# nka77/DAHiTra

Hardware: AMD Instinct MI355X
Metric: image-pairs/s (256x256) train step, 1/2/4/8 MI355X + CPU ref (higher is better)
Workload: dtype bf16; 1 GPU; LEVIR-CD 256x256 synthetic pairs, base_transformer_pos_s4, bf16, batch 32 per GPU (global 32), fwd+focal+bwd+allreduce+AdamW; net_G=base_transformer_pos_s4, global_batch=32, img_size=256, parallelism=dp1, hip_graph=True, step_form=one graph (AdamW inside), attn_dtype=bf16

## Files before the change

dahitra_amd/csrc/common.h:

```cpp
#pragma once
#include <hip/hip_runtime.h>
#include <stdint.h>

struct bf16 { unsigned short x; };

typedef __attribute__((ext_vector_type(4))) float f32x4;
typedef __attribute__((ext_vector_type(8))) short s16x8;
typedef __attribute__((ext_vector_type(4))) short s16x4;

#define DH_DTYPE_F32 0
#define DH_DTYPE_BF16 1

struct f32x3 { float v; };
struct f32x6 { float v; };
struct f32h3 { float v; };
constexpr float F32H3_WSCALE = 256.f;
template <typename T> struct Prec {
    static constexpr int NPL = 1;
    static constexpr bool X3 = false;
    static constexpr int CK = 64 / (int)sizeof(T);
};
template <> struct Prec<f32x3> {
    static constexpr int NPL = 2;
    static constexpr bool X3 = true;
// ... 116 lines not shown
#pragma unroll
    for (int j = 0; j < 8; ++j) r[j] = x[j];
#pragma unroll
    for (int p = 0; p < NPL; ++p) {
        pl[p] = pack16<bf16>(r);
        if (p + 1 < NPL) {
            float h[8];
            unpack16(pl[p], h);
#pragma unroll
            for (int j = 0; j < 8; ++j) r[j] -= h[j];
        }
    }
}
template <int NPL> __device__ __forceinline__ void split_bf16_planes(const uint4& a, const uint4& b, uint4 (&pl)[NPL]) {
    const float x[8] = {__uint_as_float(a.x), __uint_as_float(a.y), __uint_as_float(a.z), __uint_as_float(a.w),
                        __uint_as_float(b.x), __uint_as_float(b.y), __uint_as_float(b.z), __uint_as_float(b.w)};
    split_bf16_planes<NPL>(x, pl);
}
__device__ __forceinline__ void split_bf16x3(const float (&x)[8], uint4& hi, uint4& lo) {
    hi = pack16<bf16>(x);
    float h[8], r[8];
    unpack16(hi, h);
#pragma unroll
    for (int j = 0; j < 8; ++j) r[j] = x[j] - h[j];
    lo = pack16<bf16>(r);
}
__device__ __forceinline__ void split_bf16x3(const uint4& a, const uint4& b, uint4& hi, uint4& lo) {
    const float x[8] = {__uint_as_float(a.x), __uint_as_float(a.y), __uint_as_float(a.z), __uint_as_float(a.w),
                        __uint_as_float(b.x), __uint_as_float(b.y), __uint_as_float(b.z), __uint_as_float(b.w)};
    split_bf16x3(x, hi, lo);
}

__device__ __forceinline__ float row16_sum(float v) {
    v += __builtin_bit_cast(float, __builtin_amdgcn_update_dpp(0, __builtin_bit_cast(int, v), 0x128, 0xf, 0xf, false));
    v += __builtin_bit_cast(float, __builtin_amdgcn_update_dpp(0, __builtin_bit_cast(int, v), 0x124, 0xf, 0xf, false));
    v += __builtin_bit_cast(float, __builtin_amdgcn_update_dpp(0, __builtin_bit_cast(int, v), 0x122, 0xf, 0xf, false));
    v += __builtin_bit_cast(float, __builtin_amdgcn_update_dpp(0, __builtin_bit_cast(int, v), 0x121, 0xf, 0xf, false));
    return v;
}

__device__ __forceinline__ float wave_sum(float v) {
#pragma unroll
    for (int o = 32; o > 0; o >>= 1) v += __shfl_xor(v, o, 64);
    return v;
}
__device__ __forceinline__ float wave_max(float v) {
#pragma unroll
    for (int o = 32; o > 0; o >>= 1) v = fmaxf(v, __shfl_xor(v, o, 64));
    return v;
}

__device__ __forceinline__ float gelu_erf(float x) { return 0.5f * x * (1.0f + erff(x * 0.70710678118654752440f)); }
__device__ __forceinline__ float gelu_erf_grad(float x) {
    const float cdf = 0.5f * (1.0f + erff(x * 0.70710678118654752440f));
    const float pdf = 0.39894228040143267794f * __expf(-0.5f * x * x);
    return cdf + x * pdf;
}

#define DH_ACT_NONE 0
#define DH_ACT_RELU 1
#define DH_ACT_GELU 2

#include <stdio.h>
#include <string.h>
extern "C" void dh_set_error(const char* msg);
#define DH_FAIL(...)                                                     \
    do {                                                                 \
        char _b[512];                                                    \
        snprintf(_b, sizeof(_b), __VA_ARGS__);                           \
        dh_set_error(_b);                                                \
        return 1;                                                        \
    } while (0)
#define DH_REQUIRE(cond, ...)           \
    do {                                \
        if (!(cond)) DH_FAIL(__VA_ARGS__); \
    } while (0)
#define DH_CHECK_LAUNCH(name)                                                      \
    do {                                                                           \
        hipError_t _e = hipGetLastError();                                         \
        if (_e != hipSuccess) DH_FAIL("%s launch: %s", name, hipGetErrorString(_e)); \
    } while (0)
static inline int dh_cdiv(long a, long b) { return (int)((a + b - 1) / b); }

__device__ __forceinline__ void dh_reduce_partials_body(const float* __restrict__ partial, long nt, long n, float scale,
                                                        float* __restrict__ out, int accumulate, int bx, double (*red)[32]) {
    const int lane = threadIdx.x & 31, ph = threadIdx.x >> 5;
    const long i = (long)bx * 32 + lane;
    double s = 0.0;
    if (i < n) {
        double s1 = 0.0, s2 = 0.0, s3 = 0.0;
        long t = ph;
#pragma unroll 4
        for (; t + 24 < nt; t += 32) {
            s += (double)partial[t * n + i];
            s1 += (double)partial[(t + 8) * n + i];
            s2 += (double)partial[(t + 16) * n + i];
            s3 += (double)partial[(t + 24) * n + i];
        }
        for (; t < nt; t += 8) s += (double)partial[t * n + i];
        s = (s + s1) + (s2 + s3);
    }
    red[ph][lane] = s;
    __syncthreads();
    if (ph == 0 && i < n) {
        double t = 0.0;
#pragma unroll
        for (int r = 0; r < 8; ++r) t += red[r][lane];
        const float v = (float)(t * scale);
        if (accumulate) out[i] += v; else out[i] = v;
    }
}


__device__ __forceinline__ double dh_block_sum_f64(double v, double* sh) {
    for (int o = 32; o > 0; o >>= 1) v += __shfl_down(v, o, 64);
    const int w = threadIdx.x >> 6, l = threadIdx.x & 63;
    __syncthreads();
    if (l == 0) sh[w] = v;
    __syncthreads();
    double t = 0.0;
    if (threadIdx.x == 0) for (int i = 0; i < (int)(blockDim.x >> 6); ++i) t += sh[i];
    return t;
}
```

dahitra_amd/csrc/conv_wgrad.hip:

```cpp
#include "common.h"

namespace {

constexpr int TH = 8, TW = 16;
static inline int co_tile(int Cout) { return Cout <= 16 ? 16 : (Cout <= 32 ? 32 : 64); }

struct WgArgs {
    const void* x;
    const void* dy;
    float* part;
    int N, H, W, Cin, OH, OW, Cout, pad;
    int tilesX, tilesY, splitk, groups, npix, in_npix;
    int ci_tiles;
    int CinPitch;
    int dil;
    int CoutUse;
    int direct;
    const float* in_scale;
    const float* in_shift;
    int in_groups;
    int phase_mode;
    int no_xcd_remap;
    const void* dyt_y;
    const float* dytoef;
// ... 407 lines not shown
                }
            }
        }
        __syncthreads();
    }

    if constexpr (KSPLIT > 1) {
        float* red = reinterpret_cast<float*>(smem);
        for (int q = 1; q < KSPLIT; ++q) {
            if (kq == q) {
#pragma unroll
                for (int t = 0; t < TAPS; ++t)
#pragma unroll
                    for (int i = 0; i < NI; ++i)
                        *reinterpret_cast<f32x4*>(red + (((size_t)cw * TAPS * NI + t * NI + i) * 64 + lane) * 4) = acc[t][i];
            }
            __syncthreads();
            if (kq == 0) {
#pragma unroll
                for (int t = 0; t < TAPS; ++t)
#pragma unroll
                    for (int i = 0; i < NI; ++i) {
                        const f32x4 o = *reinterpret_cast<const f32x4*>(red + (((size_t)cw * TAPS * NI + t * NI + i) * 64 + lane) * 4);
                        acc[t][i][0] += o[0]; acc[t][i][1] += o[1]; acc[t][i][2] += o[2]; acc[t][i][3] += o[3];
                    }
            }
            __syncthreads();
        }
        if (kq != 0) return;
    }
    const int cob = co0 + (WCI ? 2 * cig * 16 : cw * 16) + g * 4, cib = ci0 + (WCI ? wv * 16 : cig * IT) + pl;
    float* out = p.part + ((size_t)grp * p.splitk + kz) * TAPS * p.Cout * p.Cin + (size_t)cob * p.Cin + cib;
    const int tstride = p.Cout * p.Cin;
    const int istep = WCI ? 16 * p.Cin : 16;
    bool okij[NI][4];
#pragma unroll
    for (int i = 0; i < NI; ++i)
#pragma unroll
        for (int j = 0; j < 4; ++j)
            okij[i][j] = WCI ? (cob + i * 16 + j < p.CoutUse && cib < p.Cin) : (cob + j < p.CoutUse && cib + i * 16 < p.Cin);
    if (p.direct == 2) {
#pragma unroll
        for (int t = 0; t < TAPS; ++t)
#pragma unroll
            for (int i = 0; i < NI; ++i)
#pragma unroll
                for (int j = 0; j < 4; ++j)
                    if (okij[i][j]) out[t * tstride + j * p.Cin + i * istep] += acc[t][i][j];
    } else {
#pragma unroll
        for (int t = 0; t < TAPS; ++t)
#pragma unroll
            for (int i = 0; i < NI; ++i)
#pragma unroll
                for (int j = 0; j < 4; ++j)
                    if (okij[i][j]) out[t * tstride + j * p.Cin + i * istep] = acc[t][i][j];
    }
}
template <typename T, int KS, int STRIDE, int IT, bool TR, int DIL, int CTT, int CIG, bool DYT = false>
__global__ __launch_bounds__(256 * CIG) void conv_wgrad_kernel(WgArgs p) {
    extern __shared__ __attribute__((aligned(16))) unsigned char smem[];
    wg_body<T, KS, STRIDE, IT, TR, DIL, CTT, CIG, DYT>(p, blockIdx.x, blockIdx.y, gridDim.x, gridDim.y, blockIdx.z, smem);
}
constexpr int WS_MAXJ = 16;
struct WsMulti {
    int njobs;
    int first[WS_MAXJ + 1];
    WgArgs a[WS_MAXJ];
};
static_assert(sizeof(WsMulti) <= 4096, "the kernel argument block");
template <typename T, int KS, int STRIDE, int IT, bool TR, int DIL, int CTT, int CIG>
__global__ __launch_bounds__(256 * CIG) void conv_wgrad_multi_kernel(WsMulti m) {
    extern __shared__ __attribute__((aligned(16))) unsigned char smem[];
    int j = 0;
    while (j + 1 < m.njobs && (int)blockIdx.x >= m.first[j + 1]) ++j;
    const WgArgs p = m.a[j];
    const int nbx = ((p.CoutUse + CTT - 1) / CTT) * p.ci_tiles, local = (int)blockIdx.x - m.first[j];
    if (local >= nbx * p.splitk) return;
    wg_body<T, KS, STRIDE, IT, TR, DIL, CTT, CIG, false>(p, local % nbx, local / nbx, nbx, p.splitk, 0, smem);
}

static inline int wgrad_reduce_epb(int I) { return (I & 3) == 0 ? 128 : 32; }
__device__ __forceinline__ void wgrad_reduce_block(const float* __restrict__ part, int splitk, int taps, int Oslab, int O,
                                                   int I, float* __restrict__ dw, int accumulate, long block, float (*red)[132]) {
    const long n = (long)O * I * taps;
    const int lane = threadIdx.x & 31, ph = threadIdx.x >> 5;
    const bool vec = (I & 3) == 0;
    const long i = vec ? (block * 32 + lane) * 4 : block * 32 + lane;
    float acc[4] = {0.f, 0.f, 0.f, 0.f};
    int tap = 0, ci = 0, o = 0;
    if (i < n) {
        ci = (int)(i % I);
        o = (int)((i / I) % O);
        tap = (int)(i / ((long)I * O));
        const size_t slab = (size_t)taps * Oslab * I;
        const float* src = part + ((size_t)tap * Oslab + o) * I + ci;
        if (vec) {
            float4 a0 = make_float4(0.f, 0.f, 0.f, 0.f), a1 = a0, a2 = a0, a3 = a0;
            auto add = [](float4& a, const float4 v) { a.x += v.x; a.y += v.y; a.z += v.z; a.w += v.w; };
            int k = ph;
            for (; k + 24 < splitk; k += 32) {
                add(a0, *reinterpret_cast<const float4*>(src + (size_t)k * slab));
                add(a1, *reinterpret_cast<const float4*>(src + (size_t)(k + 8) * slab));
                add(a2, *reinterpret_cast<const float4*>(src + (size_t)(k + 16) * slab));
                add(a3, *reinterpret_cast<const float4*>(src + (size_t)(k + 24) * slab));
            }
            for (; k < splitk; k += 8) add(a0, *reinterpret_cast<const float4*>(src + (size_t)k * slab));
            acc[0] = (a0.x + a1.x) + (a2.x + a3.x); acc[1] = (a0.y + a1.y) + (a2.y + a3.y);
            acc[2] = (a0.z + a1.z) + (a2.z + a3.z); acc[3] = (a0.w + a1.w) + (a2.w + a3.w);
        } else {
            float a1 = 0.f, a2 = 0.f, a3 = 0.f;
            int k = ph;
            for (; k + 24 < splitk; k += 32) {
                acc[0] += src[(size_t)k * slab];
                a1 += src[(size_t)(k + 8) * slab];
                a2 += src[(size_t)(k + 16) * slab];
                a3 += src[(size_t)(k + 24) * slab];
            }
            for (; k < splitk; k += 8) acc[0] += src[(size_t)k * slab];
            acc[0] = (acc[0] + a1) + (a2 + a3);
        }
    }
#pragma unroll
    for (int e = 0; e < 4; ++e) red[ph][lane * 4 + e] = acc[e];
    __syncthreads();
    const int t = threadIdx.x;
    if (t < (vec ? 128 : 32)) {
        const int l2 = vec ? t >> 2 : t, e = vec ? t & 3 : 0;
        const long i2 = vec ? (block * 32 + l2) * 4 + e : block * 32 + l2;
        if (i2 < n) {
            float s = 0.f;
#pragma unroll
            for (int r = 0; r < 8; ++r) s += red[r][l2 * 4 + e];
            const int ci2 = (int)(i2 % I), o2 = (int)((i2 / I) % O), tap2 = (int)(i2 / ((long)I * O));
            const size_t d = ((size_t)o2 * I + ci2) * taps + tap2;
            if (accumulate) dw[d] += s; else dw[d] = s;
        }
    }
}
__global__ void wgrad_reduce_oihw_kernel(const float* __restrict__ part, int splitk, int taps, int Oslab, int O, int I,
                                         float* __restrict__ dw, int accumulate) {
    __shared__ float red[8][132];
    const long n = (long)O * I * taps;
    wgrad_reduce_block(part + (size_t)blockIdx.y * splitk * taps * Oslab * I, splitk, taps, Oslab, O, I,
                       dw + (size_t)blockIdx.y * n, accumulate, blockIdx.x, red);
}
struct WgReduceJob {
    const float* part;
    float* dw;
    int splitk, taps, Oslab, O, I, accumulate, first_block, nblocks;
};
__global__ void wgrad_reduce_multi_kernel(const WgReduceJob* __restrict__ jobs, int njobs) {
    __shared__ float red[8][132];
    int j = 0;
    while (j + 1 < njobs && (int)blockIdx.x >= jobs[j + 1].first_block) ++j;
    const WgReduceJob job = jobs[j];
    wgrad_reduce_block(job.part, job.splitk, job.taps, job.Oslab, job.O, job.I, job.dw, job.accumulate,
                       (long)blockIdx.x - job.first_block, red);
}

#ifdef DH_WS_TIMING
__device__ long long g_ws[4096 * 16];
#define WS_NOW() ((long long)wall_clock64())
#define WS_T(...) __VA_ARGS__
#else
#define WS_T(...)
#endif
template <int DIL>
__device__ __forceinline__ void ws_body(const WgArgs& p, int bx, int kz, const int nbx, const int nkz, unsigned char* smem) {
    constexpr int KS = 3, TAPS = 9;
    constexpr int HH = (TH - 1) + (KS - 1) * DIL + 1, HWD = (TW - 1) + (KS - 1) * DIL + 1;
    constexpr int XP = lds_pitch(128), DP = lds_pitch(128);
    constexpr int STAGE = HH * HWD * XP + TH * TW * DP;
    float* bnp = reinterpret_cast<float*>(smem + 2 * STAGE);

    const int tid = threadIdx.x, lane = tid & 63, wv = tid >> 6;
    const int pl = lane & 15, g = lane >> 4;
    if (nbx > 1 && (nkz & 7) == 0 && !p.no_xcd_remap) {
        const unsigned lin = (unsigned)(kz * nbx + bx), xcd = lin & 7, sq = lin >> 3;
        bx = (int)(sq % nbx);
        kz = (int)((sq / nbx) * 8 + xcd);
    }
    const int cot = bx / p.ci_tiles, cit = bx % p.ci_tiles;
    const int co0 = cot * 64, ci0 = cit * 64;
    const int tiles_per_img = p.tilesX * p.tilesY;
    const int ntiles = p.N * tiles_per_img;
    const int my_tiles = kz < ntiles ? (ntiles - kz + p.splitk - 1) / p.splitk : 0;

    if (p.in_scale) {
        for (int i = tid; i < p.in_groups * 128; i += 512) {
            const int gi = i >> 7, k = (i >> 6) & 1, c = i & 63;
            bnp[i] = (k ? p.in_shift : p.in_scale)[gi * p.Cin + ci0 + c];
        }
        __syncthreads();
    }

    if (wv >= 4) {
        const int pt = tid - 256, q = pt & 7, prow = pt >> 3;
        constexpr int NXV = (HH * HWD + 31) / 32, NDV = TH * TW / 32;
        struct Regs { uint4 rx[NXV], rd[NDV]; unsigned okmask; int bng; };
        Regs RA, RB;
        int x_h[NXV];
#pragma unroll
        for (int i = 0; i < NXV; ++i) {
            const int px = prow + 32 * i;
            x_h[i] = px < HH * HWD ? ((px / HWD) << 8) | (px % HWD) : -1;
        }
        const unsigned xps = (unsigned)p.CinPitch * 2u, dps = (unsigned)p.Cout * 2u;
        const bool upper = p.x_split && ci0 >= p.Cin / 2;
        const long xsel = upper ? p.x_split : 0L;
        const unsigned xcb = (unsigned)((upper ? ci0 - p.Cin / 2 : ci0) + q * 8) * 2u, dcb = (unsigned)(co0 + q * 8) * 2u;
        const int dn = p.splitk / tiles_per_img, drem = p.splitk % tiles_per_img;
        const int dty = drem / p.tilesX, dtx = drem % p.tilesX;
        int f_n = kz / tiles_per_img, f_ty = (kz % tiles_per_img) / p.tilesX, f_tx = (kz % tiles_per_img) % p.tilesX;
        auto fetch = [&](Regs& R) {
            const int n = f_n;
            R.bng = p.in_scale ? n / (p.N / p.in_groups) : 0;
            const int oy0 = f_ty * TH, ox0 = f_tx * TW, iy0 = oy0 - p.pad, ix0 = ox0 - p.pad;
            const unsigned char* xb = reinterpret_cast<const unsigned char*>(p.x) + xsel + (size_t)n * p.H * p.W * xps;
            const unsigned char* db = reinterpret_cast<const unsigned char*>(p.dy) + (size_t)n * p.OH * p.OW * dps;
            R.okmask = 0;
#pragma unroll
            for (int i = 0; i < NXV; ++i) {
                const int iy = iy0 + (x_h[i] >> 8), ix = ix0 + (x_h[i] & 0xff);
                const bool ok = x_h[i] >= 0 && (unsigned)iy < (unsigned)p.H && (unsigned)ix < (unsigned)p.W;
                const uint4 v = *reinterpret_cast<const uint4*>(xb + (ok ? (unsigned)(iy * p.W + ix) * xps + xcb : 0u));
                R.rx[i] = ok ? v : make_uint4(0, 0, 0, 0);
                R.okmask |= ok ? (1u << i) : 0u;
            }
#pragma unroll
            for (int i = 0; i < NDV; ++i) {
                const int px = prow + 32 * i, oy = oy0 + (px >> 4), ox = ox0 + (px & 15);
                const bool ok = oy < p.OH && ox < p.OW;
                const uint4 v = *reinterpret_cast<const uint4*>(db + (ok ? (unsigned)(oy * p.OW + ox) * dps + dcb : 0u));
                R.rd[i] = ok ? v : make_uint4(0, 0, 0, 0);
            }
            f_tx += dtx;
            if (f_tx >= p.tilesX) { f_tx -= p.tilesX; ++f_ty; }
            f_ty += dty;
            if (f_ty >= p.tilesY) { f_ty -= p.tilesY; ++f_n; }
            f_n += dn;
// ... 565 lines not shown
    a.in_npix = npix_valid > 0 ? npix_valid : H * W;
    hipStream_t st = reinterpret_cast<hipStream_t>(stream);
    if (x_split) {
        a.ci_tiles = dh_cdiv(Cin, 64);
        DH_REQUIRE(dtype == DH_DTYPE_BF16 && ws_eligible(a, ks, stride, true, use_tr != 0) && wide_ci3x3(Cin, a.CoutUse, ks),
                   "conv2d_wgrad: a split input is served by the wave-specialised 3x3 kernel only (Cin=%d Cout=%d ks=%d)", Cin, Cout, ks);
    }
    const bool batching = g_wsb.on;
    if (!defer) g_wsb.on = false;
    int rc = dtype == DH_DTYPE_BF16 ? launch_all<bf16>(a, ks, stride, use_tr != 0, st)
             : wgrad_x3(dtype, a)   ? launch_all<f32x3>(a, ks, stride, true, st)
                                    : launch_all<float>(a, ks, stride, false, st);
    g_wsb.on = batching;
    if (rc) return rc;
    if (splitk_out) *splitk_out = a.direct ? 0 : a.splitk;
    if (a.direct || defer) return 0;
    const int taps = ks * ks;
    const int oreal = Cout_real > 0 ? Cout_real : Cout;
    const long n = (long)oreal * Cin * taps;
    hipLaunchKernelGGL(wgrad_reduce_oihw_kernel, dim3(dh_cdiv(n, wgrad_reduce_epb(Cin)), groups), dim3(256), 0, st, a.part, a.splitk,
                       taps, Cout, oreal, Cin, dw_oihw, accumulate);
    DH_CHECK_LAUNCH("wgrad_reduce");
    return 0;
}

extern "C" int dh_wgrad_batch_begin() { g_wsb.on = true; g_wsb.n = 0; g_wsb.lds = 0; g_c32b.n = 0; g_c32b.lds = 0; return 0; }
extern "C" int dh_wgrad_batch_pending() { return g_wsb.n + g_c32b.n; }
extern "C" int dh_wgrad_batch_abort() { g_wsb.on = false; g_wsb.n = 0; g_wsb.lds = 0; g_c32b.n = 0; g_c32b.lds = 0; return 0; }
extern "C" int dh_wgrad_batch_launch(void* stream) {
    const int rc = ws_batch_flush(reinterpret_cast<hipStream_t>(stream));
    return rc ? rc : c32_batch_flush(reinterpret_cast<hipStream_t>(stream));
}
extern "C" int dh_wgrad_batch_end(void* stream) {
    const int rc = dh_wgrad_batch_launch(stream);
    g_wsb.on = false;
    return rc;
}

extern "C" int dh_conv2d_wgrad(int dtype, const void* x, const void* dy, float* dw_oihw, int accumulate, int N,
                               int H, int W, int Cin, int OH, int OW, int Cout, int ks, int stride, int pad,
                               int groups, int npix_valid, int use_tr, int Cout_real, int cin_pitch, int dilation,
                               void* workspace, void* stream) {
    return conv2d_wgrad_impl(dtype, x, dy, dw_oihw, accumulate, N, H, W, Cin, OH, OW, Cout, ks, stride, pad, groups,
                             npix_valid, use_tr, Cout_real, cin_pitch, dilation, workspace, stream, 0, nullptr);
}

extern "C" int dh_conv2d_wgrad_partial(int dtype, const void* x, const void* dy, float* dw_oihw, int accumulate, int N,
                                       int H, int W, int Cin, int OH, int OW, int Cout, int ks, int stride, int pad,
                                       int groups, int npix_valid, int use_tr, int Cout_real, int cin_pitch,
                                       int dilation, void* workspace, int* splitk_out, void* stream) {
    DH_REQUIRE(groups == 1 && splitk_out, "conv2d_wgrad_partial: one group only");
    return conv2d_wgrad_impl(dtype, x, dy, dw_oihw, accumulate, N, H, W, Cin, OH, OW, Cout, ks, stride, pad, groups,
                             npix_valid, use_tr, Cout_real, cin_pitch, dilation, workspace, stream, 1, splitk_out);
}
bool dh_wgrad_split_supported(int N, int H, int W, int Cin, int Cout) {
    WgArgs a;
    memset(&a, 0, sizeof(a));
    a.dil = 1; a.in_groups = 1; a.dyt_groups = 1;
    a.N = N; a.H = H; a.W = W; a.Cin = Cin; a.OH = H; a.OW = W; a.Cout = Cout; a.CoutUse = Cout; a.pad = 1; a.groups = 1;
    a.CinPitch = Cin / 2; a.x_split = 16; a.npix = H * W; a.in_npix = H * W;
    return ws_eligible(a, 3, 1, true, true) && wide_ci3x3(Cin, Cout, 3);
}
extern "C" int dh_conv2d_wgrad_split(const void* x, long x_split_bytes, const void* dy, float* dw_oihw, int accumulate, int N, int H,
                                     int W, int Cin, int Cout, void* workspace, int* splitk_out, void* stream) {
    DH_REQUIRE(x_split_bytes > 0 && x_split_bytes % 16 == 0 && Cin % 128 == 0 && splitk_out, "conv2d_wgrad_split: bad arguments (Cin=%d)", Cin);
    return conv2d_wgrad_impl(DH_DTYPE_BF16, x, dy, dw_oihw, accumulate, N, H, W, Cin, H, W, Cout, 3, 1, 1, 1, 0, 1, 0, Cin / 2, 1,
                             workspace, stream, 1, splitk_out, nullptr, nullptr, 1, nullptr, nullptr, 1, x_split_bytes);
}
extern "C" int dh_conv2d_wgrad_bn_in(int dtype, const void* x, const void* dy, float* dw_oihw, int accumulate, int N,
                                     int H, int W, int Cin, int OH, int OW, int Cout, int ks, int stride, int pad,
                                     int use_tr, int Cout_real, int dilation, const float* in_scale, const float* in_shift,
                                     int in_groups, void* workspace, int* splitk_out, void* stream) {
    DH_REQUIRE(in_scale && in_shift, "conv2d_wgrad_bn_in: scale / shift missing");
    return conv2d_wgrad_impl(dtype, x, dy, dw_oihw, accumulate, N, H, W, Cin, OH, OW, Cout, ks, stride, pad, 1, 0, use_tr,
                             Cout_real, 0, dilation, workspace, stream, splitk_out ? 1 : 0, splitk_out, in_scale, in_shift,
                             in_groups);
}
extern "C" int dh_stem_wgrad_bn(const void* xs16, const void* d, const void* y, const float* coef, int groups, int N, int OH,
                                int OW, float* dw2, int use_tr, void* workspace, void* stream) {
    DH_REQUIRE(xs16 && d && y && coef && groups >= 1 && N % groups == 0, "stem_wgrad_bn: bad arguments (N=%d groups=%d)", N, groups);
    return conv2d_wgrad_impl(DH_DTYPE_BF16, xs16, d, dw2, 0, N, OH, OW, 16, OH, OW, 64, 4, 1, 2, 1, 0, use_tr, 0, 16, 1, workspace,
                             stream, 0, nullptr, nullptr, nullptr, 1, y, coef, groups);
}
extern "C" int dh_wgrad_reduce_job_size(void) { return (int)sizeof(WgReduceJob); }
extern "C" int dh_wgrad_reduce_outputs_per_block(int Cin) { return wgrad_reduce_epb(Cin); }
extern "C" int dh_wgrad_reduce_multi(const void* jobs_dev, int njobs, int total_blocks, void* stream) {
    if (njobs <= 0) return 0;
    hipLaunchKernelGGL(wgrad_reduce_multi_kernel, dim3(total_blocks), dim3(256), 0, reinterpret_cast<hipStream_t>(stream),
                       reinterpret_cast<const WgReduceJob*>(jobs_dev), njobs);
    DH_CHECK_LAUNCH("wgrad_reduce_multi");
    return 0;
}

static int phase_splitk(int N, int H, int W, int Cin) {
    const long tiles = (long)N * dh_cdiv(W, TW) * dh_cdiv(H, TH);
    const long slabs = (long)dh_cdiv(Cin, 32);
    long sk = (128 + slabs - 1) / slabs;
    if (sk > tiles / 8) sk = tiles / 8;
    return (int)(sk < 1 ? 1 : sk);
}
extern "C" long dh_conv2d_wgrad_phase_workspace_size(int N, int H, int W, int Cin) {
    return (long)4 * phase_splitk(N, H, W, Cin) * 4 * 32 * Cin * 4;
}
extern "C" int dh_conv2d_wgrad_phase(int dtype, const void* x, const void* dy, int N, int H, int W, int Cin, int use_tr,
                                     void* workspace, int* splitk_out, void* stream) {
    DH_REQUIRE(splitk_out && workspace, "conv2d_wgrad_phase: workspace / splitk_out missing");
    DH_REQUIRE((Cin * (dtype == DH_DTYPE_BF16 ? 2 : 4)) % 16 == 0, "conv2d_wgrad_phase: Cin=%d not 16-byte aligned", Cin);
    WgArgs a;
    a.x = x; a.dy = dy; a.part = reinterpret_cast<float*>(workspace);
    a.dil = 1; a.phase_mode = 1;
    a.no_xcd_remap = getenv("DAHITRA_NO_XCD_REMAP") ? 1 : 0;
    a.dyt_y = nullptr; a.dytoef = nullptr; a.dyt_groups = 1;
    a.in_scale = nullptr; a.in_shift = nullptr; a.in_groups = 1;
    a.CinPitch = Cin;
    a.N = N; a.H = H; a.W = W; a.Cin = Cin; a.OH = H; a.OW = W; a.Cout = 32; a.pad = 1;
    a.tilesX = dh_cdiv(W, TW); a.tilesY = dh_cdiv(H, TH);
    a.CoutUse = 32;
    a.x_split = 0;
    a.groups = 1; a.splitk = phase_splitk(N, H, W, Cin);
    a.direct = 0;
    a.npix = H * W; a.in_npix = H * W;
    hipStream_t st = reinterpret_cast<hipStream_t>(stream);
    const int rc = dtype == DH_DTYPE_BF16 ? launch_all<bf16>(a, 2, 1, use_tr != 0, st)
                   : wgrad_x3(dtype, a)   ? launch_all<f32x3>(a, 2, 1, true, st) : launch_all<float>(a, 2, 1, false, st);
    if (rc) return rc;
    *splitk_out = a.splitk;
    return 0;
}

namespace {
__global__ void phase_wgrad_combine_kernel(const float* __restrict__ dwab, float* __restrict__ dw, int Cin, int accumulate) {
    const int i = blockIdx.x * blockDim.x + threadIdx.x;
    if (i >= 32 * Cin) return;
    const size_t pstride = (size_t)32 * Cin * 4;
    const float* src = dwab + (size_t)i * 4;
    float v[4][4];
#pragma unroll
    for (int ph = 0; ph < 4; ++ph) {
        const float4 q = *reinterpret_cast<const float4*>(src + ph * pstride);
        v[ph][0] = q.x; v[ph][1] = q.y; v[ph][2] = q.z; v[ph][3] = q.w;
    }
    const int ra[3][2] = {{0, 1}, {0, 1}, {0, 1}}, rt[3][2] = {{0, 0}, {1, 0}, {1, 1}};
#pragma unroll
    for (int kh = 0; kh < 3; ++kh)
#pragma unroll
        for (int kw = 0; kw < 3; ++kw) {
            float s = 0.f;
#pragma unroll
            for (int m = 0; m < 2; ++m)
#pragma unroll
                for (int n = 0; n < 2; ++n) s += v[ra[kh][m] * 2 + ra[kw][n]][rt[kh][m] * 2 + rt[kw][n]];
            float* d = dw + (size_t)i * 9 + kh * 3 + kw;
            if (accumulate) *d += s; else *d = s;
        }
}

template <typename T>
__global__ void pack_phase_weights_kernel(const float* __restrict__ w, const float* __restrict__ bias, int Cin,
                                          T* __restrict__ fwd, T* __restrict__ dgrad, float* __restrict__ bias4) {
    const int i = blockIdx.x * blockDim.x + threadIdx.x;
    if (i < 128 && bias4) bias4[i] = bias ? bias[i & 31] : 0.f;
    if (i >= 32 * Cin) return;
    const int co = i / Cin, ci = i % Cin;
    float k[3][3];
#pragma unroll
    for (int j = 0; j < 9; ++j) k[j / 3][j % 3] = w[(size_t)i * 9 + j];
    const int lo[2][2] = {{0, 1}, {0, 2}}, hi[2][2] = {{0, 2}, {1, 2}};
#pragma unroll
    for (int a = 0; a < 2; ++a)
#pragma unroll
        for (int b = 0; b < 2; ++b)
#pragma unroll
            for (int t = 0; t < 2; ++t)
#pragma unroll
                for (int u = 0; u < 2; ++u) {
                    float s = 0.f;
                    for (int kh = lo[a][t]; kh <= hi[a][t]; ++kh)
                        for (int kw = lo[b][u]; kw <= hi[b][u]; ++kw) s += k[kh][kw];
                    const int ph = a * 2 + b;
                    if (fwd) stf(fwd + ((size_t)(t * 2 + u) * 128 + ph * 32 + co) * Cin + ci, s);
                    if (dgrad) stf(dgrad + ((size_t)((1 - t) * 2 + (1 - u)) * Cin + ci) * 128 + ph * 32 + co, s);
                }
}
}

namespace {
template <typename T>
__global__ void pack_s2_dgrad_phase_kernel(const float* __restrict__ w, int Co, int Ci, T* __restrict__ out) {
    const int i = blockIdx.x * blockDim.x + threadIdx.x;
    if (i >= Co * Ci) return;
    const int co = i / Ci, ci = i % Ci;
    float k[3][3];
#pragma unroll
    for (int j = 0; j < 9; ++j) k[j / 3][j % 3] = w[(size_t)i * 9 + j];
    const int kmap[2][2] = {{-1, 1}, {2, 0}};
#pragma unroll
    for (int a = 0; a < 2; ++a)
#pragma unroll
        for (int b = 0; b < 2; ++b)
#pragma unroll
            for (int t = 0; t < 2; ++t)
#pragma unroll
                for (int u = 0; u < 2; ++u) {
                    const int kh = kmap[a][t], kw = kmap[b][u];
                    const float v = (kh >= 0 && kw >= 0) ? k[kh][kw] : 0.f;
                    stf(out + ((size_t)(t * 2 + u) * 4 * Ci + (a * 2 + b) * Ci + ci) * Co + co, v);
                }
}
}
extern "C" int dh_pack_s2_dgrad_phase_weights(int dtype, const float* w_oihw, int Co, int Ci, void* out, void* stream) {
    DH_REQUIRE((Ci == 32 || Ci == 64) && Co % 16 == 0, "pack_s2_dgrad_phase_weights: Ci=%d (32 or 64) Co=%d", Ci, Co);
    const dim3 grid(dh_cdiv(Co * Ci, 256));
    hipStream_t st = reinterpret_cast<hipStream_t>(stream);
    if (dtype == DH_DTYPE_BF16) hipLaunchKernelGGL(pack_s2_dgrad_phase_kernel<bf16>, grid, dim3(256), 0, st, w_oihw, Co, Ci, (bf16*)out);
    else hipLaunchKernelGGL(pack_s2_dgrad_phase_kernel<float>, grid, dim3(256), 0, st, w_oihw, Co, Ci, (float*)out);
    DH_CHECK_LAUNCH("pack_s2_dgrad_phase_weights");
    return 0;
}
extern "C" int dh_phase_wgrad_combine(const float* dwab, float* dw_oihw, int Cin, int accumulate, void* stream) {
    hipLaunchKernelGGL(phase_wgrad_combine_kernel, dim3(dh_cdiv(32 * Cin, 256)), dim3(256), 0, reinterpret_cast<hipStream_t>(stream),
                       dwab, dw_oihw, Cin, accumulate);
    DH_CHECK_LAUNCH("phase_wgrad_combine");
    return 0;
}
extern "C" int dh_pack_phase_weights(int dtype, const float* w_oihw, const float* bias, int Cin, void* fwd, void* dgrad,
                                     float* bias4, void* stream) {
    DH_REQUIRE(Cin % 16 == 0, "pack_phase_weights: Cin=%d", Cin);
    const dim3 grid(dh_cdiv(32 * Cin, 256));
    hipStream_t st = reinterpret_cast<hipStream_t>(stream);
    if (dtype == DH_DTYPE_BF16)
        hipLaunchKernelGGL(pack_phase_weights_kernel<bf16>, grid, dim3(256), 0, st, w_oihw, bias, Cin, (bf16*)fwd, (bf16*)dgrad, bias4);
    else
        hipLaunchKernelGGL(pack_phase_weights_kernel<float>, grid, dim3(256), 0, st, w_oihw, bias, Cin, (float*)fwd, (float*)dgrad, bias4);
    DH_CHECK_LAUNCH("pack_phase_weights");
    return 0;
}
```

dahitra_amd/csrc/pointwise.hip:

```cpp
#include "common.h"

namespace {

inline int ew_grid(long n, int block) {
    long g = (n + block - 1) / block;
    return (int)(g > 8192 ? 8192 : (g < 1 ? 1 : g));
}
#define GSL(i, n) for (long i = (long)blockIdx.x * blockDim.x + threadIdx.x; i < (n); i += (long)gridDim.x * blockDim.x)

template <typename T>
__global__ void nchw_to_nhwc_kernel(const float* __restrict__ src, T* __restrict__ dst, int N, int C, long HW, int CP) {
    const long total = (long)N * HW * CP;
    GSL(i, total) {
        const int c = (int)(i % CP);
        const long p = (i / CP) % HW;
        const long n = i / (CP * HW);
        stf(dst + i, c < C ? src[(n * C + c) * HW + p] : 0.f);
    }
}
template <typename T>
__global__ void nchw_to_nhwc_piece_kernel(const float* __restrict__ src, T* __restrict__ dst, int N, int C, long HW) {
    constexpr int V = V16<T>::N;
    const long total = (long)N * HW;
    GSL(i, total) {
// ... 702 lines not shown

template <typename T>
__global__ void absdiff_kernel(const T* __restrict__ a, const T* __restrict__ b, T* __restrict__ y, long n) {
    GSL(i, n) stf(y + i, fabsf(ldf(a + i) - ldf(b + i)));
}
template <typename T>
__global__ void absdiff_bwd_kernel(const T* __restrict__ a, const T* __restrict__ b, const T* __restrict__ dy,
                                   T* __restrict__ da, T* __restrict__ db, long n, int accumulate) {
    GSL(i, n) {
        const float df = ldf(a + i) - ldf(b + i);
        const float sg = df > 0.f ? 1.f : (df < 0.f ? -1.f : 0.f);
        const float g = sg * ldf(dy + i);
        if (accumulate) { stf(da + i, ldf(da + i) + g); stf(db + i, ldf(db + i) - g); }
        else { stf(da + i, g); stf(db + i, -g); }
    }
}

template <typename T>
__global__ void zero_insert2_kernel(const T* __restrict__ dy, T* __restrict__ z, int N, int OH, int OW, int H, int W,
                                    int C) {
    const int vn = C / 4;
    GSL(i, (long)N * H * W * vn) {
        const int c = (int)(i % vn) * 4;
        long t = i / vn;
        const int x = (int)(t % W); t /= W;
        const int y = (int)(t % H);
        const long n = t / H;
        float v[4] = {0, 0, 0, 0};
        if (!(x & 1) && !(y & 1) && y / 2 < OH && x / 2 < OW) ld4(dy + ((n * OH + y / 2) * OW + x / 2) * C + c, v);
        st4(z + i * 4, v);
    }
}

template <typename T>
__global__ void add_coarse_kernel(T* __restrict__ x, const T* __restrict__ coarse, int N, int OH, int OW, int H, int W, int C) {
    constexpr int V = V16<T>::N;
    const int vn = C / V;
    GSL(i, (long)N * OH * OW * vn) {
        const int c = (int)(i % vn) * V;
        long t = i / vn;
        const int ox = (int)(t % OW); t /= OW;
        const int oy = (int)(t % OH);
        const long n = t / OH;
        if (2 * oy >= H || 2 * ox >= W) continue;
        float a[V], b[V];
        T* dst = x + ((n * H + 2 * oy) * W + 2 * ox) * C + c;
        ldv(dst, a);
        ldv(coarse + i * V, b);
#pragma unroll
        for (int j = 0; j < V; ++j) a[j] += b[j];
        stv(dst, a);
    }
}

template <typename T>
__global__ void pack_weight_kernel(const float* __restrict__ w, const float* __restrict__ oscale, int O, int I, int KS,
                                   int OPad, T* __restrict__ fwd, int IPad, int OK, T* __restrict__ dgrad) {
    const int taps = KS * KS;
    if (fwd) {
        GSL(i, (long)taps * OPad * I) {
            const int ci = (int)(i % I);
            const int o = (int)((i / I) % OPad);
            const int tap = (int)(i / ((long)I * OPad));
            stf(fwd + i, o < O ? w[((long)o * I + ci) * taps + tap] * (oscale ? oscale[o] : 1.f) : 0.f);
        }
    }
    if (dgrad) {
        GSL(i, (long)taps * IPad * OK) {
            const int o = (int)(i % OK);
            const int ci = (int)((i / OK) % IPad);
            const int tap = (int)(i / ((long)OK * IPad));
            stf(dgrad + i, (ci < I && o < O) ? w[((long)o * I + ci) * taps + (taps - 1 - tap)] : 0.f);
        }
    }
}

struct PackJob {
    const float* w;
    void* fwd;
    void* dgrad;
    int O, I, KS, OPad, IPad, OK;
    int dtype;
    int first_block, nblocks;
};
template <typename T>
__device__ __forceinline__ void pack_store8(T* dst, const float* __restrict__ src, unsigned stride, unsigned okmask) {
    float v[8];
#pragma unroll
    for (int e = 0; e < 8; ++e) v[e] = ((okmask >> e) & 1) ? src[(size_t)e * stride] : 0.f;
    if constexpr (sizeof(T) == 2) {
        uint4 u;
        u.x = f2bf2(v[0], v[1]); u.y = f2bf2(v[2], v[3]); u.z = f2bf2(v[4], v[5]); u.w = f2bf2(v[6], v[7]);
        *reinterpret_cast<uint4*>(dst) = u;
    } else {
        *reinterpret_cast<float4*>(dst) = make_float4(v[0], v[1], v[2], v[3]);
        *reinterpret_cast<float4*>(dst + 4) = make_float4(v[4], v[5], v[6], v[7]);
    }
}
template <typename T> __device__ __forceinline__ void pack_put8(T* dst, const float (&v)[8]) {
    if constexpr (sizeof(T) == 2) {
        uint4 u;
        u.x = f2bf2(v[0], v[1]); u.y = f2bf2(v[2], v[3]); u.z = f2bf2(v[4], v[5]); u.w = f2bf2(v[6], v[7]);
        *reinterpret_cast<uint4*>(dst) = u;
    } else {
        *reinterpret_cast<float4*>(dst) = make_float4(v[0], v[1], v[2], v[3]);
        *reinterpret_cast<float4*>(dst + 4) = make_float4(v[4], v[5], v[6], v[7]);
    }
}
constexpr int PK_T = 32, PK_ROW = PK_T * 9, PK_PITCH = PK_ROW + 1;
__host__ __device__ inline bool pack_tiled(const PackJob& j) {
    return j.KS == 3 && j.O % PK_T == 0 && j.I % PK_T == 0 && j.OPad == j.O && j.IPad == j.I && j.OK == j.O &&
           (reinterpret_cast<unsigned long long>(j.w) & 15) == 0;
}
template <typename T>
__device__ __forceinline__ void pack_job_tiled(const PackJob& j, int lb, float* t ) {
    const int tid = threadIdx.x, nti = j.I / PK_T, ntiles = (j.O / PK_T) * nti;
    T* fwd = reinterpret_cast<T*>(j.fwd);
    T* dgrad = reinterpret_cast<T*>(j.dgrad);
    const bool frag = (j.dtype & 0x200) != 0;
    for (int tile = lb; tile < ntiles; tile += j.nblocks) {
        const int o0 = (tile / nti) * PK_T, c0 = (tile % nti) * PK_T;
        __syncthreads();
        for (int q = tid; q < PK_T * (PK_ROW / 4); q += 256) {
            const int r = q / (PK_ROW / 4), k = (q % (PK_ROW / 4)) * 4;
            const float4 v = *reinterpret_cast<const float4*>(j.w + ((size_t)(o0 + r) * j.I + c0) * 9 + k);
            float* d = t + r * PK_PITCH + k;
            d[0] = v.x; d[1] = v.y; d[2] = v.z; d[3] = v.w;
        }
        __syncthreads();
        for (int q = tid; q < 9 * PK_T * 4; q += 256) {
            float v[8];
            if (frag) {
                const int lane = q & 63, tap = (q >> 6) % 9, blk = q / (64 * 9);
                const int rr = blk * 16 + (lane & 15), kk = (lane >> 4) * 8;
                if (fwd) {
#pragma unroll
                    for (int e = 0; e < 8; ++e) v[e] = t[rr * PK_PITCH + (kk + e) * 9 + tap];
                    pack_put8(fwd + ((((size_t)(o0 / 16 + blk) * (j.I / 32) + c0 / 32) * 9 + tap) * 64 + lane) * 8, v);
                }
                if (dgrad) {
#pragma unroll
                    for (int e = 0; e < 8; ++e) v[e] = t[(kk + e) * PK_PITCH + rr * 9 + (8 - tap)];
                    pack_put8(dgrad + ((((size_t)(c0 / 16 + blk) * (j.OK / 32) + o0 / 32) * 9 + tap) * 64 + lane) * 8, v);
                }
            } else {
                const int pc = q & 3, r = (q >> 2) & 31, tap = q >> 7;
                if (fwd) {
#pragma unroll
                    for (int e = 0; e < 8; ++e) v[e] = t[r * PK_PITCH + (pc * 8 + e) * 9 + tap];
                    pack_put8(fwd + ((size_t)tap * j.OPad + o0 + r) * j.I + c0 + pc * 8, v);
                }
                if (dgrad) {
#pragma unroll
                    for (int e = 0; e < 8; ++e) v[e] = t[(pc * 8 + e) * PK_PITCH + r * 9 + (8 - tap)];
                    pack_put8(dgrad + ((size_t)tap * j.IPad + c0 + r) * j.OK + o0 + pc * 8, v);
                }
            }
        }
    }
}
template <typename T>
__device__ __forceinline__ void pack_job(const PackJob& j, int lb) {
    const int taps = j.KS * j.KS;
    const unsigned step = (unsigned)j.nblocks * blockDim.x;
    T* fwd = reinterpret_cast<T*>(j.fwd);
    T* dgrad = reinterpret_cast<T*>(j.dgrad);
    const unsigned t0 = (unsigned)lb * blockDim.x + threadIdx.x;
    if (j.dtype & 0x200) {
        const int nch_f = j.I / 32, nch_d = j.OK / 32;
        if (fwd)
            for (unsigned i8 = t0; i8 < (unsigned)(taps * j.OPad * j.I) / 8; i8 += step) {
                const unsigned i = i8 * 8;
                const int lane = (int)((i >> 3) & 63), tap = (int)((i >> 9) % (unsigned)taps);
                const int c = (int)((i / (512u * (unsigned)taps)) % (unsigned)nch_f), r16 = (int)(i / (512u * (unsigned)taps * (unsigned)nch_f));
                const int o = r16 * 16 + (lane & 15), ci = c * 32 + (lane >> 4) * 8;
                pack_store8(fwd + i, j.w + (unsigned)((o * j.I + ci) * taps + tap), (unsigned)taps, o < j.O ? 0xffu : 0u);
            }
        if (dgrad)
            for (unsigned i8 = t0; i8 < (unsigned)(taps * j.IPad * j.OK) / 8; i8 += step) {
                const unsigned i = i8 * 8;
                const int lane = (int)((i >> 3) & 63), tap = (int)((i >> 9) % (unsigned)taps);
                const int c = (int)((i / (512u * (unsigned)taps)) % (unsigned)nch_d), r16 = (int)(i / (512u * (unsigned)taps * (unsigned)nch_d));
                const int ci = r16 * 16 + (lane & 15), o = c * 32 + (lane >> 4) * 8;
                unsigned ok = 0;
#pragma unroll
                for (int e = 0; e < 8; ++e) ok |= (unsigned)(ci < j.I && o + e < j.O) << e;
                pack_store8(dgrad + i, j.w + (unsigned)((o * j.I + ci) * taps + (taps - 1 - tap)), (unsigned)(j.I * taps), ok);
            }
        return;
    }
    if (fwd) {
        if (j.I % 8 == 0) {
            for (unsigned i8 = t0; i8 < (unsigned)(taps * j.OPad * j.I) / 8; i8 += step) {
                const unsigned i = i8 * 8;
                const int ci = (int)(i % (unsigned)j.I);
                const int o = (int)((i / (unsigned)j.I) % (unsigned)j.OPad);
                const int tap = (int)(i / (unsigned)(j.I * j.OPad));
                pack_store8(fwd + i, j.w + (unsigned)((o * j.I + ci) * taps + tap), (unsigned)taps, o < j.O ? 0xffu : 0u);
            }
        } else {
            for (unsigned i = t0; i < (unsigned)(taps * j.OPad * j.I); i += step) {
                const int ci = (int)(i % (unsigned)j.I);
                const int o = (int)((i / (unsigned)j.I) % (unsigned)j.OPad);
                const int tap = (int)(i / (unsigned)(j.I * j.OPad));
                stf(fwd + i, o < j.O ? j.w[(unsigned)((o * j.I + ci) * taps + tap)] : 0.f);
            }
        }
    }
    if (dgrad) {
        if (j.OK % 8 == 0) {
            for (unsigned i8 = t0; i8 < (unsigned)(taps * j.IPad * j.OK) / 8; i8 += step) {
                const unsigned i = i8 * 8;
                const int o = (int)(i % (unsigned)j.OK);
                const int ci = (int)((i / (unsigned)j.OK) % (unsigned)j.IPad);
                const int tap = (int)(i / (unsigned)(j.OK * j.IPad));
                unsigned ok = 0;
#pragma unroll
                for (int e = 0; e < 8; ++e) ok |= (unsigned)(ci < j.I && o + e < j.O) << e;
                pack_store8(dgrad + i, j.w + (unsigned)((o * j.I + ci) * taps + (taps - 1 - tap)), (unsigned)(j.I * taps), ok);
            }
        } else {
            for (unsigned i = t0; i < (unsigned)(taps * j.IPad * j.OK); i += step) {
                const int o = (int)(i % (unsigned)j.OK);
                const int ci = (int)((i / (unsigned)j.OK) % (unsigned)j.IPad);
                const int tap = (int)(i / (unsigned)(j.OK * j.IPad));
                stf(dgrad + i, (ci < j.I && o < j.O) ? j.w[(unsigned)((o * j.I + ci) * taps + (taps - 1 - tap))] : 0.f);
            }
        }
    }
}
__global__ __launch_bounds__(256) void pack_weights_multi_kernel(const PackJob* __restrict__ jobs, int njobs) {
    int lo = 0, hi = njobs - 1;
    while (lo < hi) {
        const int mid = (lo + hi + 1) >> 1;
        if (jobs[mid].first_block <= (int)blockIdx.x) lo = mid; else hi = mid - 1;
    }
    const PackJob j = jobs[lo];
    const int lb = blockIdx.x - j.first_block;
    __shared__ __attribute__((aligned(16))) float tile[PK_T * PK_PITCH];
    if (pack_tiled(j)) {
        if ((j.dtype & 0xff) == DH_DTYPE_BF16) pack_job_tiled<bf16>(j, lb, tile); else pack_job_tiled<float>(j, lb, tile);
        return;
    }
    if ((j.dtype & 0xff) == DH_DTYPE_BF16) pack_job<bf16>(j, lb); else pack_job<float>(j, lb);
}

template <typename T>
__global__ __launch_bounds__(256) void colsum_partial_kernel(const T* __restrict__ x, long P, int C,
                                                             float* __restrict__ partial) {
    __shared__ float red[256 * 8];
    constexpr int V = sizeof(T) == 2 ? 8 : 4;
    if (C % V == 0 && C <= 1024 && 256 % (C / V) == 0) {
        const int cvn = C / V, cv = threadIdx.x % cvn, ph = threadIdx.x / cvn, nph = 256 / cvn;
        float s[4][V];
#pragma unroll
        for (int u = 0; u < 4; ++u)
#pragma unroll
            for (int j = 0; j < V; ++j) s[u][j] = 0.f;
        const long step = (long)gridDim.x * nph;
        long p = (long)blockIdx.x * nph + ph;
        auto row = [&](long r, float (&acc)[V]) {
            float v[V];
            if constexpr (V == 8) unpack16(*reinterpret_cast<const uint4*>(x + r * C + cv * V), v);
            else ld4(x + r * C + cv * V, v);
#pragma unroll
            for (int j = 0; j < V; ++j) acc[j] += v[j];
        };
        for (; p + 3 * step < P; p += 4 * step) {
            row(p, s[0]); row(p + step, s[1]); row(p + 2 * step, s[2]); row(p + 3 * step, s[3]);
        }
        for (int u = 0; p < P; p += step, ++u) row(p, s[u & 3]);
        float* mine = red + threadIdx.x * V;
#pragma unroll
        for (int j = 0; j < V; ++j) mine[j] = (s[0][j] + s[1][j]) + (s[2][j] + s[3][j]);
        __syncthreads();
        for (int c = threadIdx.x; c < C; c += 256) {
            float t = 0.f;
            for (int r = 0; r < nph; ++r) t += red[(r * cvn + c / V) * V + (c % V)];
            partial[(long)blockIdx.x * C + c] = t;
        }
        return;
    }
    const int c = threadIdx.x % C, ph = threadIdx.x / C, nph = 256 / C;
    float s = 0.f;
    if (ph < nph)
        for (long p = (long)blockIdx.x * nph + ph; p < P; p += (long)gridDim.x * nph) s += ldf(x + p * C + c);
    red[threadIdx.x] = s;
    __syncthreads();
    if (threadIdx.x < C) {
        float t = 0.f;
        for (int r = 0; r < nph; ++r) t += red[r * C + threadIdx.x];
        partial[(long)blockIdx.x * C + threadIdx.x] = t;
    }
}

template <typename T>
__global__ void cast_from_f32_kernel(const float* __restrict__ src, T* __restrict__ dst, long n) {
    GSL(i, n) stf(dst + i, src[i]);
}
template <typename T>
__global__ void cast_to_f32_kernel(const T* __restrict__ src, float* __restrict__ dst, long n, int accumulate) {
    GSL(i, n) { if (accumulate) dst[i] += ldf(src + i); else dst[i] = ldf(src + i); }
}

}

#define ST(s) reinterpret_cast<hipStream_t>(s)
extern "C" int dh_reduce_partials(const float* partial, long nt, long n, float scale, float* out, int accumulate,
                                  void* stream);

extern "C" int dh_nchw_to_nhwc(int dtype, const float* src, void* dst, int N, int C, long HW, int CP, void* stream) {
    if (CP < C) CP = C;
    const long n = (long)N * CP * HW;
    if (CP * (dtype == DH_DTYPE_BF16 ? 2 : 4) == 16) {
        const long np = (long)N * HW;
        if (dtype == DH_DTYPE_BF16) hipLaunchKernelGGL(nchw_to_nhwc_piece_kernel<bf16>, dim3(ew_grid(np, 256)), dim3(256), 0, ST(stream), src, (bf16*)dst, N, C, HW);
        else hipLaunchKernelGGL(nchw_to_nhwc_piece_kernel<float>, dim3(ew_grid(np, 256)), dim3(256), 0, ST(stream), src, (float*)dst, N, C, HW);
        DH_CHECK_LAUNCH("nchw_to_nhwc");
        return 0;
    }
    if (dtype == DH_DTYPE_BF16) hipLaunchKernelGGL(nchw_to_nhwc_kernel<bf16>, dim3(ew_grid(n, 256)), dim3(256), 0, ST(stream), src, (bf16*)dst, N, C, HW, CP);
// ... 178 lines not shown
    return 0;
}
extern "C" int dh_upsample2_nearest_bwd(int dtype, const void* dy, void* dx, int N, int H, int W, int C, void* stream) {
    const int V = dtype == DH_DTYPE_BF16 ? 8 : 4;
    DH_REQUIRE(C % V == 0, "upsample2: C=%d must be a multiple of %d", C, V);
    const long n = (long)N * H * W * (C / V);
    if (dtype == DH_DTYPE_BF16) hipLaunchKernelGGL(up2_bwd_kernel<bf16>, dim3(ew_grid(n, 256)), dim3(256), 0, ST(stream), (const bf16*)dy, (bf16*)dx, N, H, W, C);
    else hipLaunchKernelGGL(up2_bwd_kernel<float>, dim3(ew_grid(n, 256)), dim3(256), 0, ST(stream), (const float*)dy, (float*)dx, N, H, W, C);
    DH_CHECK_LAUNCH("up2_bwd");
    return 0;
}
extern "C" int dh_absdiff_upsample4_fwd(int dtype, const void* a, const void* b, void* y, int N, int H, int W, int C, void* stream) {
    const int V = dtype == DH_DTYPE_BF16 ? 8 : 4;
    DH_REQUIRE(C % V == 0, "absdiff_upsample4: C=%d must be a multiple of %d", C, V);
    const long n = (long)N * H * W * (C / V);
    if (dtype == DH_DTYPE_BF16) hipLaunchKernelGGL(absdiff_up4_fwd_kernel<bf16>, dim3(ew_grid(n, 256)), dim3(256), 0, ST(stream), (const bf16*)a, (const bf16*)b, (bf16*)y, N, H, W, C);
    else hipLaunchKernelGGL(absdiff_up4_fwd_kernel<float>, dim3(ew_grid(n, 256)), dim3(256), 0, ST(stream), (const float*)a, (const float*)b, (float*)y, N, H, W, C);
    DH_CHECK_LAUNCH("absdiff_up4_fwd");
    return 0;
}
extern "C" int dh_absdiff_upsample4_bwd(int dtype, const void* a, const void* b, const void* dy, void* da, void* db, int N, int H, int W, int C, void* stream) {
    const int V = dtype == DH_DTYPE_BF16 ? 8 : 4;
    DH_REQUIRE(C % V == 0, "absdiff_upsample4: C=%d must be a multiple of %d", C, V);
    const long n = (long)N * H * W * (C / V);
    if (dtype == DH_DTYPE_BF16) hipLaunchKernelGGL(absdiff_up4_bwd_kernel<bf16>, dim3(ew_grid(n, 256)), dim3(256), 0, ST(stream), (const bf16*)a, (const bf16*)b, (const bf16*)dy, (bf16*)da, (bf16*)db, N, H, W, C);
    else hipLaunchKernelGGL(absdiff_up4_bwd_kernel<float>, dim3(ew_grid(n, 256)), dim3(256), 0, ST(stream), (const float*)a, (const float*)b, (const float*)dy, (float*)da, (float*)db, N, H, W, C);
    DH_CHECK_LAUNCH("absdiff_up4_bwd");
    return 0;
}
extern "C" int dh_absdiff_up4_combine(const float* partial, const void* a, const void* b, void* da, void* db, int N, int H, int W,
                                      void* stream) {
    DH_REQUIRE(H % 2 == 0 && W % 4 == 0, "absdiff_up4_combine: coarse map %dx%d must tile into 8x16 fine tiles", H, W);
    const long n = (long)N * H * W * 4;
    hipLaunchKernelGGL(absdiff_up4_combine_kernel, dim3(ew_grid(n, 256)), dim3(256), 0, ST(stream), partial, (const bf16*)a,
                       (const bf16*)b, (bf16*)da, (bf16*)db, N, H, W);
    DH_CHECK_LAUNCH("absdiff_up4_combine");
    return 0;
}
extern "C" int dh_absdiff(int dtype, const void* a, const void* b, void* y, long n, void* stream) {
    if (dtype == DH_DTYPE_BF16) hipLaunchKernelGGL(absdiff_kernel<bf16>, dim3(ew_grid(n, 256)), dim3(256), 0, ST(stream), (const bf16*)a, (const bf16*)b, (bf16*)y, n);
    else hipLaunchKernelGGL(absdiff_kernel<float>, dim3(ew_grid(n, 256)), dim3(256), 0, ST(stream), (const float*)a, (const float*)b, (float*)y, n);
    DH_CHECK_LAUNCH("absdiff");
    return 0;
}
extern "C" int dh_absdiff_bwd(int dtype, const void* a, const void* b, const void* dy, void* da, void* db, long n, int accumulate, void* stream) {
    if (dtype == DH_DTYPE_BF16) hipLaunchKernelGGL(absdiff_bwd_kernel<bf16>, dim3(ew_grid(n, 256)), dim3(256), 0, ST(stream), (const bf16*)a, (const bf16*)b, (const bf16*)dy, (bf16*)da, (bf16*)db, n, accumulate);
    else hipLaunchKernelGGL(absdiff_bwd_kernel<float>, dim3(ew_grid(n, 256)), dim3(256), 0, ST(stream), (const float*)a, (const float*)b, (const float*)dy, (float*)da, (float*)db, n, accumulate);
    DH_CHECK_LAUNCH("absdiff_bwd");
    return 0;
}
extern "C" int dh_zero_insert2(int dtype, const void* dy, void* z, int N, int OH, int OW, int H, int W, int C, void* stream) {
    DH_REQUIRE(C % 4 == 0, "zero_insert2: C %% 4");
    const long n = (long)N * H * W * (C / 4);
    if (dtype == DH_DTYPE_BF16) hipLaunchKernelGGL(zero_insert2_kernel<bf16>, dim3(ew_grid(n, 256)), dim3(256), 0, ST(stream), (const bf16*)dy, (bf16*)z, N, OH, OW, H, W, C);
    else hipLaunchKernelGGL(zero_insert2_kernel<float>, dim3(ew_grid(n, 256)), dim3(256), 0, ST(stream), (const float*)dy, (float*)z, N, OH, OW, H, W, C);
    DH_CHECK_LAUNCH("zero_insert2");
    return 0;
}
extern "C" int dh_add_coarse(int dtype, void* x, const void* coarse, int N, int OH, int OW, int H, int W, int C, void* stream) {
    const int V = dtype == DH_DTYPE_BF16 ? 8 : 4;
    DH_REQUIRE(C % V == 0 && x && coarse && OH == (H + 1) / 2 && OW == (W + 1) / 2, "add_coarse: C=%d, %dx%d <- %dx%d", C, H, W, OH, OW);
    const long n = (long)N * OH * OW * (C / V);
    if (dtype == DH_DTYPE_BF16) hipLaunchKernelGGL(add_coarse_kernel<bf16>, dim3(ew_grid(n, 256)), dim3(256), 0, ST(stream), (bf16*)x, (const bf16*)coarse, N, OH, OW, H, W, C);
    else hipLaunchKernelGGL(add_coarse_kernel<float>, dim3(ew_grid(n, 256)), dim3(256), 0, ST(stream), (float*)x, (const float*)coarse, N, OH, OW, H, W, C);
    DH_CHECK_LAUNCH("add_coarse");
    return 0;
}
extern "C" int dh_pack_weight(int dtype, const float* w_oihw, const float* out_scale, int O, int I, int ks, int OPad, void* fwd, int IPad, int dgrad_inner, void* dgrad, void* stream) {
    const int OK = dgrad_inner > O ? dgrad_inner : O;
    const long n = (long)ks * ks * (OPad > IPad ? OPad : IPad) * (OK > I ? OK : I);
    if (dtype == DH_DTYPE_BF16) hipLaunchKernelGGL(pack_weight_kernel<bf16>, dim3(ew_grid(n, 256)), dim3(256), 0, ST(stream), w_oihw, out_scale, O, I, ks, OPad, (bf16*)fwd, IPad, OK, (bf16*)dgrad);
    else hipLaunchKernelGGL(pack_weight_kernel<float>, dim3(ew_grid(n, 256)), dim3(256), 0, ST(stream), w_oihw, out_scale, O, I, ks, OPad, (float*)fwd, IPad, OK, (float*)dgrad);
    DH_CHECK_LAUNCH("pack_weight");
    return 0;
}
extern "C" int dh_pack_job_size(void) { return (int)sizeof(PackJob); }
extern "C" int dh_pack_weights_multi(const void* jobs_dev, int njobs, int total_blocks, void* stream) {
    if (njobs <= 0) return 0;
    hipLaunchKernelGGL(pack_weights_multi_kernel, dim3(total_blocks), dim3(256), 0, ST(stream),
                       reinterpret_cast<const PackJob*>(jobs_dev), njobs);
    DH_CHECK_LAUNCH("pack_weights_multi");
    return 0;
}
extern "C" int dh_colsum(int dtype, const void* x, long P, int C, float* out, int accumulate, void* workspace, void* stream) {
    DH_REQUIRE(C >= 1 && C <= 256, "colsum: C=%d out of range", C);
    const long rows_per_pass = 256 / (C >= 4 && (C & 3) == 0 ? C / 4 : C);
    long want = (P + rows_per_pass * 8 - 1) / (rows_per_pass * 8);
    const int grid = (int)(want < 64 ? 64 : (want > 256 ? 256 : want));
    float* partial = reinterpret_cast<float*>(workspace);
    if (dtype == DH_DTYPE_BF16) hipLaunchKernelGGL(colsum_partial_kernel<bf16>, dim3(grid), dim3(256), 0, ST(stream), (const bf16*)x, P, C, partial);
    else hipLaunchKernelGGL(colsum_partial_kernel<float>, dim3(grid), dim3(256), 0, ST(stream), (const float*)x, P, C, partial);
    DH_CHECK_LAUNCH("colsum");
    return dh_reduce_partials(partial, grid, C, 1.0f, out, accumulate, stream);
}
extern "C" int dh_cast_from_f32(int dtype, const float* src, void* dst, long n, void* stream) {
    if (dtype == DH_DTYPE_BF16) hipLaunchKernelGGL(cast_from_f32_kernel<bf16>, dim3(ew_grid(n, 256)), dim3(256), 0, ST(stream), src, (bf16*)dst, n);
    else hipLaunchKernelGGL(cast_from_f32_kernel<float>, dim3(ew_grid(n, 256)), dim3(256), 0, ST(stream), src, (float*)dst, n);
    DH_CHECK_LAUNCH("cast_from_f32");
    return 0;
}
extern "C" int dh_cast_to_f32(int dtype, const void* src, float* dst, long n, int accumulate, void* stream) {
    if (dtype == DH_DTYPE_BF16) hipLaunchKernelGGL(cast_to_f32_kernel<bf16>, dim3(ew_grid(n, 256)), dim3(256), 0, ST(stream), (const bf16*)src, dst, n, accumulate);
    else hipLaunchKernelGGL(cast_to_f32_kernel<float>, dim3(ew_grid(n, 256)), dim3(256), 0, ST(stream), (const float*)src, dst, n, accumulate);
    DH_CHECK_LAUNCH("cast_to_f32");
    return 0;
}

namespace {
template <typename T>
__device__ __forceinline__ void absdiff_halves_body(const T* __restrict__ tok, T* __restrict__ out, int B, long n, int bid, int nb) {
    GSLB(i, (long)B * n, bid, nb) {
        const long b = i / n, j = i % n;
        stf(out + i, fabsf(ldf(tok + (b * 2 + 1) * n + j) - ldf(tok + (b * 2) * n + j)));
    }
}
template <typename T>
__global__ void absdiff_halves_kernel(const T* __restrict__ tok, T* __restrict__ out, int B, long n) {
    absdiff_halves_body<T>(tok, out, B, n, blockIdx.x, gridDim.x);
}
template <typename T>
__device__ __forceinline__ void absdiff_halves_bwd_body(const T* __restrict__ tok, const T* __restrict__ dout, T* __restrict__ dtok,
                                                        int B, long n, int bid, int nb) {
    GSLB(i, (long)B * n, bid, nb) {
        const long b = i / n, j = i % n;
        const float df = ldf(tok + (b * 2 + 1) * n + j) - ldf(tok + (b * 2) * n + j);
        const float g = (df > 0.f ? 1.f : (df < 0.f ? -1.f : 0.f)) * ldf(dout + i);
        T* p1 = dtok + (b * 2 + 1) * n + j;
        T* p0 = dtok + (b * 2) * n + j;
        stf(p1, ldf(p1) + g);
        stf(p0, ldf(p0) - g);
    }
}
template <typename T>
__global__ void absdiff_halves_bwd_kernel(const T* __restrict__ tok, const T* __restrict__ dout, T* __restrict__ dtok,
                                          int B, long n) {
    absdiff_halves_bwd_body<T>(tok, dout, dtok, B, n, blockIdx.x, gridDim.x);
}

enum { DH_EW_ADD_POS = 1, DH_EW_CAT_HALVES = 2, DH_EW_SPLIT_HALVES = 3, DH_EW_ABSDIFF_HALVES = 4, DH_EW_ABSDIFF_HALVES_BWD = 5,
       DH_EW_ADD_POS_BWD = 6 };
struct EwJob {
    int op, blk0, nblk, i0, i1;
    long l0;
    const void* a;
    const void* b;
    void* c;
};
constexpr int EW_MAXJ = 12;
struct EwMulti {
    EwJob j[EW_MAXJ];
    int n;
};
__global__ __launch_bounds__(256) void ew_multi_kernel(EwMulti m) {
    int k = 0;
    while (k + 1 < m.n && (int)blockIdx.x >= m.j[k + 1].blk0) ++k;
    const EwJob& J = m.j[k];
    const int bid = (int)blockIdx.x - J.blk0, nb = J.nblk;
    switch (J.op) {
        case DH_EW_ADD_POS: add_pos16_body<bf16>((const bf16*)J.a, (const float*)J.b, (bf16*)J.c, J.i0, J.l0, J.i1, bid, nb); break;
        case DH_EW_CAT_HALVES: cat_halves_body<bf16, false>((bf16*)const_cast<void*>(J.a), (bf16*)J.c, J.i0, J.l0, bid, nb); break;
        case DH_EW_SPLIT_HALVES: cat_halves_body<bf16, true>((bf16*)J.c, (bf16*)const_cast<void*>(J.a), J.i0, J.l0, bid, nb); break;
        case DH_EW_ABSDIFF_HALVES: absdiff_halves_body<float>((const float*)J.a, (float*)J.c, J.i0, J.l0, bid, nb); break;
        case DH_EW_ABSDIFF_HALVES_BWD: absdiff_halves_bwd_body<float>((const float*)J.a, (const float*)J.b, (float*)J.c, J.i0, J.l0, bid, nb); break;
        case DH_EW_ADD_POS_BWD: add_pos_bwd32_body((const bf16*)J.a, (float*)J.c, J.i0, J.l0, J.i1, bid); break;
        default: break;
    }
}
}
extern "C" int dh_ew_multi(int n, const int* op, const void* const* a, const void* const* b, void* const* c, const int* i0,
                           const int* i1, const long* l0, void* stream) {
    DH_REQUIRE(n >= 1 && n <= EW_MAXJ && op && a && b && c && i0 && i1 && l0, "ew_multi: 1 .. %d jobs, got %d", EW_MAXJ, n);
    EwMulti m;
    int nblk = 0;
    for (int k = 0; k < n; ++k) {
        EwJob& J = m.j[k];
        J.op = op[k]; J.a = a[k]; J.b = b[k]; J.c = c[k]; J.i0 = i0[k]; J.i1 = i1[k]; J.l0 = l0[k];
// ... 42 lines not shown
```

dahitra_amd/engine.py:

```python
import os
import sys
import types

import torch

from . import ops
from .netspec import (ATTN_SCALE, BIT_DIM_HEAD, BIT_HEADS, BN_EPS, BN_MOMENTUM, DIM, LN_EPS, UNET_LEVELS,
                      get_config, is_active, state_spec)

RELU, GELU, NONE = ops.ACT_RELU, ops.ACT_GELU, ops.ACT_NONE



def _drain(gen):
    try:
        while True:
            next(gen)
    except StopIteration as e:
        return e.value


class Packed:
    __slots__ = ("fwd", "dgrad", "fwd_frag", "dgrad_frag")

# ... 175 lines not shown
                       w_frag=self.pk[wkey].dgrad_frag if stride == 1 else None)
        return Gated(*r) if gate is not None else r

    def conv_bn(self, x, wkey, bnkey, ks, stride, pad, groups, relu, residual=None, dilation=1, lazy=False, side_wgrad=False):
        cout = self.shapes[wkey][0]
        lazy = lazy and self.training and self.lazy_bn and relu and residual is None and not self.fused_bn_bwd
        gamma, beta = self.p[bnkey + ".weight"], self.p[bnkey + ".bias"]
        rm, rv = self.p[bnkey + ".running_mean"], self.p[bnkey + ".running_var"]
        act = RELU if relu else NONE
        split = isinstance(x, ops.SplitCat)
        if split and not (self.training and ks == 3 and stride == 1 and pad == 1 and dilation == 1 and residual is None):
            x, split = x.materialize(), False
        relu_bits = None
        if self.training:
            if split:
                y, st = ops.conv3x3_split(x, self.pk[wkey].fwd, self.pk[wkey].fwd_frag, cout, want_stats=True)
            else:
                y, st = ops.conv2d(x, self.pk[wkey].fwd, cout, ks, stride, pad, want_stats=True, dilation=dilation,
                                   w_frag=self.pk[wkey].fwd_frag if stride == 1 else None)
            N, OH, OW, _ = y.shape
            mean, invstd, scale, shift = ops.bn_finalize(st, cout, groups, (N // groups) * OH * OW, gamma, beta, rm, rv,
                                                         BN_MOMENTUM, BN_EPS, nbt=self.p[bnkey + ".num_batches_tracked"])
            if lazy:
                out = ops.BnInput(y, scale, shift, groups)
            elif relu and residual is not None and self.need_grad:
                out, relu_bits = ops.bn_apply(y, scale, shift, groups, act, residual, want_bits=True)
            else:
                out = ops.bn_apply(y, scale, shift, groups, act, residual)
        else:
            scale, shift = ops.bn_eval_params(gamma, beta, rm, rv, BN_EPS)
            wp = ops.pack_weight(self.p[wkey], self.dtype, want_dgrad=False, out_scale=scale)[0]
            out = ops.conv2d(x, wp, cout, ks, stride, pad, bias=shift, residual=residual, act=act, dilation=dilation)
            y = mean = invstd = None
        if not self.need_grad:
            return out, None
        has_res = residual is not None

        def bwd(dout, need_dx=True, dx_res=None, next_gate=None, coarse_dx=False, through_up4=None):
            if isinstance(dout, HeadGrad):
                dy = ops.head_bn_bwd(dout.dl, dout.w, dout.ncls, y, scale, shift, mean, invstd, gamma,
                                     self.g[bnkey + ".weight"], self.g[bnkey + ".bias"], groups, dw=dout.gw, db=dout.gb)
                dres = None
            elif isinstance(dout, Gated):
                dy = ops.bn_bwd_from_partials(dout.g, y, dout.partial, mean, invstd, gamma, self.g[bnkey + ".weight"],
                                              self.g[bnkey + ".bias"], groups, accumulate=True)
                dres = dout.g if has_res else None
            elif relu and not has_res:
                dy, dres = ops.bn_bwd(dout, None, y, mean, invstd, gamma, self.g[bnkey + ".weight"],
                                      self.g[bnkey + ".bias"], groups, accumulate=True, mask_scale=scale,
                                      mask_shift=shift), None
            else:
                r = ops.bn_bwd(dout, out if relu else None, y, mean, invstd, gamma, self.g[bnkey + ".weight"],
                               self.g[bnkey + ".bias"], groups, accumulate=True, want_dres=has_res, bits=relu_bits)
                dy, dres = r if has_res else (r, None)
            if side_wgrad and self.side is not None:
                self._deferred_wgrad = (x, dy, wkey, ks, stride, pad, dilation)
            else:
                ops.conv2d_wgrad(x, dy, self.g[wkey], ks, stride, pad, accumulate=True, use_tr=self.use_tr,
                                 dilation=dilation)
            if through_up4 is not None:
                return ops.conv3x3_dgrad_through_up4(dy, self.pk[wkey].dgrad, *through_up4), dres
            if split and need_dx:
                assert dx_res is None and next_gate is None and not coarse_dx
                cin = x.shape[-1]
                return ops.conv3x3_split(dy, self.pk[wkey].dgrad, self.pk[wkey].dgrad_frag, cin, split_out=True,
                                         alg_flops=2.0 * dy.shape[0] * dy.shape[1] * dy.shape[2] * cout * cin * 9), dres
            dx = self.conv_dgrad(dy, wkey, ks, stride, pad, x.shape, residual=dx_res, dilation=dilation,
                                 gate=next_gate, coarse=coarse_dx) if need_dx else None
            return dx, dres
        bwd.gate = (out if relu else None, y, mean, invstd, groups) if (self.fused_bn_bwd and cout % 16 == 0) else None
        bwd.bn = (y, scale, shift, mean, invstd, groups) if (self.training and relu and not has_res) else None
        return out, bwd

    def conv_act(self, x, wkey, bkey, ks, pad, act, cpad_grad=False):
        cout = self.shapes[wkey][0]
        out = ops.conv2d(x, self.pk[wkey].fwd, cout, ks, 1, pad, bias=self.p[bkey] if bkey else None, act=act)
        if not self.need_grad:
            return out, None

        def bwd(dout, need_dx=True, dx_res=None, masked=False):
            dy = ops.act_bwd(dout, out, RELU) if (act == RELU and not masked) else dout
            ops.conv2d_wgrad(x, dy, self.g[wkey], ks, 1, pad, accumulate=True, use_tr=self.use_tr)
            if bkey:
                ops.colsum(dy.view(-1, cout), self.g[bkey], accumulate=True)
            dx = self.conv_dgrad(dy, wkey, ks, 1, pad, x.shape, residual=dx_res) if need_dx else None
            return dx
        return out, bwd

    def conv_pred_phase(self, x):
        wkey, bkey = "conv_pred.weight", "conv_pred.bias"
        wf, wd, b4 = ops.pack_phase_weights(self.p[wkey], self.p[bkey], self.dtype)
        out = ops.conv_up2_fwd(x, wf, b4)
        if not self.need_grad:
            return out, None

        def bwd(dout):
            ops.conv_up2_wgrad(x, dout, self.g[wkey], accumulate=True, use_tr=self.use_tr)
            ops.colsum(dout.view(-1, 32), self.g[bkey], accumulate=True)
            return ops.conv_up2_dgrad(dout, wd, x.shape[-1])
        return out, bwd

    def stem(self, x1, x2, groups, pool=False):
        B = x1.shape[0]
        H, W = x1.shape[2], x1.shape[3]
        wkey, bnkey = "resnet.conv1.weight", "resnet.bn1"
        gamma, beta = self.p[bnkey + ".weight"], self.p[bnkey + ".bias"]
        rm, rv = self.p[bnkey + ".running_mean"], self.p[bnkey + ".running_var"]
        oh, ow = H // 2, W // 2
        direct = self.direct_stem and self.dtype == torch.bfloat16
        if not direct:
            cp = ops.chunk_channels(self.dtype)
            xs = torch.empty(2 * B, H // 2, W // 2, cp, dtype=self.dtype, device=x1.device)
            ops.stem_space_to_depth_into(x1, xs[:B])
            ops.stem_space_to_depth_into(x2, xs[B:])
        if self.training:
            if direct:
                y, st, xs = ops.stem7_fwd(x1, x2, self.p[wkey], want_stats=True, want_xs=self.need_grad, groups=groups)
            else:
                y, st = ops.conv2d(xs, self.pk[wkey].fwd, 64, 4, 1, 2, want_stats=True, out_hw=(oh, ow))
            mean, invstd, scale, shift = ops.bn_finalize(st, 64, groups, B * oh * ow, gamma, beta, rm, rv, BN_MOMENTUM,
                                                         BN_EPS, nbt=self.p[bnkey + ".num_batches_tracked"])
            if pool:
                out = None
                pooled, parg = ops.maxpool(y, want_arg=True, bn=(scale, shift, groups))
            else:
                out = ops.bn_apply(y, scale, shift, groups, RELU)
        else:
            scale, shift = ops.bn_eval_params(gamma, beta, rm, rv, BN_EPS)
            if direct:
                out = ops.stem7_fwd(x1, x2, self.p[wkey], out_scale=scale, bias=shift, relu=True)[0]
            else:
                wp = ops.stem_pack_weight(self.p[wkey], self.dtype, out_scale=scale)
                out = ops.conv2d(xs, wp, 64, 4, 1, 2, bias=shift, act=RELU, out_hw=(oh, ow))
            y = mean = invstd = None
            if pool:
                pooled, parg = ops.maxpool(out), None
        oshape = (2 * B, oh, ow, 64)

        def bwd(dout):
            dy = ops.bn_bwd(dout, None, y, mean, invstd, gamma, self.g[bnkey + ".weight"], self.g[bnkey + ".bias"],
                            groups, accumulate=True, mask_scale=scale, mask_shift=shift)
            ops.stem_wgrad(xs, dy, self.g[wkey], accumulate=True, use_tr=self.use_tr)

        def from_pool(parg_, dpool, extra=None):
            d, coef = ops.stem_pool_bn_bwd(parg_, dpool, y, scale, shift, mean, invstd, gamma, self.g[bnkey + ".weight"],
                                           self.g[bnkey + ".bias"], groups, extra=extra)
            ops.stem_wgrad(xs, d, self.g[wkey], accumulate=True, use_tr=self.use_tr, bn=(y, coef, groups))
        if self.training and direct and self.fused_stem_bwd and self.need_grad:
            bwd.from_pool = from_pool
        if pool:
            return pooled, parg, oshape, (bwd if self.need_grad else None)
        if not self.need_grad:
            return out, None
        return out, bwd

    def basic_block(self, x, pfx, stride, groups):
        h, b1 = self.conv_bn(x, pfx + ".conv1.weight", pfx + ".bn1", 3, stride, 1, groups, True, lazy=True)
        has_ds = (pfx + ".downsample.0.weight") in self.shapes
        if has_ds:
            idt, bds = self.conv_bn(x, pfx + ".downsample.0.weight", pfx + ".downsample.1", 1, stride, 0, groups, False)
        else:
            idt, bds = x, None
        out, b2 = self.conv_bn(h, pfx + ".conv2.weight", pfx + ".bn2", 3, 1, 1, groups, True, residual=idt)
        if not self.need_grad:
            return out, None

        def bwd(dout, next_gate=None):
            dh, dres = b2(dout, next_gate=b1.gate)
            if has_ds:
                if stride == 2 and next_gate is None and self.phase_s2_dgrad and x.shape[-1] in (32, 64):
                    dxds, _ = bds(dres, coarse_dx=True)
                    dx, _ = b1(dh, dx_res=CoarseRes(dxds), next_gate=next_gate)
                else:
                    dxds, _ = bds(dres)
                    dx, _ = b1(dh, dx_res=dxds, next_gate=next_gate)
            else:
                dx, _ = b1(dh, dx_res=dres, next_gate=next_gate)
            return dx
        bwd.gate = b2.gate
        return out, bwd

# ... 447 lines not shown
        with self.side.fork(x.y if isinstance(x, ops.BnInput) else (x.a if isinstance(x, ops.Up4Input) else x), dy):
            ops.conv2d_wgrad(x, dy, self.g[wkey], ks, stride, pad, accumulate=True, use_tr=self.use_tr, dilation=dilation)

    def _side_join(self):
        if self.side is not None:
            self.run_deferred_wgrad()
            self.side.join()

    def backward_second(self):
        ops.set_f32_mma_mode(self.mma_bwd)
        second, state = self._split_state
        self._split_state = None
        try:
            second(state)
            self._wgrad_plan.run()
        finally:
            self._wgrad_plan.__exit__(*sys.exc_info())

    def _head_out(self, h, wkey, bkey):
        ncls = self.shapes[wkey][0]
        ck = ops.chunk_channels(self.dtype)
        if self.pk[wkey].fwd.shape[-2] == 16 and self.fused_head_out:
            out = ops.conv3x3_head(h, self.pk[wkey].fwd, ncls, self.p[bkey], w_oihw=self.p[wkey])
        else:
            out = ops.nhwc_to_nchw(ops.conv2d(h, self.pk[wkey].fwd, ncls, 3, 1, 1, bias=self.p[bkey]))
        if not self.need_grad:
            return out, None

        small = 8 if (self.dtype == torch.bfloat16 or ncls > 4) else 4
        direct = h.shape[-1] == 32 and ncls <= small

        def bwd(dl_nchw, next_gate=None, head_bn=None, relu_out=None):
            if direct and next_gate is None:
                fuse = self.fused_head_bn and ncls <= 8 and self.g[wkey].is_contiguous() and \
                    (self.dtype == torch.bfloat16 or (self.dtype == torch.float32 and ops.get_f32_mma_mode() != 0))
                if head_bn is not None and fuse:
                    return HeadGrad(ops.head_dlogits_pack(dl_nchw, self.dtype), self.p[wkey], ncls, self.g[wkey], self.g[bkey])
                if relu_out is not None and fuse and relu_out is h:
                    return ops.head_relu_bwd(ops.head_dlogits_pack(dl_nchw, self.dtype), self.p[wkey], ncls, h, self.g[wkey],
                                             self.g[bkey])
                dl = ops.nchw_to_nhwc(dl_nchw, self.dtype, cpad=small)
                ops.conv2d_wgrad(h, dl, self.g[wkey], 3, 1, 1, accumulate=True, use_tr=self.use_tr, cout_real=ncls)
                tmp = torch.empty(small, dtype=torch.float32, device=h.device)
                ops.colsum(dl.view(-1, small), tmp)
                ops.reduce_rows(tmp, 1, ncls, self.g[bkey], accumulate=True)
                if head_bn is not None and self.gated_head_dgrad and self.dtype == torch.bfloat16 and ncls <= 2:
                    return Gated(*ops.head_dgrad3x3_bn(dl, self.p[wkey], ncls, *head_bn))
                return ops.head_dgrad3x3(dl, self.p[wkey], ncls, relu_out=relu_out)
            dl = ops.nchw_to_nhwc(dl_nchw, self.dtype, cpad=ck)
            ops.conv2d_wgrad(h, dl, self.g[wkey], 3, 1, 1, accumulate=True, use_tr=self.use_tr, cout_real=ncls)
            tmp = torch.empty(ck, dtype=torch.float32, device=h.device)
            ops.colsum(dl.view(-1, ck), tmp)
            ops.reduce_rows(tmp, 1, ncls, self.g[bkey], accumulate=True)
            dh = self.conv_dgrad(dl, wkey, 3, 1, 1, h.shape, gate=next_gate)
            return ops.act_bwd(dh, relu_out, RELU) if relu_out is not None else dh
        return out, bwd

    def _bit(self, x1, x2):
        cfg, L = self.cfg, self.cfg["token_len"]
        B = x1.shape[0]
        S2 = 2 * B
        xp, xarg, xshape, b_stem = self.stem(x1, x2, 2, pool=True)
        self._pack_join()
        if cfg.get("backbone") == "resnet50":
            l1, b_l1 = self.res50_layer(xp, 1, 1, 1, 1, 2)
            l2, b_l2 = self.res50_layer(l1, 2, 2, 1, 1, 2)
            l3, b_l3 = self.res50_layer(l2, 3, 1, 1, 2, 2)
        else:
            l1, b_l1 = self.res_layer(xp, 1, 1, 2)
            l2, b_l2 = self.res_layer(l1, 2, 2, 2)
            l3, b_l3 = self.res_layer(l2, 3, 1, 2)
        phased = self.phase_conv_pred and l3.shape[-1] % 64 == 0
        if phased:
            feat, b_pred = self.conv_pred_phase(l3)
        else:
            up = ops.upsample2(l3)
            feat, b_pred = self.conv_act(up, "conv_pred.weight", "conv_pred.bias", 3, 1, NONE)
        _, fh, fw, _ = feat.shape
        hw = fh * fw
        wa = self.p["conv_a.weight"]
        tok_cat, tsaved = ops.tokenizer_fwd(feat, wa, self.p["pos_embedding"], B, L)
        tok2d, b_enc = self.encoder(tok_cat.view(B * 2 * L, DIM), "transformer", cfg["enc_depth"], BIT_HEADS,
                                    BIT_DIM_HEAD, B, 2 * L)
        dtok = torch.zeros_like(tok2d) if self.need_grad else None
        dec, b_dec = self.decoder(feat.view(S2 * hw, DIM), S2, tok2d, 2 * L * DIM, L * DIM, B, dtok,
                                  "transformer_decoder", cfg["dec_depth"], BIT_HEADS, cfg["dec_dim_head"], L)
        dec4 = dec.view(S2, fh, fw, DIM)
        k0 = "classifier.0.weight"
        if self.fused_up4_fwd and self.dtype == torch.bfloat16 and DIM == 32 and tuple(self.shapes[k0][:2]) == (32, 32) and \
                tuple(self.pk[k0].fwd.shape) == (9, 32, 32):
            upd = ops.Up4Input(dec4[:B].contiguous(), dec4[B:].contiguous())
        else:
            upd = ops.absdiff_upsample4(dec4[:B], dec4[B:])
        h, b_c0 = self.conv_bn(upd, k0, "classifier.1", 3, 1, 1, 1, True, lazy=True, side_wgrad=True)
        logits, b_out = self._head_out(h, "classifier.3.weight", "classifier.3.bias")
        if not self.need_grad:
            return logits, None

        def bwd_first(dl):
            dh = b_out(dl, next_gate=b_c0.gate, head_bn=getattr(b_c0, "bn", None))
            fuse = self.fused_up4_bwd and self.dtype == torch.bfloat16 and fh % 2 == 0 and fw % 4 == 0 and \
                self.pk["classifier.0.weight"].dgrad.dim() == 3 and self.pk["classifier.0.weight"].dgrad.shape[1] == 32
            if fuse:
                dec_g = torch.empty_like(dec4)
                b_c0(dh, through_up4=(dec4[:B], dec4[B:], dec_g[:B], dec_g[B:]))
            else:
                dupd, _ = b_c0(dh)
                dec_g = torch.empty_like(dec4)
                ops.absdiff_upsample4_bwd_into(dec4[:B], dec4[B:], dupd, dec_g[:B], dec_g[B:])
            dfeat = b_dec(dec_g.view(S2 * hw, DIM))
            if self.side is not None:
                self.run_deferred_wgrad()
            dtok_cat = b_enc(dtok)
            dfeat4 = dfeat.view(S2, fh, fw, DIM)
            ops.tokenizer_bwd(feat, wa, tsaved, dtok_cat, dfeat4, self.g["conv_a.weight"], self.g["pos_embedding"],
                              B, L, accumulate=True)
            dl3 = b_pred(dfeat4) if phased else ops.upsample2_bwd(b_pred(dfeat4))
            return b_l3(dl3, next_gate=b_l2.gate)

        def bwd_second(dl2):
            dxp = b_l1(b_l2(dl2, next_gate=b_l1.gate))
            if hasattr(b_stem, "from_pool"):
                b_stem.from_pool(xarg, dxp)
            else:
                b_stem(ops.maxpool_bwd(xarg, dxp, xshape))

        def bwd(dl):
            bwd_second(bwd_first(dl))
        bwd.split = (bwd_first, bwd_second, ("resnet.conv1.", "resnet.bn1.", "resnet.layer1.", "resnet.layer2."))
        return logits, bwd

    def _zeros_like(self, t):
        zp, n = getattr(self, "_zpool", None), t.numel()
        if zp is not None and t.dtype == torch.float32 and zp[1] + n <= zp[0].numel():
            out = zp[0][zp[1]:zp[1] + n].view(t.shape)
            zp[1] += (n + 63) // 64 * 64
            return out
        return torch.zeros_like(t)

    def _run_staged(self, gens, ew=False):
        vals = {}
        streams = None
        if self.level_streams and len(gens) > 1 and ops.PROFILE is None:
            dev = torch.cuda.current_device()
            while len(self._lstreams) < len(gens):
                self._lstreams.append(ops.SideStream(torch.device("cuda", dev)))
            streams = self._lstreams
        with ops.EncoderBatch(decoder=True, ew=ew and streams is None) as eb:
            live = list(enumerate(gens))
            while live:
                paused = []
                for i, g in live:
                    try:
                        if streams is not None:
                            with streams[i].fork():
                                next(g)
                        else:
                            next(g)
                        paused.append((i, g))
                    except StopIteration as e:
                        vals[id(g)] = e.value
                if streams is not None:
                    for st in streams:
                        st.join()
                eb.launch()
                live = paused
        return [vals[id(g)] for g in gens]

    def _level(self, l, xa_b, B):
        lv, L = UNET_LEVELS[l], self.cfg["token_len"]
        S2 = 2 * B
        sq, b_sq = self.conv_act(xa_b, "conv_squeeze_%d.0.weight" % l, None, 1, 0, RELU)
        _, fh, fw, _ = sq.shape
        hw = fh * fw
        wa = self.p["conv_token_%d.weight" % l]
        tok_cat, tsaved = ops.tokenizer_fwd(sq, wa, self.p["pos_embedding_%d" % l], B, L)
        tok2d, b_enc = self.encoder(tok_cat.view(B * 2 * L, DIM), "transformer_%d" % l, self.cfg["enc_depth"],
                                    lv["heads"], lv["dim_head"], B, 2 * L)
        pos = self.p["pos_embedding_decoder_%d" % l]
        xin = ops.add_pos(sq, pos)
        yield
        dtok = self._zeros_like(tok2d) if self.need_grad else None
        dp = "transformer_decoder_%d" % l
        dec, b_dec = yield from self._decoder_gen(xin.view(S2 * hw, DIM), S2, tok2d, 2 * L * DIM, L * DIM, B, dtok, dp,
                                                  lv["dec_depth"], lv["heads"], lv["dim_head"], L)
        dec4 = dec.view(S2, fh, fw, DIM)
        cat = ops.cat_halves(dec4)
        tk3 = tok2d.view(B, 2, L * DIM)
        dtk = torch.empty(B, L, DIM, dtype=torch.float32, device=sq.device)
        ops.absdiff_halves(tk3, dtk)
        ddtk = self._zeros_like(dtk) if self.need_grad else None
        yield
        dxc, b_cd = self.conv_act(cat, "conv_decode_%d.weight" % l, None, 3, 1, NONE)
        xin3 = ops.add_pos(dxc, pos)
        out, b_dec3 = yield from self._decoder_gen(xin3.view(B * hw, DIM), B, dtk.view(B * L, DIM), L * DIM, 0, B, ddtk, dp,
                                                   lv["dec_depth"], lv["heads"], lv["dim_head"], L)
        out4 = out.view(B, fh, fw, DIM)
        if not self.need_grad:
            return out4, None
        gpos = self.g["pos_embedding_decoder_%d" % l]

        def bwd(dout4):
            dxin3 = (yield from b_dec3(dout4.reshape(B * hw, DIM))).view(B, fh, fw, DIM)
            ops.add_pos_bwd(dxin3, gpos, accumulate=True)
            dcat = b_cd(dxin3)
            ops.absdiff_halves_bwd(tk3, ddtk, dtok)
            ddec = ops.split_halves(dcat)
            dxin = (yield from b_dec(ddec.view(S2 * hw, DIM))).view(S2, fh, fw, DIM)
            ops.add_pos_bwd(dxin, gpos, accumulate=True)
            dtok_cat = b_enc(dtok)
            yield
            ops.tokenizer_bwd(sq, wa, tsaved, dtok_cat, dxin, self.g["conv_token_%d.weight" % l],
                              self.g["pos_embedding_%d" % l], B, L, accumulate=True)
            yield
            return b_sq(dxin)
        return out4, bwd

    def _xbd_level(self, l, xa_b, B):
        lv, L = UNET_LEVELS[l], self.cfg["token_len"]
        sq, b_sq = self.conv_act(xa_b, "conv_squeeze_%d.0.weight" % l, None, 1, 0, RELU)
        _, fh, fw, _ = sq.shape
        hw = fh * fw
        wa = self.p["conv_token_%d.weight" % l]
        with_pos = l == 5
        pos_tok = self.p["pos_embedding_3"] if with_pos else torch.zeros(1, 2 * L, DIM, device=sq.device)
        tok_cat, tsaved = ops.tokenizer_fwd(sq, wa, pos_tok, B, L)
        tok2d, b_enc = self.encoder(tok_cat.view(B * 2 * L, DIM), "transformer_%d" % l, self.cfg["enc_depth"],
                                    lv["heads"], lv["dim_head"], B, 2 * L)
        yield
        tk3 = tok2d.view(B, 2, L * DIM)
        dtk = torch.empty(B, L, DIM, dtype=torch.float32, device=sq.device)
        ops.absdiff_halves(tk3, dtk)
        ddtk = self._zeros_like(dtk) if self.need_grad else None
        cat = ops.cat_halves(sq)
        dxc, b_cd = self.conv_act(cat, "conv_decode_%d.weight" % l, None, 3, 1, NONE)
        pos = self.p["pos_embedding_decoder_3"] if (with_pos and self.cfg["decoder_pos"]) else None
        xin = ops.add_pos(dxc, pos) if pos is not None else dxc
        out, b_dec = yield from self._decoder_gen(xin.view(B * hw, DIM), B, dtk.view(B * L, DIM), L * DIM, 0, B, ddtk,
                                                  "transformer_decoder_%d" % l, lv["dec_depth"], lv["heads"], lv["dim_head"], L)
        out4 = out.view(B, fh, fw, DIM)
        if not self.need_grad:
            return out4, None

        def bwd(dout4):
            dxin = (yield from b_dec(dout4.reshape(B * hw, DIM))).view(B, fh, fw, DIM)
            if pos is not None:
                ops.add_pos_bwd(dxin, self.g["pos_embedding_decoder_3"], accumulate=True)
            dcat = b_cd(dxin)
            dtok = torch.zeros_like(tok2d)
            ops.absdiff_halves_bwd(tk3, ddtk, dtok)
            dtok_cat = b_enc(dtok)
            yield
            dsq = ops.split_halves(dcat)
            gpos = self.g["pos_embedding_3"] if with_pos else torch.zeros(1, 2 * L, DIM, device=sq.device)
            ops.tokenizer_bwd(sq, wa, tsaved, dtok_cat, dsq, self.g["conv_token_%d.weight" % l], gpos, B, L,
                              accumulate=True)
            yield
            return b_sq(dsq)
        return out4, bwd

    def _up_conv(self, l, x):
        wkey, bkey = "conv_layer%d.0.weight" % l, "conv_layer%d.0.bias" % l
        if not (self.phase_up_conv and x.shape[-1] == 32 and self.shapes[wkey][0] == 32):
            up = ops.upsample2(x)
            out, b = self.conv_act(up, wkey, bkey, 3, 1, RELU)
            if not self.need_grad:
                return out, None
            return out, (lambda d, masked=False: ops.upsample2_bwd(b(d, masked=masked)))
        wf, wd, b4 = ops.pack_phase_weights(self.p[wkey], self.p[bkey], self.dtype)
        out = ops.conv_up2_fwd(x, wf, b4, act=RELU)
        if not self.need_grad:
            return out, None

        def bwd(dout, masked=False):
            dy = dout if masked else ops.act_bwd(dout, out, RELU)
            ops.conv_up2_wgrad(x, dy, self.g[wkey], accumulate=True, use_tr=self.use_tr)
            ops.colsum(dy.view(-1, 32), self.g[bkey], accumulate=True)
            return ops.conv_up2_dgrad(dy, wd, 32)
        return out, bwd

    def _unet(self, x1, x2):
        B = x1.shape[0]
        s2, b_stem = self.stem(x1, x2, 2)
        self._pack_join()
        p4, arg4 = ops.maxpool(s2, want_arg=True)
        s4, b_l1 = self.res_layer(p4, 1, 1, 2)
        s8, b_l2 = self.res_layer(s4, 2, 2, 2)
        p16, arg16 = ops.maxpool(s8, want_arg=True)
        s16, b_l3 = self.res_layer(p16, 3, 1, 2)
        level = self._xbd_level if self.cfg["kind"] == "xbd" else self._level
        if self.need_grad:
            self._zpool = [torch.zeros(3 * 3 * B * self.cfg["token_len"] * DIM, dtype=torch.float32, device=s4.device), 0]
        ew = self.cfg["kind"] != "xbd"
        (o5, b5), (t4, b4), (t3, b3) = self._run_staged([level(5, s16, B), level(4, s8, B), level(3, s4, B)], ew=ew)
        self._zpool = None
        o5u = ops.upsample2(o5)
        o4, bu4 = self._up_conv(4, ops.add(t4, o5u))
        o3, bu3 = self._up_conv(3, ops.add(t3, o4))
        _, h2, w2, c2 = s2.shape
        k20 = "conv_layer2_0.0.weight"
        split2 = self.split_cat and self.training and self.pk[k20].fwd_frag is not None and \
            (not self.need_grad or self.pk[k20].dgrad_frag is not None) and \
            ops.conv3x3_split_supported(B, h2, w2, 2 * c2, self.shapes[k20][0], self.dtype)
        cat2 = ops.SplitCat(s2) if split2 else ops.SplitCat(s2).materialize()
        y, b20 = self.conv_bn(cat2, k20, "conv_layer2_0.1", 3, 1, 1, 1, True, lazy=True)
        y2 = ops.conv2d(y, self.pk["conv_layer2_0.3.weight"].fwd, 32, 3, 1, 1, bias=self.p["conv_layer2_0.3.bias"],
                        residual=o3)
        o2, bu2 = self._up_conv(2, y2)
        logits, b_out = self._head_out(o2, "classifier.weight", "classifier.bias")
        if not self.need_grad:
            return logits, None

        def bwd_first(dl):
            do2 = b_out(dl, relu_out=o2)
            dy2 = bu2(do2, masked=True)
            ops.conv2d_wgrad(y, dy2, self.g["conv_layer2_0.3.weight"], 3, 1, 1, accumulate=True, use_tr=self.use_tr)
            ops.colsum(dy2.view(-1, 32), self.g["conv_layer2_0.3.bias"], accumulate=True)
            dy = self.conv_dgrad(dy2, "conv_layer2_0.3.weight", 3, 1, 1, y.shape, gate=b20.gate)
            dcat2, _ = b20(dy)
            if split2:
                ds2 = dcat2
            else:
                ds2 = ops.split_halves(dcat2)
            dsum3 = bu3(dy2)
            dsum4 = bu4(dsum3)
            ds4, ds8, ds16 = self._run_staged([b3(dsum3), b4(dsum4), b5(ops.upsample2_bwd(dsum4))], ew=ew)
            return ds16, ds8, ds4, ds2

        def bwd_second(state):
            ds16, ds8, ds4, ds2 = state
            dp16 = b_l3(ds16)
            ds8 = ops.add(ds8, ops.maxpool_bwd(arg16, dp16, s8.shape))
            ds4 = ops.add(ds4, b_l2(ds8))
            dp4 = b_l1(ds4)
            if hasattr(b_stem, "from_pool") and os.environ.get("DAHITRA_NO_FUSED_STEM_BWD_UNET", "0") != "1":
                b_stem.from_pool(arg4, dp4, extra=ds2)
            else:
                b_stem(ops.add(ds2, ops.maxpool_bwd(arg4, dp4, s2.shape)))

        def bwd(dl):
            bwd_second(bwd_first(dl))
        bwd.split = (bwd_first, bwd_second, ("resnet.",))
        return logits, bwd
```

dahitra_amd/graph.py:

```python
import os

import torch
import torch.distributed as dist

from . import ops, parallel
from .models import losses


class GraphedTrainStep:
    CHECK_EVERY = 64

    def __init__(self, net, opt, a, b, lab, warmup=3, confusion=None):
        if not getattr(opt, "capturable", False):
            raise ValueError("GraphedTrainStep needs dahitra_amd.optim.AdamW(..., capturable=True)")
        self.net, self.opt = net, opt
        self.confusion = confusion
        self.world = dist.get_world_size() if dist.is_initialized() else 1
        self.exchange = parallel.exchange_enabled()
        self.split_off = None
        self.persist_bn_launches = None
        self._set_inputs(a, b, lab)
        net._ensure_arena(a.device)
        flat0 = net._arena.flat.clone()
        bufs0 = [t.clone() for t in net.buffers()]
        conf0 = confusion.clone() if confusion is not None else None
        opt0 = opt.snapshot_flat_state(net)
        s = torch.cuda.Stream()
        s.wait_stream(torch.cuda.current_stream())
        split = self.exchange and self._can_split()
        with torch.cuda.stream(s):
            for _ in range(warmup):
                if split:
                    self._split_first()
                    self._second()
                    self._update()
                else:
                    self._body(include_opt=True)
        torch.cuda.current_stream().wait_stream(s)
        torch.cuda.synchronize()
        net._arena.flat.copy_(flat0)
        for t, t0 in zip(net.buffers(), bufs0):
            t.copy_(t0)
        opt.restore_flat_state(net, opt0)
        if confusion is not None:
            confusion.copy_(conf0)
        cs = self._capture_stream = torch.cuda.Stream()
        ops.rekey_workspace(a.device, s, cs)
        self.graph = torch.cuda.CUDAGraph()
        if split:
            self.graph2 = torch.cuda.CUDAGraph()
            n0 = ops.BN_PERSIST_LAUNCHES
            with torch.cuda.graph(self.graph, stream=cs):
                self.loss = self._split_first()
            n1 = ops.BN_PERSIST_LAUNCHES
            with torch.cuda.graph(self.graph2, pool=self.graph.pool(), stream=cs):
                self._second()
            self.persist_bn_launches = (n1 - n0, ops.BN_PERSIST_LAUNCHES - n1)
            if self.persist_bn_launches[1] and os.environ.get("DAHITRA_OVERLAP_PERSIST_BN") != "1":
                raise RuntimeError("dahitra_amd: %d persistent BatchNorm launches were recorded into the graph that overlaps the "
                                   "gradient all-reduce" % self.persist_bn_launches[1])
        else:
            self.split_off = None
            with torch.cuda.graph(self.graph, stream=cs):
                self.loss = self._body(include_opt=not self.exchange)
        self._pinned = ops.pin_captured_buffers(net)
        self._generation = net._arena.generation
        self._calls = 0
        torch.cuda.synchronize()
        ops.bn_persist_check(a.device)

    def _set_inputs(self, a, b, lab):
        self.a, self.b, self.lab = a.clone(), b.clone(), lab.clone()

    def _copy_inputs(self, a, b, lab):
        self.a.copy_(a, non_blocking=True)
        self.b.copy_(b, non_blocking=True)
        self.lab.copy_(lab, non_blocking=True)

    def _eager_body(self, include_opt):
        logits = self.net(self.a, self.b)
        self.logits = logits.detach()
        self.opt.zero_grad()
        loss = losses.focal_loss(logits, self.lab)
        loss.backward()
        self._count(self.logits)
        if include_opt:
            self.opt.step()
        return loss.detach()

    def _body(self, include_opt):
        if type(self)._eager_body is not GraphedTrainStep._eager_body or os.environ.get("DAHITRA_GRAPH_AUTOGRAD") == "1":
            return self._eager_body(include_opt)
        net = self.net
        logits = self._forward_split()
        bwd = net._engine.take_backward()
        self.logits = logits
        loss, dl = self._loss_and_grad(logits)
        self._count(logits)
        net._arena.grad.zero_()
        net._engine.backward(dl, bwd)
        net._bind_grad_views()
        if include_opt:
            self.opt.step()
        return loss

    def _forward_split(self):
        return self.net._run_forward(self.a, self.b, need_grad=True)

    def _loss_and_grad(self, logits):
        tgt = self.lab[:, 0] if self.lab.dim() == logits.dim() else self.lab
        return ops.focal_loss(logits, tgt.to(torch.int64).contiguous(), want_grad=True)

    def _count(self, logits):
        if self.confusion is not None:
            tgt = self.lab[:, 0] if self.lab.dim() == logits.dim() else self.lab
            ops.confusion_matrix(logits, tgt.to(torch.int64).contiguous(), self.confusion)

    def _can_split(self):
        self.split_off = parallel.split_offset(self.net, self.world)
        return self.split_off is not None

    def _split_first(self):
        net = self.net
        logits = self._forward_split()
        bwd = net._engine.take_backward()
        self.logits = logits
        loss, dl = self._loss_and_grad(logits)
        self._count(logits)
        net._arena.grad.zero_()
        net._engine.backward_first(dl, bwd)
        net._bind_grad_views()
        return loss

    def _second(self):
        if os.environ.get("DAHITRA_OVERLAP_PERSIST_BN") == "1":
            self.net._engine.backward_second()
            return
        with ops.no_persist_bn():
            self.net._engine.backward_second()

    def _after_replay(self):
        parallel.allreduce_net_grads_(self.net)
        self._update()

    def _replay_overlapped(self):
        _, grad = self.net.flat_params()
        self.graph.replay()
        w1 = dist.all_reduce(grad[self.split_off:], op=dist.ReduceOp.SUM, async_op=True)
        self.graph2.replay()
        w2 = dist.all_reduce(grad[:self.split_off], op=dist.ReduceOp.SUM, async_op=True)
        w1.wait()
        w2.wait()
        self._update()

    def _update(self):
        self.opt.step()

    def __call__(self, *inputs):
        if self.net._arena.generation != self._generation:
            raise RuntimeError("dahitra_amd: the net's parameter arena was rebuilt (moved to another device / "
                               "parameters replaced) after this step was captured; build a new GraphedTrainStep")
        if inputs and inputs[0] is not None:
            self._copy_inputs(*inputs)
        self._calls += 1
        if self._calls in (2, 8) or self._calls % self.CHECK_EVERY == 0:
            ops.bn_persist_check(self.a.device)
        self.opt.sync_hyper(1.0 / self.world)
        if self.split_off is not None:
            self._replay_overlapped()
            return self.loss
        self.graph.replay()
        if self.exchange:
            self._after_replay()
        return self.loss


class GraphedEvalStep:

    def __init__(self, net, a, b, lab=None, confusion=None, warmup=2):
        self.net, self.confusion = net, confusion
        net.eval()
        self.a, self.b = a.clone(), b.clone()
        self.lab = lab.clone() if lab is not None else None
        if confusion is not None and lab is None:
            raise ValueError("GraphedEvalStep: a confusion matrix needs the labels")
        net._ensure_arena(a.device)
        conf0 = confusion.clone() if confusion is not None else None
        s = torch.cuda.Stream()
        s.wait_stream(torch.cuda.current_stream())
        with torch.cuda.stream(s):
            for _ in range(warmup):
                self._body()
        torch.cuda.current_stream().wait_stream(s)
        torch.cuda.synchronize()
        if confusion is not None:
            confusion.copy_(conf0)
        cs = self._capture_stream = torch.cuda.Stream()
        ops.rekey_workspace(a.device, s, cs)
        self.graph = torch.cuda.CUDAGraph()
        with torch.cuda.graph(self.graph, stream=cs):
            self.logits = self._body()
        self._pinned = ops.pin_captured_buffers(net)
        self._generation = net._arena.generation
        torch.cuda.synchronize()

    def _body(self):
        with torch.no_grad():
            logits = self.net(self.a, self.b)
        if self.confusion is not None:
            tgt = self.lab[:, 0] if self.lab.dim() == logits.dim() else self.lab
            ops.confusion_matrix(logits.detach().float().contiguous(), tgt.to(torch.int64).contiguous(), self.confusion)
        return logits

    def __call__(self, a=None, b=None, lab=None):
        if self.net._arena.generation != self._generation:
            raise RuntimeError("dahitra_amd: the net's parameter arena was rebuilt after this evaluation step was captured; "
                               "build a new GraphedEvalStep")
        if self.net.training:
            raise RuntimeError("dahitra_amd: GraphedEvalStep replays the eval-mode forward; call net.eval() (a train-mode forward "
                               "in between re-packs the weights for training)")
        if a is not None:
            self.a.copy_(a, non_blocking=True)
# ... 59 lines not shown
```

dahitra_amd/ops.py:

```python
import ctypes
import os
import sys

import torch

from . import _lib

ACT_NONE, ACT_RELU, ACT_GELU = 0, 1, 2
_DT = {torch.float32: 0, torch.bfloat16: 1}
_vp = ctypes.c_void_p
_ci = ctypes.c_int
_cl = ctypes.c_long
_cf = ctypes.c_float
_cd = ctypes.c_double


def dt(t):
    try:
        return _DT[t.dtype]
    except KeyError:
        raise TypeError("dahitra_amd: unsupported activation dtype %s" % t.dtype)


def set_f32_mma_mode(mode):
# ... 29 lines not shown
    assert t.is_cuda and t.is_contiguous(), "dahitra_amd ops need contiguous device tensors"
    return _vp(t.data_ptr())


def S():
    return _vp(torch.cuda.current_stream().cuda_stream)


_ws = {}


def workspace(nbytes, device):
    key = (str(device), torch.cuda.current_stream(device).cuda_stream) if torch.device(device).type == "cuda" else str(device)
    buf = _ws.get(key)
    if buf is None or buf.numel() < nbytes:
        buf = torch.empty(max(int(nbytes), 1 << 20), dtype=torch.uint8, device=device)
        _ws[key] = buf
    return buf


def rekey_workspace(device, old_stream, new_stream):
    buf = _ws.pop((str(device), old_stream.cuda_stream), None)
    if buf is not None:
        cur = _ws.get((str(device), new_stream.cuda_stream))
        if cur is None or cur.numel() < buf.numel():
            _ws[(str(device), new_stream.cuda_stream)] = buf


_PINNED = []


def pin_captured_buffers(net):
    keep = list(_ws.values())
    eng = net._engine
    if eng._wgrad_plan is not None:
        keep += list(eng._wgrad_plan.slots) + list(eng._wgrad_plan.tables.values())
    for pack, _, xstack, wstack in eng._plans.values():
        keep += [pack.table] + list(pack.keep) + list(xstack.values())
        for fwd_stack, dgrad_stack in wstack.values():
            keep += [fwd_stack, dgrad_stack]
    keep += [net._arena.flat, net._arena.grad]
    keep = [t for t in keep if t is not None]
    _PINNED.extend(keep)
    return keep


def _call(name, *args):
    L = _lib.lib()
    _lib.check(getattr(L, name)(*args), name)


def cdiv(a, b):
    return (a + b - 1) // b


def pad16(c):
    return cdiv(c, 16) * 16


def pack_weight(w, dtype, want_dgrad=True, dgrad_inner=0, out_scale=None, want_fwd=True, out_dgrad=None):
    if w.dim() == 2:
        O, I = w.shape
        ks = 1
    else:
        O, I, ks, _ = w.shape
    OPad, IPad = pad16(O), pad16(I)
    OK = max(O, dgrad_inner)
    fwd = torch.empty(ks * ks, OPad, I, dtype=dtype, device=w.device) if want_fwd else None
    if out_dgrad is not None:
        assert out_dgrad.numel() == ks * ks * IPad * OK and out_dgrad.dtype == dtype
        dg = out_dgrad
    else:
        dg = torch.empty(ks * ks, IPad, OK, dtype=dtype, device=w.device) if want_dgrad else None
    _call("dh_pack_weight", _ci(_DT[dtype]), P(w), P(out_scale), _ci(O), _ci(I), _ci(ks), _ci(OPad), P(fwd), _ci(IPad), _ci(OK),
          P(dg), S())
    return fwd, dg


class PackPlan:

    class _Job(ctypes.Structure):
        _fields_ = [("w", ctypes.c_void_p), ("fwd", ctypes.c_void_p), ("dgrad", ctypes.c_void_p), ("O", ctypes.c_int),
                    ("I", ctypes.c_int), ("KS", ctypes.c_int), ("OPad", ctypes.c_int), ("IPad", ctypes.c_int),
                    ("OK", ctypes.c_int), ("dtype", ctypes.c_int), ("first_block", ctypes.c_int), ("nblocks", ctypes.c_int)]

    def __init__(self, device):
        self.device, self.jobs, self.blocks, self.table, self.keep = device, [], 0, None, []

    def add(self, w, dtype, want_fwd=True, want_dgrad=True, dgrad_inner=0, out_dgrad=None, frag=False, out_fwd=None):
        if w.dim() == 2:
            (O, I), ks = w.shape, 1
        else:
            O, I, ks, _ = w.shape
        OPad, IPad, OK = pad16(O), pad16(I), max(O, dgrad_inner)
        ck = chunk_channels(dtype)
        if frag:
            assert ks == 3 and dtype == torch.bfloat16 and I % 32 == 0 and OK % 32 == 0 and out_dgrad is None
            fwd = torch.empty(OPad // 16, I // 32, ks * ks, 64, 8, dtype=dtype, device=w.device) if want_fwd else None
            dg = torch.empty(IPad // 16, OK // 32, ks * ks, 64, 8, dtype=dtype, device=w.device) if want_dgrad else None
        else:
            fwd = out_fwd if out_fwd is not None else \
                (torch.empty(ks * ks, OPad, I, dtype=dtype, device=w.device) if want_fwd else None)
            dg = out_dgrad if out_dgrad is not None else \
                (torch.empty(ks * ks, IPad, OK, dtype=dtype, device=w.device) if want_dgrad else None)
        n = max(fwd.numel() if fwd is not None else 0, dg.numel() if dg is not None else 0)
        assert n < 2 ** 31 and w.numel() < 2 ** 31, "pack_weights_multi indexes a layer with 32-bit arithmetic"
        nb = max(1, min(256, cdiv(n, 2048)))
        if ks == 3 and O % 32 == 0 and I % 32 == 0 and OK == O:
            nb = min(256, (O // 32) * (I // 32))
        self.jobs.append(self._Job(w.data_ptr(), fwd.data_ptr() if fwd is not None else None,
                                   dg.data_ptr() if dg is not None else None, O, I, ks, OPad, IPad, OK,
                                   _DT[dtype] | (0x200 if frag else 0), self.blocks, nb))
        self.blocks += nb
        self.keep += [w, fwd, dg]
        return fwd, dg

    def run(self):
        if not self.jobs:
            return
        if self.table is None:
            assert ctypes.sizeof(self._Job) == _lib.lib().dh_pack_job_size()
            raw = b"".join(bytes(j) for j in self.jobs)
            self.table = torch.frombuffer(bytearray(raw), dtype=torch.uint8).to(self.device)
        _call("dh_pack_weights_multi", P(self.table), _ci(len(self.jobs)), _ci(self.blocks), S())


class WgradPlan:

    class _Job(ctypes.Structure):
        _fields_ = [("part", ctypes.c_void_p), ("dw", ctypes.c_void_p), ("splitk", ctypes.c_int), ("taps", ctypes.c_int),
                    ("Oslab", ctypes.c_int), ("O", ctypes.c_int), ("I", ctypes.c_int), ("accumulate", ctypes.c_int),
                    ("first_block", ctypes.c_int), ("nblocks", ctypes.c_int)]

    def __init__(self, device, batch=False):
        self.device, self.slots, self.cur, self.blocks = device, [], 0, 0
        self.tables, self.sigs, self.phase = {}, {}, 0
        self._prev = None
        self.post = []
        self.batch = batch and os.environ.get("DAHITRA_WGRAD_BATCH", "1") != "0"
        self.batching, self.keep = False, []

    def __enter__(self):
        global _WGRAD_PLAN
        self._prev, _WGRAD_PLAN = _WGRAD_PLAN, self
        self.cur = 0
        self.jobs = []
        self.post = []
        self.blocks = 0
        self.phase = 0
        self.keep = []
        self.batching = self.batch and PROFILE is None
        if self.batching:
            _call("dh_wgrad_batch_begin")
        elif self._prev is None:
            _call("dh_wgrad_batch_abort")
        return self

    def __exit__(self, *exc):
        global _WGRAD_PLAN
        _WGRAD_PLAN = self._prev
        if self.batching:
            self.batching = False
            if exc and exc[0] is not None:
                _lib.lib().dh_wgrad_batch_abort()
            else:
                _call("dh_wgrad_batch_end", S())
            self.keep = []
        return False

    def hold(self, *tensors):
        if self.batching:
            self.keep += [t for t in tensors if t is not None]

    def slab(self, nbytes):
        if self.cur == len(self.slots):
            self.slots.append(torch.empty(max(int(nbytes), 16), dtype=torch.uint8, device=self.device))
        elif self.slots[self.cur].numel() < nbytes:
            _PINNED.append(self.slots[self.cur])
            self.slots[self.cur] = torch.empty(int(nbytes), dtype=torch.uint8, device=self.device)
            self.tables = {}
        buf = self.slots[self.cur]
        self.cur += 1
        return buf

    def add(self, part, dw, splitk, taps, oslab, o, i, accumulate):
        nb = cdiv(o * i * taps, _lib.lib().dh_wgrad_reduce_outputs_per_block(i))
        self.jobs.append(self._Job(part.data_ptr(), dw.data_ptr(), splitk, taps, oslab, o, i, int(accumulate),
                                   self.blocks, nb))
        self.blocks += nb

    def run(self):
        if self.batching:
            _call("dh_wgrad_batch_launch", S())
            self.keep = []
        if self.jobs:
            self._run_reduce()
        for fn in self.post:
            fn()
        self.jobs, self.post, self.blocks = [], [], 0
        self.phase += 1

    def _run_reduce(self):
        sig = b"".join(bytes(j) for j in self.jobs)
        if self.tables.get(self.phase) is None or sig != self.sigs.get(self.phase):
            if torch.cuda.is_current_stream_capturing():
                raise RuntimeError("dahitra_amd: the weight-gradient plan changed during graph capture; run one eager "
                                   "step of the same shapes first")
            assert ctypes.sizeof(self._Job) == _lib.lib().dh_wgrad_reduce_job_size()
            if self.tables.get(self.phase) is not None:
                _PINNED.append(self.tables[self.phase])
            self.tables[self.phase] = torch.frombuffer(bytearray(sig), dtype=torch.uint8).to(self.device)
            self.sigs[self.phase] = sig
        _call("dh_wgrad_reduce_multi", P(self.tables[self.phase]), _ci(len(self.jobs)), _ci(self.blocks), S())


_WGRAD_PLAN = None


class SideStream:

    def __init__(self, device):
        self.stream, self.keep, self.active, self._ctx = torch.cuda.Stream(device=device), [], False, None

    def fork(self, *tensors):
        global _PERSIST_BLOCK
        self.stream.wait_stream(torch.cuda.current_stream())
        self.keep += [t for t in tensors if t is not None]
        if not self.active:
            _PERSIST_BLOCK += 1
        self.active = True
        return self

    def __enter__(self):
        self._ctx = torch.cuda.stream(self.stream)
        self._ctx.__enter__()
        return self

    def __exit__(self, *exc):
        self._ctx.__exit__(*exc)
        self._ctx = None
        return False

    def join(self):
        global _PERSIST_BLOCK
        if self.active:
            torch.cuda.current_stream().wait_stream(self.stream)
            self.keep, self.active = [], False
            _PERSIST_BLOCK -= 1


PROFILE = None
REPLAY = None


class _Prof:
    __slots__ = ("ev",)

    def __init__(self, key, flops, nbytes):
        self.ev = None
        if PROFILE is not None:
            self.ev = (torch.cuda.Event(enable_timing=True), torch.cuda.Event(enable_timing=True))
            PROFILE.setdefault(key, []).append((self.ev, float(flops), float(nbytes)))

    def __enter__(self):
        if self.ev is not None:
            self.ev[0].record()

    def __exit__(self, *exc):
        if self.ev is not None:
            self.ev[1].record()
        return False


def _nb(*tensors):
    return sum(t.numel() * t.element_size() for t in tensors if t is not None)


def _bn_in_args(b):
    if b is None:
        return _vp(0), _vp(0), _ci(0)
    return P(b.scale), P(b.shift), _ci(b.groups)

# ... 190 lines not shown
          _cl(w_image_stride), P(pre), _ci(1), *_gate_args(None), *_bn_in_args(None), _ci(0), _vp(0), S())
    assert images == 1 or rpi % 16 == 0
    return (y, pre) if want_preact else y


def conv2d_wgrad(x, dy, dw, ks, stride, pad, accumulate=False, groups=1, use_tr=True, cout_real=0, cin=0, dilation=1,
                 defer=True):
    if isinstance(x, BnInput):
        return _conv2d_wgrad_bn_in(x, dy, dw, ks, stride, pad, accumulate, use_tr, cout_real, dilation, defer)
    if isinstance(x, SplitCat):
        return _conv2d_wgrad_split(x, dy, dw, ks, stride, pad, accumulate, defer)
    if isinstance(x, Up4Input):
        x = x.materialize()
    N, H, W, pitch = x.shape
    Cin = cin if cin else pitch
    _, OH, OW, Cout = dy.shape
    L = _lib.lib()
    nbytes = L.dh_conv2d_wgrad_workspace_size(N, OH, OW, Cin, Cout, ks, groups)
    plan = _WGRAD_PLAN
    if plan is not None and groups == 1 and defer:
        ws = plan.slab(nbytes)
        sk = ctypes.c_int(0)
        with _Prof("conv_wgrad<%s,ks%d,s%d>" % ("bf16" if x.dtype == torch.bfloat16 else "f32", ks, stride),
                   2.0 * N * OH * OW * Cout * Cin * ks * ks, _nb(x, dy)):
            _call("dh_conv2d_wgrad_partial", _ci(dt(x)), P(x), P(dy), P(dw), _ci(int(accumulate)), _ci(N), _ci(H), _ci(W),
                  _ci(Cin), _ci(OH), _ci(OW), _ci(Cout), _ci(ks), _ci(stride), _ci(pad), _ci(1), _ci(0), _ci(int(use_tr)),
                  _ci(cout_real), _ci(pitch), _ci(dilation), P(ws), ctypes.byref(sk), S())
        plan.hold(x, dy)
        if sk.value > 0:
            plan.add(ws, dw, sk.value, ks * ks, Cout, cout_real if cout_real else Cout, Cin, accumulate)
        return
    ws = workspace(nbytes, x.device)
    _call("dh_conv2d_wgrad", _ci(dt(x)), P(x), P(dy), P(dw), _ci(int(accumulate)), _ci(N), _ci(H), _ci(W), _ci(Cin),
          _ci(OH), _ci(OW), _ci(Cout), _ci(ks), _ci(stride), _ci(pad), _ci(groups), _ci(0), _ci(int(use_tr)),
          _ci(cout_real), _ci(pitch), _ci(dilation), P(ws), S())


def _conv2d_wgrad_split(xs, dy, dw, ks, stride, pad, accumulate, defer):
    assert ks == 3 and stride == 1 and pad == 1
    N, H, W, Cin = xs.shape
    Cout = dy.shape[-1]
    nbytes = _lib.lib().dh_conv2d_wgrad_workspace_size(N, H, W, Cin, Cout, 3, 1)
    plan, own = (_WGRAD_PLAN if defer else None), False
    if plan is None:
        plan, own = WgradPlan(dy.device), True
        plan.__enter__()
    try:
        ws = plan.slab(nbytes)
        sk = ctypes.c_int(0)
        with _Prof("conv_wgrad<bf16,ks3,s1>", 2.0 * N * H * W * Cout * Cin * 9, _nb(xs.t, dy)):
            _call("dh_conv2d_wgrad_split", P(xs.t), _cl(xs.split_bytes), P(dy), P(dw), _ci(int(accumulate)), _ci(N), _ci(H), _ci(W),
                  _ci(Cin), _ci(Cout), P(ws), ctypes.byref(sk), S())
        plan.hold(xs.t, dy)
        plan.add(ws, dw, sk.value, 9, Cout, Cout, Cin, accumulate)
        if own:
            plan.run()
    finally:
        if own:
            plan.__exit__(*sys.exc_info())


def _conv2d_wgrad_bn_in(b, dy, dw, ks, stride, pad, accumulate, use_tr, cout_real, dilation, defer):
    x = b.y
    N, H, W, Cin = x.shape
    _, OH, OW, Cout = dy.shape
    nbytes = _lib.lib().dh_conv2d_wgrad_workspace_size(N, OH, OW, Cin, Cout, ks, 1)
    plan = _WGRAD_PLAN if defer else None
    ws = plan.slab(nbytes) if plan is not None else workspace(nbytes, x.device)
    sk = ctypes.c_int(0)
    with _Prof("conv_wgrad<%s,ks%d,s%d>" % ("bf16" if x.dtype == torch.bfloat16 else "f32", ks, stride),
               2.0 * N * OH * OW * Cout * Cin * ks * ks, _nb(x, dy)):
        _call("dh_conv2d_wgrad_bn_in", _ci(dt(x)), P(x), P(dy), P(dw), _ci(int(accumulate)), _ci(N), _ci(H), _ci(W), _ci(Cin),
              _ci(OH), _ci(OW), _ci(Cout), _ci(ks), _ci(stride), _ci(pad), _ci(int(use_tr)), _ci(cout_real), _ci(dilation),
              P(b.scale), P(b.shift), _ci(b.groups), P(ws), ctypes.byref(sk) if plan is not None else None, S())
    if plan is not None:
        plan.hold(x, dy, b.scale, b.shift)
    if plan is not None and sk.value > 0:
        plan.add(ws, dw, sk.value, ks * ks, Cout, cout_real if cout_real else Cout, Cin, accumulate)


def pack_phase_weights(w, bias, dtype):
    O, I = w.shape[0], w.shape[1]
    assert O == 32 and tuple(w.shape[2:]) == (3, 3)
    fwd = torch.empty(4, 128, I, dtype=dtype, device=w.device)
    dg = torch.empty(4, I, 128, dtype=dtype, device=w.device)
    b4 = torch.empty(128, dtype=torch.float32, device=w.device)
    _call("dh_pack_phase_weights", _ci(_DT[dtype]), P(w), P(bias), _ci(I), P(fwd), P(dg), P(b4), S())
    return fwd, dg, b4


def conv_up2_fwd(x, wfwd, bias4, act=ACT_NONE):
    N, H, W, Cin = x.shape
    y = torch.empty(N, 2 * H, 2 * W, 32, dtype=x.dtype, device=x.device)
    key = "conv_phase<%s,up2_fwd>" % ("bf16" if x.dtype == torch.bfloat16 else "f32")
    with _Prof(key, 2.0 * N * 4 * H * W * 32 * Cin * 9, _nb(x, y, wfwd)):
        _call("dh_conv2d_fwd", _ci(dt(x)), P(x), P(wfwd), P(y), P(bias4), _vp(0), _vp(0), _ci(N), _ci(H), _ci(W), _ci(Cin),
              _ci(H), _ci(W), _ci(128), _ci(128), _ci(2), _ci(1), _ci(1), _ci(act), _ci(0), _cl(0), _vp(0), _ci(1),
              *_gate_args(None), *_bn_in_args(None), _ci(1), _vp(0), S())
    return y


def pack_s2_dgrad_phase_weights(w, dtype):
    Co, Ci = w.shape[0], w.shape[1]
    out = torch.empty(4, 4 * Ci, Co, dtype=dtype, device=w.device)
    _call("dh_pack_s2_dgrad_phase_weights", _ci(_DT[dtype]), P(w), _ci(Co), _ci(Ci), P(out), S())
    return out


def conv3x3s2_dgrad(dy, wphase, cin, coarse_residual=None, alg_flops=0):
    N, OH, OW, Co = dy.shape
    dx = torch.empty(N, 2 * OH, 2 * OW, cin, dtype=dy.dtype, device=dy.device)
    key = "conv_phase<%s,s2_dgrad>" % ("bf16" if dy.dtype == torch.bfloat16 else "f32")
    with _Prof(key, alg_flops if alg_flops else 2.0 * N * OH * OW * Co * cin * 9, _nb(dy, dx, wphase, coarse_residual)):
        _call("dh_conv2d_fwd", _ci(dt(dy)), P(dy), P(wphase), P(dx), _vp(0), P(coarse_residual), _vp(0), _ci(N), _ci(OH),
              _ci(OW), _ci(Co), _ci(OH), _ci(OW), _ci(4 * cin), _ci(4 * cin), _ci(2), _ci(1), _ci(1), _ci(ACT_NONE), _ci(0),
              _cl(0), _vp(0), _ci(1), *_gate_args(None), *_bn_in_args(None), _ci(1), _vp(0), S())
    return dx


def conv_up2_dgrad(dy, wdgrad, cin):
    N, H2, W2, C = dy.shape
    assert C == 32 and H2 % 2 == 0 and W2 % 2 == 0 and (cin % 64 == 0 or cin == 32)
    H, W = H2 // 2, W2 // 2
    dx = torch.empty(N, H, W, cin, dtype=dy.dtype, device=dy.device)
    key = "conv_phase<%s,up2_dgrad>" % ("bf16" if dy.dtype == torch.bfloat16 else "f32")
    with _Prof(key, 2.0 * N * H2 * W2 * 32 * cin * 9, _nb(dy, dx, wdgrad)):
        _call("dh_conv2d_fwd", _ci(dt(dy)), P(dy), P(wdgrad), P(dx), _vp(0), _vp(0), _vp(0), _ci(N), _ci(H), _ci(W), _ci(128),
              _ci(H), _ci(W), _ci(cin), _ci(cin), _ci(2), _ci(1), _ci(1), _ci(ACT_NONE), _ci(0), _cl(0), _vp(0), _ci(1),
              *_gate_args(None), *_bn_in_args(None), _ci(2), _vp(0), S())
    return dx


def conv_up2_wgrad(x, dy, dw, accumulate=True, use_tr=True):
    N, H, W, Cin = x.shape
    L = _lib.lib()
    plan, own = _WGRAD_PLAN, False
    if plan is None:
        plan, own = WgradPlan(x.device), True
        plan.__enter__()
    try:
        ws = plan.slab(L.dh_conv2d_wgrad_phase_workspace_size(N, H, W, Cin))
        dwab = plan.slab(4 * 32 * Cin * 4 * 4).view(torch.float32)
        sk = ctypes.c_int(0)
        with _Prof("conv_wgrad<%s,ks3,s1>" % ("bf16" if x.dtype == torch.bfloat16 else "f32"),
                   2.0 * N * 4 * H * W * 32 * Cin * 9, _nb(x, dy)):
            _call("dh_conv2d_wgrad_phase", _ci(dt(x)), P(x), P(dy), _ci(N), _ci(H), _ci(W), _ci(Cin), _ci(int(use_tr)), P(ws),
                  ctypes.byref(sk), S())
        per = sk.value * 4 * 32 * Cin * 4
        for ph in range(4):
            plan.add(ws[ph * per:], dwab[ph * 32 * Cin * 4:], sk.value, 4, 32, 32, Cin, False)
        plan.post.append(lambda: _call("dh_phase_wgrad_combine", P(dwab), P(dw), _ci(Cin), _ci(int(accumulate)), S()))
        if own:
            plan.run()
    finally:
        if own:
            plan.__exit__()


def linear_wgrad(x2d, dy2d, dw, accumulate=False, images=1, per_image=False, use_tr=True):
    rows, Cin = x2d.shape
    Cout = dy2d.shape[1]
    rpi = rows // images
    Hh = cdiv(rpi, 16)
    groups = images if per_image else 1
    L = _lib.lib()
    nbytes = L.dh_conv2d_wgrad_workspace_size(images, Hh, 16, Cin, Cout, 1, groups)
    ws = workspace(nbytes, x2d.device)
    assert images == 1 or rpi % 16 == 0
    _call("dh_conv2d_wgrad", _ci(dt(x2d)), P(x2d), P(dy2d), P(dw), _ci(int(accumulate)), _ci(images), _ci(Hh), _ci(16),
          _ci(Cin), _ci(Hh), _ci(16), _ci(Cout), _ci(1), _ci(1), _ci(0), _ci(groups), _ci(rpi), _ci(int(use_tr)),
          _ci(0), _ci(0), _ci(1), P(ws), S())


def add_coarse_(x, coarse):
    N, H, W, C = x.shape
    n2, OH, OW, c2 = coarse.shape
    assert n2 == N and c2 == C and x.dtype == coarse.dtype and x.is_contiguous() and coarse.is_contiguous()
    _call("dh_add_coarse", _ci(dt(x)), P(x), P(coarse), _ci(N), _ci(OH), _ci(OW), _ci(H), _ci(W), _ci(C), S())
    return x


def zero_insert2(dy, H, W):
    N, OH, OW, C = dy.shape
    z = torch.empty(N, H, W, C, dtype=dy.dtype, device=dy.device)
    _call("dh_zero_insert2", _ci(dt(dy)), P(dy), P(z), _ci(N), _ci(OH), _ci(OW), _ci(H), _ci(W), _ci(C), S())
    return z


def stem_space_to_depth(x_nchw, dtype):
    N, C, H, W = x_nchw.shape
    assert C == 3
    cp = chunk_channels(dtype)
    y = torch.empty(N, H // 2, W // 2, cp, dtype=dtype, device=x_nchw.device)
    _call("dh_stem_space_to_depth", _ci(_DT[dtype]), P(x_nchw), P(y), _ci(N), _ci(H), _ci(W), _ci(cp), S())
    return y


def stem_pack_weight(w, dtype, out_scale=None):
    O = w.shape[0]
    cp = chunk_channels(dtype)
    out = torch.empty(16, O, cp, dtype=dtype, device=w.device)
    _call("dh_stem_pack_weight", _ci(_DT[dtype]), P(w), P(out_scale), P(out), _ci(O), _ci(cp), S())
    return out


def stem7_fwd(x1, x2, w, out_scale=None, bias=None, relu=False, want_stats=False, want_xs=False, groups=1):
    B, C, H, W = x1.shape
    assert C == 3 and x1.dtype == torch.float32 and x1.is_contiguous() and (x2 is None or (x2.shape == x1.shape and x2.is_contiguous()))
    N = B if x2 is None else 2 * B
    y = torch.empty(N, H // 2, W // 2, 64, dtype=torch.bfloat16, device=x1.device)
    nt = _lib.lib().dh_stem7_fwd_num_slots(N, H, W, groups)
    stats = torch.empty(2, 64, nt, dtype=torch.float32, device=x1.device) if want_stats else None
    xs = torch.empty(N, H // 2, W // 2, 16, dtype=torch.bfloat16, device=x1.device) if want_xs else None
    with _Prof("stem7_fwd", 2.0 * N * (H // 2) * (W // 2) * 64 * 147, _nb(x1, x2, y, xs)):
        _call("dh_stem7_fwd", P(x1), P(x2), _ci(B), _ci(N), _ci(H), _ci(W), P(w), P(out_scale), P(bias), _ci(int(relu)), P(y),
              P(stats), _ci(groups), P(xs), S())
    return y, stats, xs


def stem_pool_bn_bwd(arg, dpool, y, scale, shift, mean, invstd, gamma, dgamma, dbeta, groups, accumulate=True, extra=None):
    N, H, W, C = y.shape
    d = torch.empty_like(y)
    coef = torch.empty(groups, 3, C, dtype=torch.float32, device=y.device)
    L = _lib.lib()
    ws = workspace(L.dh_stem_pool_bn_bwd_workspace_size(C, groups), y.device)
    assert extra is None or (extra.shape == y.shape and extra.dtype == y.dtype)
    with _Prof("bn_bwd", 0, _nb(arg, dpool, y, d, extra)):
        _call("dh_stem_pool_bn_bwd_plus", P(arg), P(dpool), P(extra), P(y), P(scale), P(shift), P(mean), P(invstd), P(gamma), _ci(N), _ci(H),
              _ci(W), _ci(C), _ci(groups), P(d), P(coef), P(dgamma), P(dbeta), _ci(int(accumulate)), P(ws), S())
    return d, coef


def stem_wgrad(x_s2d, dy, dw, accumulate=False, use_tr=True, bn=None):
    N, H2, W2, cp = x_s2d.shape
    O = dy.shape[-1]
    dw2 = torch.empty(O, 16, 4, 4, dtype=torch.float32, device=dy.device)
    if bn is not None:
        y, coef, groups = bn
        assert cp == 16 and O == 64 and y.shape == dy.shape
        L = _lib.lib()
        ws = workspace(L.dh_conv2d_wgrad_workspace_size(N, H2, W2, 16, O, 4, 1), dy.device)
        with _Prof("conv_wgrad<bf16,ks4,s1>", 2.0 * N * H2 * W2 * O * 16 * 16, _nb(x_s2d, dy, y)):
            _call("dh_stem_wgrad_bn", P(x_s2d), P(dy), P(y), P(coef), _ci(groups), _ci(N), _ci(H2), _ci(W2), P(dw2),
                  _ci(int(use_tr)), P(ws), S())
    else:
        conv2d_wgrad(x_s2d, dy, dw2, ks=4, stride=1, pad=2, use_tr=use_tr, cin=16, defer=False)
    _call("dh_stem_unpack_grad", P(dw2), P(dw), _ci(O), _ci(16), _ci(int(accumulate)), S())


def bn_finalize(stats, C, groups, count, gamma, beta, running_mean, running_var, momentum=0.1, eps=1e-5, nbt=None):
    _, cp, nt = stats.shape
    dev = stats.device
    mean = torch.empty(groups, C, dtype=torch.float32, device=dev)
    invstd, scale, shift = torch.empty_like(mean), torch.empty_like(mean), torch.empty_like(mean)
    _call("dh_bn_finalize", P(stats), _ci(nt), _ci(cp), _ci(C), _ci(groups), _cd(float(count)), P(gamma), P(beta),
          P(running_mean), P(running_var), _cf(momentum), _cf(eps), P(mean), P(invstd), P(scale), P(shift), P(nbt), S())
    return mean, invstd, scale, shift


def bn_eval_params(gamma, beta, rm, rv, eps=1e-5):
    C = gamma.numel()
    scale = torch.empty(1, C, dtype=torch.float32, device=gamma.device)
    shift = torch.empty_like(scale)
    _call("dh_bn_eval_params", P(gamma), P(beta), P(rm), P(rv), _cf(eps), _ci(C), P(scale), P(shift), S())
    return scale, shift


RELU_BITS = os.environ.get("DAHITRA_NO_RELU_BITS", "0") != "1"


def bn_apply(x, scale, shift, groups=1, act=ACT_NONE, residual=None, want_bits=False):
    C = x.shape[-1]
    npix = x.numel() // C
    y = torch.empty_like(x)
    bits = None
    v = 8 if x.dtype == torch.bfloat16 else 4
    if want_bits and RELU_BITS and act == ACT_RELU and C % v == 0:
        bits = torch.empty(x.numel() // v, dtype=torch.uint8, device=x.device)
    with _Prof("bn_apply", 0, _nb(x, residual, y)):
        if bits is not None:
            _call("dh_bn_apply_bits", _ci(dt(x)), P(x), P(residual), P(y), P(scale), P(shift), _cl(npix), _ci(C), _ci(groups),
                  _ci(act), P(bits), S())
        else:
            _call("dh_bn_apply", _ci(dt(x)), P(x), P(residual), P(y), P(scale), P(shift), _cl(npix), _ci(C), _ci(groups),
                  _ci(act), S())
    return (y, bits) if want_bits else y


_BN_SYNC = {}
BN_BWD_PERSIST = os.environ.get("DAHITRA_NO_PERSIST_BN", "0") != "1"
if os.environ.get("DAHITRA_PERSIST_BN_FORCE", "0") == "1":
    BN_BWD_PERSIST = "force"
_PERSIST_BLOCK = 0
BN_PERSIST_LAUNCHES = 0


class no_persist_bn:

    def __enter__(self):
        global _PERSIST_BLOCK
        _PERSIST_BLOCK += 1

    def __exit__(self, *exc):
        global _PERSIST_BLOCK
        _PERSIST_BLOCK -= 1
        return False


def bn_sync_words(device):
    key = (str(device), torch.cuda.current_stream(device).cuda_stream)
    t = _BN_SYNC.get(key)
    if t is None:
        t = _BN_SYNC[key] = torch.zeros(8192, dtype=torch.int32, device=device)
    return t


def bn_persist_check(device=None):
    bad = []
    for (dev, stream), t in list(_BN_SYNC.items()):
        if device is not None and dev != str(device):
            continue
        word = _lib.lib().dh_bn_bwd_persist_status(P(t), _vp(torch.cuda.current_stream(t.device).cuda_stream))
        if word:
            bad.append((dev, stream, word))
    if bad:
        raise _lib.HipLibraryError(
            "dahitra_amd: the persistent BatchNorm backward failed (device, stream, word): %s -- bit 0: its device-wide "
            "barrier timed out (another stream's kernel kept workgroups out: set DAHITRA_NO_PERSIST_BN=1 or keep such "
            "launches inside ops.no_persist_bn()), bit 1: non-finite gradient sums; the gradients of that step are NaN" % bad)


def bn_bwd(dout, out_relu, x, mean, invstd, gamma, dgamma, dbeta, groups=1, accumulate=False, want_dres=False,
           mask_scale=None, mask_shift=None, bits=None):
    C = x.shape[-1]
    npix = x.numel() // C
    dx = torch.empty_like(x)
    dres = torch.empty_like(x) if want_dres else None
    L = _lib.lib()
    ws = workspace(L.dh_bn_bwd_workspace_size(_cl(npix), C, groups), x.device)
    if BN_BWD_PERSIST and not _PERSIST_BLOCK and \
            (L.dh_bn_bwd_persist_preferred if BN_BWD_PERSIST is True else L.dh_bn_bwd_persist_supported)(
            _ci(dt(x)), _cl(npix), C, groups):
        global BN_PERSIST_LAUNCHES
        BN_PERSIST_LAUNCHES += 1
        with _Prof("bn_bwd", 0, _nb(dout, bits if bits is not None else out_relu, x) + _nb(dx, dres)):
            if bits is not None:
                _call("dh_bn_bwd_persist_bits", P(dout), P(bits), P(x), P(mean), P(invstd), P(gamma), _cl(npix), _ci(C),
                      _ci(groups), P(dx), P(dres), P(dgamma), P(dbeta), _ci(int(accumulate)), P(ws), P(bn_sync_words(x.device)), S())
            else:
                _call("dh_bn_bwd_persist", P(dout), P(out_relu), P(x), P(mean), P(invstd), P(gamma), _cl(npix), _ci(C),
                      _ci(groups), P(dx), P(dres), P(dgamma), P(dbeta), _ci(int(accumulate)), P(mask_scale), P(mask_shift),
                      P(ws), P(bn_sync_words(x.device)), S())
        return (dx, dres) if want_dres else dx
    with _Prof("bn_bwd", 0, 2 * _nb(dout, bits if bits is not None else out_relu, x) + _nb(dx, dres)):
        if bits is not None:
            _call("dh_bn_bwd_bits", _ci(dt(x)), P(dout), P(bits), P(x), P(mean), P(invstd), P(gamma), _cl(npix), _ci(C),
                  _ci(groups), P(dx), P(dres), P(dgamma), P(dbeta), _ci(int(accumulate)), P(ws), S())
        else:
            _call("dh_bn_bwd", _ci(dt(x)), P(dout), P(out_relu), P(x), P(mean), P(invstd), P(gamma), _cl(npix), _ci(C),
                  _ci(groups), P(dx), P(dres), P(dgamma), P(dbeta), _ci(int(accumulate)), P(mask_scale), P(mask_shift), P(ws), S())
    return (dx, dres) if want_dres else dx


def bn_bwd_from_partials(g, x, partial, mean, invstd, gamma, dgamma, dbeta, groups=1, accumulate=False):
    C = x.shape[-1]
    npix = x.numel() // C
    _, cp, nt = partial.shape
    assert cp == C and g.shape == x.shape
    dx = torch.empty_like(x)
    ws = workspace(groups * 2 * C * 4, x.device)
    _call("dh_bn_bwd_from_partials", _ci(dt(x)), P(g), P(x), P(partial), _ci(nt), P(mean), P(invstd), P(gamma), _cl(npix),
          _ci(C), _ci(groups), P(dx), P(dgamma), P(dbeta), _ci(int(accumulate)), P(ws), S())
    return dx


def layernorm(x2d, gamma, beta, eps=1e-5, want_stats=True):
    rows, C = x2d.shape
    y = torch.empty_like(x2d)
    stats = torch.empty(rows, 2, dtype=torch.float32, device=x2d.device) if want_stats else None
    _call("dh_layernorm_fwd", _ci(dt(x2d)), P(x2d), P(gamma), P(beta), P(y), P(stats), _cl(rows), _ci(C), _cf(eps), S())
    return (y, stats) if want_stats else y


def layernorm_bwd(dy, x2d, stats, gamma, dgamma, dbeta, dx_add=None, accumulate=False):
    rows, C = x2d.shape
    dx = torch.empty_like(x2d)
    L = _lib.lib()
    ws = workspace(L.dh_layernorm_bwd_workspace_size(_cl(rows)), x2d.device)
    _call("dh_layernorm_bwd", _ci(dt(x2d)), P(dy), P(x2d), P(stats), P(gamma), P(dx), P(dx_add), P(dgamma), P(dbeta),
          _ci(int(accumulate)), _cl(rows), _ci(C), P(ws), S())
    return dx


def nchw_to_nhwc(x, dtype, cpad=0):
    N, C, H, W = x.shape
    cp = max(C, cpad)
    y = torch.empty(N, H, W, cp, dtype=dtype, device=x.device)
# ... 150 lines not shown

def add_pos_bwd(dy, dpos, accumulate=False):
    N, H, W, C = dy.shape
    assert dy.is_contiguous() and dpos.is_contiguous()
    if dy.dtype == torch.bfloat16 and C == 32 and _ew_record(EW_ADD_POS_BWD, dy, None, dpos, N, int(accumulate), H * W):
        return
    _call("dh_add_pos_bwd", _ci(dt(dy)), P(dy), P(dpos), _ci(N), _cl(H * W), _ci(C), _ci(int(accumulate)), S())


def act_bwd(dy, ref, act):
    dx = torch.empty_like(dy)
    _call("dh_act_bwd", _ci(dt(dy)), P(dy), P(ref), P(dx), _cl(dy.numel()), _ci(act), S())
    return dx


def maxpool(x, want_arg=False, bn=None):
    N, H, W, C = x.shape
    y = torch.empty(N, (H - 1) // 2 + 1, (W - 1) // 2 + 1, C, dtype=x.dtype, device=x.device)
    arg = torch.empty(y.shape, dtype=torch.uint8, device=x.device) if want_arg else None
    sc, sh, groups = bn if bn is not None else (None, None, 0)
    _call("dh_maxpool3x3s2_fwd", _ci(dt(x)), P(x), P(y), P(arg), _ci(N), _ci(H), _ci(W), _ci(C), P(sc), P(sh), _ci(groups),
          S())
    return (y, arg) if want_arg else y


def maxpool_bwd(arg, dy, in_shape):
    N, H, W, C = in_shape
    dx = torch.empty(N, H, W, C, dtype=dy.dtype, device=dy.device)
    _call("dh_maxpool3x3s2_bwd", _ci(dt(dy)), P(arg), P(dy), P(dx), _ci(N), _ci(H), _ci(W), _ci(C), S())
    return dx


def upsample2(x):
    N, H, W, C = x.shape
    y = torch.empty(N, 2 * H, 2 * W, C, dtype=x.dtype, device=x.device)
    _call("dh_upsample2_nearest_fwd", _ci(dt(x)), P(x), P(y), _ci(N), _ci(H), _ci(W), _ci(C), S())
    return y


def upsample2_bwd(dy):
    N, H2, W2, C = dy.shape
    dx = torch.empty(N, H2 // 2, W2 // 2, C, dtype=dy.dtype, device=dy.device)
    _call("dh_upsample2_nearest_bwd", _ci(dt(dy)), P(dy), P(dx), _ci(N), _ci(H2 // 2), _ci(W2 // 2), _ci(C), S())
    return dx


def absdiff_upsample4(a, b):
    N, H, W, C = a.shape
    y = torch.empty(N, 4 * H, 4 * W, C, dtype=a.dtype, device=a.device)
    _call("dh_absdiff_upsample4_fwd", _ci(dt(a)), P(a), P(b), P(y), _ci(N), _ci(H), _ci(W), _ci(C), S())
    return y


def absdiff_upsample4_bwd(a, b, dy):
    N, H, W, C = a.shape
    da, db = torch.empty_like(a), torch.empty_like(b)
    _call("dh_absdiff_upsample4_bwd", _ci(dt(a)), P(a), P(b), P(dy), P(da), P(db), _ci(N), _ci(H), _ci(W), _ci(C), S())
    return da, db


def conv3x3_dgrad_through_up4(dy, wdgrad, a, b, da=None, db=None):
    N, H, W, C = a.shape
    assert C == 32 and a.dtype == torch.bfloat16 and dy.shape[:3] == (N, 4 * H, 4 * W) and wdgrad.shape[-2] == 32
    L = _lib.lib()
    partial = torch.empty(L.dh_conv3x3_dgrad_up4_partial_floats(N, 4 * H, 4 * W), dtype=torch.float32, device=a.device)
    with _Prof("conv_mfma<bf16,ks3,s1,nt32>", 2.0 * N * 16 * H * W * 32 * dy.shape[-1] * 9, _nb(dy, wdgrad, partial)):
        _call("dh_conv3x3_dgrad_up4", _ci(dt(dy)), P(dy), P(wdgrad), _ci(N), _ci(4 * H), _ci(4 * W), _ci(dy.shape[-1]), P(partial), S())
    da = torch.empty_like(a) if da is None else da
    db = torch.empty_like(b) if db is None else db
    _call("dh_absdiff_up4_combine", P(partial), P(a), P(b), P(da), P(db), _ci(N), _ci(H), _ci(W), S())
    return da, db


def absdiff(a, b):
    y = torch.empty_like(a)
    _call("dh_absdiff", _ci(dt(a)), P(a), P(b), P(y), _cl(a.numel()), S())
    return y


def absdiff_bwd(a, b, dy, da, db, accumulate=True):
    _call("dh_absdiff_bwd", _ci(dt(a)), P(a), P(b), P(dy), P(da), P(db), _cl(a.numel()), _ci(int(accumulate)), S())


def colsum(x2d, out, accumulate=False):
    C = x2d.shape[-1]
    Pn = x2d.numel() // C
    ws = workspace(1024 * C * 4 + 1024, x2d.device)
    _call("dh_colsum", _ci(dt(x2d)), P(x2d), _cl(Pn), _ci(C), P(out), _ci(int(accumulate)), P(ws), S())


def cast_from_f32(src, dtype):
    dst = torch.empty(src.shape, dtype=dtype, device=src.device)
    _call("dh_cast_from_f32", _ci(_DT[dtype]), P(src), P(dst), _cl(src.numel()), S())
    return dst


def cast_to_f32(src, dst=None, accumulate=False):
    if dst is None:
        dst = torch.empty(src.shape, dtype=torch.float32, device=src.device)
    _call("dh_cast_to_f32", _ci(dt(src)), P(src), P(dst), _cl(src.numel()), _ci(int(accumulate)), S())
    return dst


def tokenizer_fwd(x, wa, pos, B, L):
    Sn, H, W, C = x.shape
    HW = H * W
    dev = x.device
    logits = torch.empty(Sn * HW, L, dtype=torch.float32, device=dev)
    stats = torch.empty(Sn, L, 2, dtype=torch.float32, device=dev)
    pooled = torch.empty(Sn, L, 32, dtype=torch.float32, device=dev)
    tok = torch.empty(B, 2 * L, 32, dtype=torch.float32, device=dev)
    nws = _lib.lib().dh_tokenizer_fwd_workspace_size(Sn, HW, L)
    args = lambda ws: (_ci(dt(x)), P(x), P(wa), P(pos), _ci(Sn), _ci(B), _ci(HW), _ci(L), P(logits), P(stats), P(pooled),
                       P(tok), P(ws), S())
    if _XPREP_BATCH is not None and _ENC_BATCH is not None:
        ws = torch.empty(max(int(nws), 1), dtype=torch.uint8, device=dev)
        _XPREP_BATCH.extend((ws, x, pos))
        _call("dh_tokenizer_fwd", *args(ws))
    else:
        with _XprepPaused():
            _call("dh_tokenizer_fwd", *args(workspace(nws, dev)))
    return tok, (logits, stats, pooled)


def flush_recorded_tokens():
    if _XPREP_BATCH is not None:
        _call("dh_xprep_batch_launch_fwd", S())


def tokenizer_bwd(x, wa, saved, dtok_cat, dx_accum, dwa, dpos, B, L, accumulate=False):
    Sn, H, W, C = x.shape
    HW = H * W
    logits, stats, pooled = saved
    Lb = _lib.lib()
    nws = Lb.dh_tokenizer_bwd_workspace_size(Sn, HW, L)
    if _XPREP_BATCH is not None:
        ws = torch.empty(max(int(nws), 1), dtype=torch.uint8, device=x.device)
        _XPREP_BATCH.extend((ws, dtok_cat, dx_accum, dpos))
    else:
        ws = workspace(nws, x.device)
    assert dtok_cat.dtype == torch.float32
    _call("dh_tokenizer_bwd", _ci(dt(x)), P(x), P(wa), _ci(Sn), _ci(B), _ci(HW), _ci(L), P(logits), P(stats), P(pooled),
          P(dtok_cat), P(dx_accum), P(dwa), P(dpos), _ci(int(accumulate)), P(ws), S())


def prep_mfma_supported(dtype, Sn, L, heads, dim_head, HLP):
    return bool(_lib.lib().dh_xattn_prep_mfma_supported(_ci(_DT[dtype]), _ci(Sn), _ci(L), _ci(heads), _ci(dim_head), _ci(HLP)))


DEC_RECORD = None


def _dec_recorded(kind, rows_of, depth_of, mlp_of):
    import functools

    def deco(fn):
        @functools.wraps(fn)
        def wrapped(*a, **k):
            if DEC_RECORD is not None:
                DEC_RECORD.append(dict(kind=kind, rows=rows_of(a), depth=depth_of(a), mlp=mlp_of(a, k),
                                       call=functools.partial(fn, *a, **k)))
            return fn(*a, **k)
        return wrapped
    return deco


class XattnPrep:

    def __init__(self, tok, bstride, sstride, B, Sn, L, heads, dim_head, ln_g, ln_b, wq, wkT, wvT, woT, dtype,
# ... 481 lines not shown
```

include/dahitra_hip.h:

```cpp
#ifndef DAHITRA_HIP_H
#define DAHITRA_HIP_H
#ifdef __cplusplus
extern "C" {
#endif

#define DH_F32 0
#define DH_BF16 1
#define DH_ACT_NONE 0
#define DH_ACT_RELU 1
#define DH_ACT_GELU 2

int dh_abi_version(void);
const char* dh_last_error(void);
void dh_set_error(const char* msg);

int dh_conv2d_fwd(int dtype, const void* x, const void* w_packed, void* y, const float* bias,
                  const void* residual, float* stats_partial, int N, int H, int W, int Cin, int OH, int OW,
                  int Cout, int CoutPad, int ks, int stride, int pad, int act, int npix_valid,
                  long w_image_stride, void* y_preact, int dilation, const void* gate_out, const void* gate_y,
                  const float* gate_mean, const float* gate_invstd, int gate_groups, const float* in_scale,
                  const float* in_shift, int in_groups, int phase_mode, const void* w_frag, void* stream);
int dh_conv2d_fwd_num_tiles(int dtype, int N, int OH, int OW, int Cin, int ks, int stride);
int dh_conv_wreg_mode(int mode);
int dh_set_f32_mma_mode(int mode);
int dh_get_f32_mma_mode(void);
long dh_conv3x3_dgrad_up4_partial_floats(int N, int H, int W);
int dh_conv3x3_dgrad_up4(int dtype, const void* dy, const void* w_packed, int N, int H, int W, int K, float* partial, void* stream);
int dh_absdiff_up4_combine(const float* partial, const void* a, const void* b, void* da, void* db, int N, int H, int W, void* stream);
int dh_conv3x3_head_fwd(int dtype, const void* x, const void* w_packed, const float* bias, int N, int H, int W, int Cin,
                        int Cout, const float* in_scale, const float* in_shift, int in_groups, float* logits_nchw, void* stream);

int dh_conv2d_wgrad(int dtype, const void* x, const void* dy, float* dw_oihw, int accumulate, int N, int H,
                    int W, int Cin, int OH, int OW, int Cout, int ks, int stride, int pad, int groups,
                    int npix_valid, int use_tr, int Cout_real, int cin_pitch, int dilation, void* workspace, void* stream);
int dh_conv2d_wgrad_1x1_blocks(int N, int H, int W, int Cin, int Cout);
long dh_conv2d_wgrad_workspace_size(int N, int OH, int OW, int Cin, int Cout, int ks, int groups);
int dh_conv2d_wgrad_partial(int dtype, const void* x, const void* dy, float* dw_oihw, int accumulate, int N, int H,
                            int W, int Cin, int OH, int OW, int Cout, int ks, int stride, int pad, int groups,
                            int npix_valid, int use_tr, int Cout_real, int cin_pitch, int dilation, void* workspace,
                            int* splitk_out, void* stream);
int dh_conv2d_wgrad_bn_in(int dtype, const void* x, const void* dy, float* dw_oihw, int accumulate, int N, int H, int W,
                          int Cin, int OH, int OW, int Cout, int ks, int stride, int pad, int use_tr, int Cout_real,
                          int dilation, const float* in_scale, const float* in_shift, int in_groups, void* workspace,
                          int* splitk_out, void* stream);
int dh_conv3x3_split_supported(int N, int H, int W, int Cin, int Cout);
int dh_conv3x3_split_fwd(const void* x, long x_split_bytes, const void* w_packed, const void* w_frag, void* y, long y_split_bytes,
                         float* stats_partial, int N, int H, int W, int Cin, int Cout, void* stream);
int dh_conv2d_wgrad_split(const void* x, long x_split_bytes, const void* dy, float* dw_oihw, int accumulate, int N, int H, int W,
                          int Cin, int Cout, void* workspace, int* splitk_out, void* stream);
int dh_conv3x3_up4_fwd(const void* a, const void* b, const void* w_packed, const float* bias, int act, void* y, float* stats_partial,
                       int N, int H, int W, void* stream);
int dh_wgrad_batch_begin(void);
int dh_wgrad_batch_pending(void);
int dh_wgrad_batch_launch(void* stream);
int dh_wgrad_batch_end(void* stream);
int dh_wgrad_batch_abort(void);
int dh_wgrad_reduce_multi(const void* jobs_dev, int njobs, int total_blocks, void* stream);
int dh_pack_phase_weights(int dtype, const float* w_oihw, const float* bias, int Cin, void* fwd, void* dgrad, float* bias4,
                          void* stream);
long dh_conv2d_wgrad_phase_workspace_size(int N, int H, int W, int Cin);
int dh_conv2d_wgrad_phase(int dtype, const void* x, const void* dy, int N, int H, int W, int Cin, int use_tr, void* workspace,
                          int* splitk_out, void* stream);
int dh_phase_wgrad_combine(const float* dwab, float* dw_oihw, int Cin, int accumulate, void* stream);
int dh_pack_s2_dgrad_phase_weights(int dtype, const float* w_oihw, int Co, int Ci, void* out, void* stream);
int dh_wgrad_reduce_job_size(void);
int dh_wgrad_reduce_outputs_per_block(int Cin);
int dh_conv2d_wgrad_splitk(int N, int OH, int OW, int Cin, int Cout, int ks, int groups);

int dh_pack_weight(int dtype, const float* w_oihw, const float* out_scale, int O, int I, int ks, int OPad, void* fwd, int IPad,
                   int dgrad_inner, void* dgrad, void* stream);
int dh_pack_weights_multi(const void* jobs_dev, int njobs, int total_blocks, void* stream);
int dh_pack_job_size(void);
int dh_zero_insert2(int dtype, const void* dy, void* z, int N, int OH, int OW, int H, int W, int C, void* stream);
int dh_add_coarse(int dtype, void* x, const void* coarse, int N, int OH, int OW, int H, int W, int C, void* stream);

int dh_stem_space_to_depth(int dtype, const float* x_nchw, void* y, int N, int H, int W, int CP, void* stream);
int dh_stem_pack_weight(int dtype, const float* w_oihw, const float* out_scale, void* packed, int O, int CP, void* stream);
int dh_stem_unpack_grad(const float* dw2, float* dw_oihw, int O, int CP, int accumulate, void* stream);
int dh_stem7_fwd(const float* xa, const float* xb, int B, int N, int H, int W, const float* w_oihw, const float* out_scale,
                 const float* bias, int relu, void* y, float* stats, int groups, void* xs16, void* stream);
int dh_stem7_fwd_num_slots(int N, int H, int W, int groups);
long dh_stem_pool_bn_bwd_workspace_size(int C, int groups);
int dh_stem_pool_bn_bwd(const unsigned char* argmax, const void* dpool, const void* y, const float* mask_scale,
                        const float* mask_shift, const float* mean, const float* invstd, const float* gamma, int N, int H, int W,
                        int C, int groups, void* d, float* coef, float* dgamma, float* dbeta, int accumulate, void* workspace,
                        void* stream);
int dh_stem_pool_bn_bwd_plus(const unsigned char* argmax, const void* dpool, const void* extra, const void* y,
                             const float* mask_scale, const float* mask_shift, const float* mean, const float* invstd,
                             const float* gamma, int N, int H, int W, int C, int groups, void* d, float* coef, float* dgamma,
                             float* dbeta, int accumulate, void* workspace, void* stream);
int dh_stem_wgrad_bn(const void* xs16, const void* d, const void* y, const float* coef, int groups, int N, int OH, int OW,
                     float* dw2, int use_tr, void* workspace, void* stream);

int dh_bn_finalize(const float* partial, int ntiles, int CP, int C, int groups, double count, const float* gamma,
                   const float* beta, float* running_mean, float* running_var, float momentum, float eps,
                   float* mean, float* invstd, float* scale, float* shift, long long* num_batches_tracked,
                   void* stream);
int dh_bn_eval_params(const float* gamma, const float* beta, const float* running_mean, const float* running_var,
                      float eps, int C, float* scale, float* shift, void* stream);
int dh_bn_apply(int dtype, const void* x, const void* residual, void* y, const float* scale, const float* shift,
                long npix, int C, int groups, int act, void* stream);
int dh_bn_bwd(int dtype, const void* dout, const void* out_relu, const void* x, const float* mean,
              const float* invstd, const float* gamma, long npix, int C, int groups, void* dx, void* dres,
              float* dgamma, float* dbeta, int accumulate, const float* mask_scale, const float* mask_shift,
              void* workspace, void* stream);
long dh_bn_bwd_workspace_size(long npix, int C, int groups);
int dh_bn_bwd_persist_supported(int dtype, long npix, int C, int groups);
int dh_bn_bwd_persist_preferred(int dtype, long npix, int C, int groups);
int dh_bn_bwd_persist(const void* dout, const void* out_relu, const void* x, const float* mean, const float* invstd,
                      const float* gamma, long npix, int C, int groups, void* dx, void* dres, float* dgamma, float* dbeta,
                      int accumulate, const float* mask_scale, const float* mask_shift, void* workspace, unsigned* sync,
                      void* stream);
int dh_bn_apply_bits(int dtype, const void* x, const void* residual, void* y, const float* scale, const float* shift, long npix,
                     int C, int groups, int act, unsigned char* relu_bits, void* stream);
int dh_bn_bwd_bits(int dtype, const void* dout, const unsigned char* relu_bits, const void* x, const float* mean, const float* invstd,
                   const float* gamma, long npix, int C, int groups, void* dx, void* dres, float* dgamma, float* dbeta, int accumulate,
                   void* workspace, void* stream);
int dh_bn_bwd_persist_bits(const void* dout, const unsigned char* relu_bits, const void* x, const float* mean, const float* invstd,
                           const float* gamma, long npix, int C, int groups, void* dx, void* dres, float* dgamma, float* dbeta,
                           int accumulate, void* workspace, unsigned* sync, void* stream);
int dh_bn_bwd_persist_status(unsigned* sync, void* stream);
int dh_bn_bwd_persist_test_spin_limit(unsigned limit);
int dh_bn_bwd_from_partials(int dtype, const void* g, const void* x, const float* partial, int ntiles, const float* mean,
                            const float* invstd, const float* gamma, long npix, int C, int groups, void* dx,
                            float* dgamma, float* dbeta, int accumulate, void* workspace, void* stream);
int dh_layernorm_fwd(int dtype, const void* x, const float* gamma, const float* beta, void* y, float* stats,
                     long rows, int C, float eps, void* stream);
int dh_layernorm_bwd(int dtype, const void* dy, const void* x, const float* stats, const float* gamma, void* dx,
                     const void* dx_add, float* dgamma, float* dbeta, int accumulate, long rows, int C,
                     void* workspace, void* stream);
long dh_layernorm_bwd_workspace_size(long rows);
int dh_reduce_partials(const float* partial, long nt, long n, float scale, float* out, int accumulate, void* stream);

int dh_augment_pairs_u8(const unsigned char* a, const unsigned char* b, const unsigned char* l, const int* idx,
                        const int* params, int N, int H, int W, int h, int w, float* out_a, float* out_b,
                        unsigned char* out_l, void* stream);
int dh_nchw_to_nhwc(int dtype, const float* src, void* dst, int N, int C, long HW, int CP, void* stream);
int dh_head_dgrad3x3(int dtype, const void* dy, int CP, const float* w_oihw, int NC, void* dx, int N, int H, int W,
                     void* stream);
int dh_head_dgrad3x3_relu(const void* dy, const float* w_oihw, int NC, const void* relu_out, void* dx, int N, int H, int W,
                          void* stream);
int dh_head_dgrad3x3_bn_blocks(int N, int H, int W, int groups);
int dh_head_dgrad3x3_bn(const void* dy, const float* w_oihw, int NC, const void* y, const float* mask_scale, const float* mask_shift,
                        const float* mean, const float* invstd, int groups, void* g, float* partial, int N, int H, int W,
                        void* stream);
int dh_head_bn_bwd_blocks(int N, int H, int W, int groups);
long dh_head_bn_bwd_workspace_size(int N, int H, int W, int groups);
int dh_head_dlogits_pack(int dtype, const float* dlogits_nchw, int N, int NC, int H, int W, void* dlp, void* stream);
int dh_head_bn_bwd(int dtype, const void* dlp, const float* w_oihw, int NC, const void* y, const float* mask_scale, const float* mask_shift,
                   const float* mean, const float* invstd, const float* gamma, int groups, void* dx, float* dgamma, float* dbeta,
                   float* dw, float* db, int accumulate, int N, int H, int W, void* workspace, void* stream);
int dh_head_relu_bwd(int dtype, const void* dlp, const float* w_oihw, int NC, const void* relu_out, void* dx, float* dw, float* db,
                     int accumulate, int N, int H, int W, void* workspace, void* stream);
int dh_head_fwd_supported(int NC, int W);
int dh_head_fwd(int dtype, const void* x, const float* w_oihw, const float* bias, int NC, const float* in_scale, const float* in_shift,
                int in_groups, float* logits_nchw, int N, int H, int W, void* stream);
enum { DH_EW_ADD_POS = 1, DH_EW_CAT_HALVES = 2, DH_EW_SPLIT_HALVES = 3, DH_EW_ABSDIFF_HALVES = 4, DH_EW_ABSDIFF_HALVES_BWD = 5,
       DH_EW_ADD_POS_BWD = 6 };
int dh_ew_multi(int n, const int* op, const void* const* a, const void* const* b, void* const* c, const int* i0, const int* i1,
                const long* l0, void* stream);
int dh_nhwc_to_nchw(int dtype, const void* src, float* dst, int N, int C, long HW, void* stream);
int dh_copy_channels(int dtype, const void* src, int Cs, int sc0, void* dst, int Cd, int dc0, int Cn, long P, void* stream);
int dh_cat_halves(int dtype, void* t, void* cat, int C, long P, int inverse, void* stream);
int dh_add(int dtype, const void* a, const void* b, void* y, long n, void* stream);
int dh_add_pos(int dtype, const void* x, const float* pos, void* y, int N, long HW, int C, void* stream);
int dh_add_pos_bwd(int dtype, const void* dy, float* dpos, int N, long HW, int C, int accumulate, void* stream);
int dh_act_bwd(int dtype, const void* dy, const void* ref, void* dx, long n, int act, void* stream);
int dh_maxpool3x3s2_fwd(int dtype, const void* x, void* y, unsigned char* argmax, int N, int H, int W, int C,
                        const float* bn_scale, const float* bn_shift, int groups, void* stream);
int dh_maxpool3x3s2_bwd(int dtype, const unsigned char* argmax, const void* dy, void* dx, int N, int H, int W, int C, void* stream);
int dh_upsample2_nearest_fwd(int dtype, const void* x, void* y, int N, int H, int W, int C, void* stream);
int dh_upsample2_nearest_bwd(int dtype, const void* dy, void* dx, int N, int H, int W, int C, void* stream);
int dh_absdiff_upsample4_fwd(int dtype, const void* a, const void* b, void* y, int N, int H, int W, int C, void* stream);
int dh_absdiff_upsample4_bwd(int dtype, const void* a, const void* b, const void* dy, void* da, void* db, int N, int H, int W, int C, void* stream);
int dh_absdiff(int dtype, const void* a, const void* b, void* y, long n, void* stream);
int dh_absdiff_bwd(int dtype, const void* a, const void* b, const void* dy, void* da, void* db, long n, int accumulate, void* stream);
int dh_colsum(int dtype, const void* x, long P, int C, float* out, int accumulate, void* workspace, void* stream);
int dh_cast_from_f32(int dtype, const float* src, void* dst, long n, void* stream);
int dh_cast_to_f32(int dtype, const void* src, float* dst, long n, int accumulate, void* stream);

int dh_tokenizer_fwd(int dtype, const void* x, const float* wa, const float* pos, int S, int B, int HW, int L,
                     float* logits, float* stats, float* pooled, float* tok_cat, void* workspace, void* stream);
long dh_tokenizer_fwd_workspace_size(int S, int HW, int L);
int dh_tokenizer_bwd(int dtype, const void* x, const float* wa, int S, int B, int HW, int L, const float* logits,
                     const float* stats, const float* pooled, const float* dtok_cat, void* dx_accum, float* dwa,
                     float* dpos, int accumulate, void* workspace, void* stream);
long dh_tokenizer_bwd_workspace_size(int S, int HW, int L);
int dh_xattn_prep_fwd(int dtype, const void* tok, long tok_bstride, long tok_sstride, int B, int S, int L, int heads,
                      int dim_head, int HLP, float scale, float eps, const float* ln_g, const float* ln_b,
                      const float* wq, const void* wkT, const void* wvT, const void* woT, float* mn, float* mstats,
                      float* k, float* v, void* kq, void* kqT, void* vo, void* voT, void* stream);
int dh_xattn_prep_fwd_stack(int dtype, const void* tok, long tok_bstride, long tok_sstride, int B, int S, int L, int heads,
                            int dim_head, int HLP, float scale, float eps, int layers, long param_stride,
                            const float* ln_g, const float* ln_b, const float* wq, const void* wkT, const void* wvT,
                            const void* woT, float* mn, float* mstats, float* k, float* v, void* kq, void* kqT, void* vo,
                            void* voT, void* stream);
int dh_xattn_prep_mfma_supported(int dtype, int S, int L, int heads, int dim_head, int HLP);
int dh_xattn_prep_fwd_stack_mfma(const void* tok, long tok_bstride, long tok_sstride, int B, int S, int heads, int dim_head,
                                 int HLP, float scale, float eps, int layers, long param_stride, const float* ln_g,
                                 const float* ln_b, const float* wk, const float* wv, const float* wo, const void* wqT,
                                 float* mn, float* mstats, float* k, float* v, void* kq, void* kqT, void* vo, void* voT,
                                 void* stream);
int dh_xattn_prep_bwd_stack_mfma(const void* tok, void* dtok_accum, long tok_bstride, long tok_sstride, int B, int S, int heads,
                                 int dim_head, int HLP, float scale, int layers, long param_stride, const float* ln_g,
                                 const float* wq, const void* woT, const void* wkT, const void* wvT, const float* mn,
                                 const float* mstats, const float* k, const float* v, const float* dkq, const float* dvoT,
                                 float* dk, float* dv, float* dln_g, float* dln_b, float* dwq, float* dwk, float* dwv,
                                 float* dwo, int accumulate, void* workspace, void* stream);
int dh_xattn_prep_bwd_stack(int dtype, const void* tok, void* dtok_accum, long tok_bstride, long tok_sstride, int B, int S,
                            int L, int heads, int dim_head, int HLP, float scale, int layers, long param_stride,
                            const float* ln_g, const void* wqT, const float* wk, const float* wv, const float* wo,
                            const float* mn, const float* mstats, const float* k, const float* v, const float* dkq,
                            const float* dvoT, float* dk, float* dv, float* dln_g, float* dln_b, float* dwq, float* dwk,
                            float* dwv, float* dwo, int accumulate, void* workspace, void* stream);
long dh_xattn_prep_bwd_stack_workspace_size(int S, int L, int layers);
int dh_xattn_prep_bwd(int dtype, const void* tok, void* dtok_accum, long tok_bstride, long tok_sstride, int B, int S,
                      int L, int heads, int dim_head, int HLP, float scale, const float* ln_g, const void* wqT,
                      const float* wk, const float* wv, const float* wo, const float* mn, const float* mstats,
                      const float* k, const float* v, const float* dkq, const float* dvoT, float* dk, float* dv,
                      float* dln_g, float* dln_b, float* dwq, float* dwk, float* dwv, float* dwo, int accumulate,
                      void* workspace, void* stream);
long dh_xattn_prep_bwd_workspace_size(int S);
int dh_softmax_groups_fwd(int dtype, const void* x, void* y, long rows, int heads, int L, int HLP, void* stream);
int dh_softmax_groups_bwd(int dtype, const void* y, const void* dy, void* dx, long rows, int heads, int L, int HLP, void* stream);
int dh_self_attn_fwd(int dtype, const void* qkv, void* o, float* attn, int B, int n, int heads, int dim_head, float scale, void* stream);
int dh_self_attn_bwd(int dtype, const void* qkv, const float* attn, const void* dout, void* dqkv, int B, int n, int heads, int dim_head, float scale, void* stream);

int dh_encoder_supported(int n, int heads, int dim_head, int mlp);
int dh_encoder_fwd(const float* x, float* y, float* saved_inputs, int B, int n, int depth, int heads, int dim_head,
                   int mlp, float scale, float eps, long param_stride, const float* ln1_g, const float* ln1_b,
                   const float* wqkv, const float* wo, const float* bo, const float* ln2_g, const float* ln2_b,
                   const float* w1, const float* b1, const float* w2, const float* b2, void* stream);
int dh_encoder_bwd(const float* dy, float* dx, const float* saved_inputs, int B, int n, int depth, int heads,
                   int dim_head, int mlp, float scale, float eps, long param_stride, const float* ln1_g,
                   const float* ln1_b, const float* wqkv, const float* wo, const float* bo, const float* ln2_g,
                   const float* ln2_b, const float* w1, const float* b1, const float* w2, const float* b2,
                   float* dln1_g, float* dln1_b, float* dwqkv, float* dwo, float* dbo, float* dln2_g, float* dln2_b,
                   float* dw1, float* db1, float* dw2, float* db2, void* workspace, void* stream);
int dh_encoder_batch_begin(void);
int dh_encoder_batch_pending(void);
int dh_encoder_batch_launch(void* stream);
int dh_encoder_batch_end(void* stream);
int dh_encoder_batch_abort(void);
int dh_decoder_batch_begin(void);
int dh_decoder_batch_pending(void);
int dh_decoder_batch_launch(void* stream);
int dh_decoder_batch_end(void* stream);
int dh_decoder_batch_abort(void);
int dh_xprep_batch_begin(void);
int dh_xprep_batch_pending(void);
int dh_xprep_batch_pause(int paused);
int dh_xprep_batch_launch_fwd(void* stream);
int dh_xprep_batch_launch_bwd(void* stream);
int dh_xprep_batch_end(void* stream);
int dh_xprep_batch_abort(void);
long dh_encoder_bwd_workspace_size(int B, int n, int depth, int heads, int dim_head, int mlp);
long dh_encoder_saved_floats(int B, int n, int depth, int heads, int dim_head, int mlp);

int dh_decoder_layer_fwd(const void* x, void* y, const void* kq, const void* voT, const float* ln1_g,
                         const float* ln1_b, const float* bo, const float* ln2_g, const float* ln2_b, const void* w1,
// ... 65 lines not shown
```

Measured before the change: 10060 image-pairs/s.

## Fold bias colsums, stem wgrad reduce and weight packs into batched multi-job kernels

Bias-gradient colsum reductions, the stem weight-gradient reduction (with its space-to-depth to 7x7 remap) and the phase/s2-dgrad weight packing and zero-fills are now queued as jobs in the existing multi-job reduce and pack kernels instead of being launched separately. A step plan collects zeroing and packing requests so they run in one batched launch. The goal is to cut the kernel launch count and tail gaps inside the training-step graph. In exchange it adds job-dispatch branching, ordering constraints that depend on plan phases, and a fallback path when two colsums target the same output.

Measured after the change: 10120 image-pairs/s, median of 5. Within noise of the previous version (+0.6%).

```diff
diff --git a/dahitra_amd/csrc/common.h b/dahitra_amd/csrc/common.h
--- a/dahitra_amd/csrc/common.h
+++ b/dahitra_amd/csrc/common.h
@@ -222,6 +222,55 @@
     } while (0)
 static inline int dh_cdiv(long a, long b) { return (int)((a + b - 1) / b); }
 
+template <typename T>
+__device__ __forceinline__ void dh_pack_phase_weights_elem(const float* __restrict__ w, const float* __restrict__ bias, int Cin,
+                                                           T* __restrict__ fwd, T* __restrict__ dgrad, float* __restrict__ bias4,
+                                                           int i) {
+    if (i < 128 && bias4) bias4[i] = bias ? bias[i & 31] : 0.f;
+    if (i >= 32 * Cin) return;
+    const int co = i / Cin, ci = i % Cin;
+    float k[3][3];
+#pragma unroll
+    for (int j = 0; j < 9; ++j) k[j / 3][j % 3] = w[(size_t)i * 9 + j];
+    const int lo[2][2] = {{0, 1}, {0, 2}}, hi[2][2] = {{0, 2}, {1, 2}};
+#pragma unroll
+    for (int a = 0; a < 2; ++a)
+#pragma unroll
+        for (int b = 0; b < 2; ++b)
+#pragma unroll
+            for (int t = 0; t < 2; ++t)
+#pragma unroll
+                for (int u = 0; u < 2; ++u) {
+                    float s = 0.f;
+                    for (int kh = lo[a][t]; kh <= hi[a][t]; ++kh)
+                        for (int kw = lo[b][u]; kw <= hi[b][u]; ++kw) s += k[kh][kw];
+                    const int ph = a * 2 + b;
+                    if (fwd) stf(fwd + ((size_t)(t * 2 + u) * 128 + ph * 32 + co) * Cin + ci, s);
+                    if (dgrad) stf(dgrad + ((size_t)((1 - t) * 2 + (1 - u)) * Cin + ci) * 128 + ph * 32 + co, s);
+                }
+}
+template <typename T>
+__device__ __forceinline__ void dh_pack_s2_dgrad_phase_elem(const float* __restrict__ w, int Co, int Ci, T* __restrict__ out, int i) {
+    if (i >= Co * Ci) return;
+    const int co = i / Ci, ci = i % Ci;
+    float k[3][3];
+#pragma unroll
+    for (int j = 0; j < 9; ++j) k[j / 3][j % 3] = w[(size_t)i * 9 + j];
+    const int kmap[2][2] = {{-1, 1}, {2, 0}};
+#pragma unroll
+    for (int a = 0; a < 2; ++a)
+#pragma unroll
+        for (int b = 0; b < 2; ++b)
+#pragma unroll
+            for (int t = 0; t < 2; ++t)
+#pragma unroll
+                for (int u = 0; u < 2; ++u) {
+                    const int kh = kmap[a][t], kw = kmap[b][u];
+                    const float v = (kh >= 0 && kw >= 0) ? k[kh][kw] : 0.f;
+                    stf(out + ((size_t)(t * 2 + u) * 4 * Ci + (a * 2 + b) * Ci + ci) * Co + co, v);
+                }
+}
+
 __device__ __forceinline__ void dh_reduce_partials_body(const float* __restrict__ partial, long nt, long n, float scale,
                                                         float* __restrict__ out, int accumulate, int bx, double (*red)[32]) {
     const int lane = threadIdx.x & 31, ph = threadIdx.x >> 5;
diff --git a/dahitra_amd/csrc/conv_wgrad.hip b/dahitra_amd/csrc/conv_wgrad.hip
--- a/dahitra_amd/csrc/conv_wgrad.hip
+++ b/dahitra_amd/csrc/conv_wgrad.hip
@@ -513,7 +513,8 @@
 
 static inline int wgrad_reduce_epb(int I) { return (I & 3) == 0 ? 128 : 32; }
 __device__ __forceinline__ void wgrad_reduce_block(const float* __restrict__ part, int splitk, int taps, int Oslab, int O,
-                                                   int I, float* __restrict__ dw, int accumulate, long block, float (*red)[132]) {
+                                                   int I, float* __restrict__ dw, int accumulate, long block, float (*red)[132],
+                                                   int stem = 0) {
     const long n = (long)O * I * taps;
     const int lane = threadIdx.x & 31, ph = threadIdx.x >> 5;
     const bool vec = (I & 3) == 0;
@@ -564,7 +565,12 @@
 #pragma unroll
             for (int r = 0; r < 8; ++r) s += red[r][l2 * 4 + e];
             const int ci2 = (int)(i2 % I), o2 = (int)((i2 / I) % O), tap2 = (int)(i2 / ((long)I * O));
-            const size_t d = ((size_t)o2 * I + ci2) * taps + tap2;
+            size_t d = ((size_t)o2 * I + ci2) * taps + tap2;
+            if (stem) {
+                const int r = ci2 / 3, c = ci2 % 3, kh = 2 * (tap2 >> 2) + (r >> 1) - 1, kw = 2 * (tap2 & 3) + (r & 1) - 1;
+                if (ci2 >= 12 || kh < 0 || kh >= 7 || kw < 0 || kw >= 7) return;
+                d = ((size_t)(o2 * 3 + c) * 7 + kh) * 7 + kw;
+            }
             if (accumulate) dw[d] += s; else dw[d] = s;
         }
     }
@@ -576,18 +582,26 @@
     wgrad_reduce_block(part + (size_t)blockIdx.y * splitk * taps * Oslab * I, splitk, taps, Oslab, O, I,
                        dw + (size_t)blockIdx.y * n, accumulate, blockIdx.x, red);
 }
+enum { WGR_SPLITK = 0, WGR_PARTIALS = 1, WGR_STEM = 2 };
 struct WgReduceJob {
     const float* part;
     float* dw;
     int splitk, taps, Oslab, O, I, accumulate, first_block, nblocks;
+    int kind;
+    float scale;
 };
 __global__ void wgrad_reduce_multi_kernel(const WgReduceJob* __restrict__ jobs, int njobs) {
-    __shared__ float red[8][132];
+    __shared__ __attribute__((aligned(16))) float red[8][132];
     int j = 0;
     while (j + 1 < njobs && (int)blockIdx.x >= jobs[j + 1].first_block) ++j;
     const WgReduceJob job = jobs[j];
+    if (job.kind == WGR_PARTIALS) {
+        dh_reduce_partials_body(job.part, job.splitk, job.O, job.scale, job.dw, job.accumulate, (int)blockIdx.x - job.first_block,
+                                reinterpret_cast<double(*)[32]>(&red[0][0]));
+        return;
+    }
     wgrad_reduce_block(job.part, job.splitk, job.taps, job.Oslab, job.O, job.I, job.dw, job.accumulate,
-                       (long)blockIdx.x - job.first_block, red);
+                       (long)blockIdx.x - job.first_block, red, job.kind == WGR_STEM);
 }
 
 #ifdef DH_WS_TIMING
@@ -1319,6 +1333,13 @@
     return conv2d_wgrad_impl(DH_DTYPE_BF16, xs16, d, dw2, 0, N, OH, OW, 16, OH, OW, 64, 4, 1, 2, 1, 0, use_tr, 0, 16, 1, workspace,
                              stream, 0, nullptr, nullptr, nullptr, 1, y, coef, groups);
 }
+extern "C" int dh_stem_wgrad_bn_partial(const void* xs16, const void* d, const void* y, const float* coef, int groups, int N,
+                                        int OH, int OW, int use_tr, void* workspace, int* splitk_out, void* stream) {
+    DH_REQUIRE(xs16 && d && y && coef && groups >= 1 && N % groups == 0 && workspace && splitk_out,
+               "stem_wgrad_bn_partial: bad arguments (N=%d groups=%d)", N, groups);
+    return conv2d_wgrad_impl(DH_DTYPE_BF16, xs16, d, nullptr, 0, N, OH, OW, 16, OH, OW, 64, 4, 1, 2, 1, 0, use_tr, 0, 16, 1, workspace,
+                             stream, 1, splitk_out, nullptr, nullptr, 1, y, coef, groups);
+}
 extern "C" int dh_wgrad_reduce_job_size(void) { return (int)sizeof(WgReduceJob); }
 extern "C" int dh_wgrad_reduce_outputs_per_block(int Cin) { return wgrad_reduce_epb(Cin); }
 extern "C" int dh_wgrad_reduce_multi(const void* jobs_dev, int njobs, int total_blocks, void* stream) {
@@ -1395,54 +1416,11 @@
 template <typename T>
 __global__ void pack_phase_weights_kernel(const float* __restrict__ w, const float* __restrict__ bias, int Cin,
                                           T* __restrict__ fwd, T* __restrict__ dgrad, float* __restrict__ bias4) {
-    const int i = blockIdx.x * blockDim.x + threadIdx.x;
-    if (i < 128 && bias4) bias4[i] = bias ? bias[i & 31] : 0.f;
-    if (i >= 32 * Cin) return;
-    const int co = i / Cin, ci = i % Cin;
-    float k[3][3];
-#pragma unroll
-    for (int j = 0; j < 9; ++j) k[j / 3][j % 3] = w[(size_t)i * 9 + j];
-    const int lo[2][2] = {{0, 1}, {0, 2}}, hi[2][2] = {{0, 2}, {1, 2}};
-#pragma unroll
-    for (int a = 0; a < 2; ++a)
-#pragma unroll
-        for (int b = 0; b < 2; ++b)
-#pragma unroll
-            for (int t = 0; t < 2; ++t)
-#pragma unroll
-                for (int u = 0; u < 2; ++u) {
-                    float s = 0.f;
-                    for (int kh = lo[a][t]; kh <= hi[a][t]; ++kh)
-                        for (int kw = lo[b][u]; kw <= hi[b][u]; ++kw) s += k[kh][kw];
-                    const int ph = a * 2 + b;
-                    if (fwd) stf(fwd + ((size_t)(t * 2 + u) * 128 + ph * 32 + co) * Cin + ci, s);
-                    if (dgrad) stf(dgrad + ((size_t)((1 - t) * 2 + (1 - u)) * Cin + ci) * 128 + ph * 32 + co, s);
-                }
-}
-}
-
-namespace {
+    dh_pack_phase_weights_elem<T>(w, bias, Cin, fwd, dgrad, bias4, blockIdx.x * blockDim.x + threadIdx.x);
+}
 template <typename T>
 __global__ void pack_s2_dgrad_phase_kernel(const float* __restrict__ w, int Co, int Ci, T* __restrict__ out) {
-    const int i = blockIdx.x * blockDim.x + threadIdx.x;
-    if (i >= Co * Ci) return;
-    const int co = i / Ci, ci = i % Ci;
-    float k[3][3];
-#pragma unroll
-    for (int j = 0; j < 9; ++j) k[j / 3][j % 3] = w[(size_t)i * 9 + j];
-    const int kmap[2][2] = {{-1, 1}, {2, 0}};
-#pragma unroll
-    for (int a = 0; a < 2; ++a)
-#pragma unroll
-        for (int b = 0; b < 2; ++b)
-#pragma unroll
-            for (int t = 0; t < 2; ++t)
-#pragma unroll
-                for (int u = 0; u < 2; ++u) {
-                    const int kh = kmap[a][t], kw = kmap[b][u];
-                    const float v = (kh >= 0 && kw >= 0) ? k[kh][kw] : 0.f;
-                    stf(out + ((size_t)(t * 2 + u) * 4 * Ci + (a * 2 + b) * Ci + ci) * Co + co, v);
-                }
+    dh_pack_s2_dgrad_phase_elem<T>(w, Co, Ci, out, blockIdx.x * blockDim.x + threadIdx.x);
 }
 }
 extern "C" int dh_pack_s2_dgrad_phase_weights(int dtype, const float* w_oihw, int Co, int Ci, void* out, void* stream) {
diff --git a/dahitra_amd/csrc/pointwise.hip b/dahitra_amd/csrc/pointwise.hip
--- a/dahitra_amd/csrc/pointwise.hip
+++ b/dahitra_amd/csrc/pointwise.hip
@@ -808,7 +808,11 @@
     int O, I, KS, OPad, IPad, OK;
     int dtype;
     int first_block, nblocks;
+    int kind;
+    const float* bias;
+    float* bias4;
 };
+enum { PACK_KIND_WEIGHT = 0, PACK_KIND_ZERO = 1, PACK_KIND_PHASE = 2, PACK_KIND_S2_DGRAD = 3 };
 template <typename T>
 __device__ __forceinline__ void pack_store8(T* dst, const float* __restrict__ src, unsigned stride, unsigned okmask) {
     float v[8];
@@ -955,6 +959,20 @@
         }
     }
 }
+__device__ __forceinline__ void pack_job_zero(const PackJob& j, int lb) {
+    unsigned char* p = reinterpret_cast<unsigned char*>(j.fwd);
+    const long bytes = (long)j.O + ((long)j.I << 31);
+    long head = (long)((16 - (reinterpret_cast<unsigned long long>(p) & 15)) & 15);
+    if (head > bytes) head = bytes;
+    const long nvec = (bytes - head) >> 4, tail0 = head + (nvec << 4);
+    const long t0 = (long)lb * 256 + threadIdx.x, step = (long)j.nblocks * 256;
+    uint4* v = reinterpret_cast<uint4*>(p + head);
+    for (long i = t0; i < nvec; i += step) v[i] = make_uint4(0u, 0u, 0u, 0u);
+    if (lb == 0) {
+        if ((long)threadIdx.x < head) p[threadIdx.x] = 0;
+        if (tail0 + (long)threadIdx.x < bytes) p[tail0 + threadIdx.x] = 0;
+    }
+}
 __global__ __launch_bounds__(256) void pack_weights_multi_kernel(const PackJob* __restrict__ jobs, int njobs) {
     int lo = 0, hi = njobs - 1;
     while (lo < hi) {
@@ -963,6 +981,21 @@
     }
     const PackJob j = jobs[lo];
     const int lb = blockIdx.x - j.first_block;
+    if (j.kind == PACK_KIND_ZERO) { pack_job_zero(j, lb); return; }
+    if (j.kind == PACK_KIND_PHASE || j.kind == PACK_KIND_S2_DGRAD) {
+        const int n = (j.kind == PACK_KIND_PHASE ? 32 : j.O) * j.I, n128 = n < 128 ? 128 : n;
+        const bool b16 = (j.dtype & 0xff) == DH_DTYPE_BF16;
+        for (int i = lb * 256 + (int)threadIdx.x; i < n128; i += j.nblocks * 256) {
+            if (j.kind == PACK_KIND_PHASE) {
+                if (b16) dh_pack_phase_weights_elem<bf16>(j.w, j.bias, j.I, (bf16*)j.fwd, (bf16*)j.dgrad, j.bias4, i);
+                else dh_pack_phase_weights_elem<float>(j.w, j.bias, j.I, (float*)j.fwd, (float*)j.dgrad, j.bias4, i);
+            } else {
+                if (b16) dh_pack_s2_dgrad_phase_elem<bf16>(j.w, j.O, j.I, (bf16*)j.fwd, i);
+                else dh_pack_s2_dgrad_phase_elem<float>(j.w, j.O, j.I, (float*)j.fwd, i);
+            }
+        }
+        return;
+    }
     __shared__ __attribute__((aligned(16))) float tile[PK_T * PK_PITCH];
     if (pack_tiled(j)) {
         if ((j.dtype & 0xff) == DH_DTYPE_BF16) pack_job_tiled<bf16>(j, lb, tile); else pack_job_tiled<float>(j, lb, tile);
@@ -1307,16 +1340,26 @@
     DH_CHECK_LAUNCH("pack_weights_multi");
     return 0;
 }
-extern "C" int dh_colsum(int dtype, const void* x, long P, int C, float* out, int accumulate, void* workspace, void* stream) {
+static int colsum_partial(int dtype, const void* x, long P, int C, float* partial, int* rows_out, void* stream) {
     DH_REQUIRE(C >= 1 && C <= 256, "colsum: C=%d out of range", C);
     const long rows_per_pass = 256 / (C >= 4 && (C & 3) == 0 ? C / 4 : C);
     long want = (P + rows_per_pass * 8 - 1) / (rows_per_pass * 8);
     const int grid = (int)(want < 64 ? 64 : (want > 256 ? 256 : want));
-    float* partial = reinterpret_cast<float*>(workspace);
     if (dtype == DH_DTYPE_BF16) hipLaunchKernelGGL(colsum_partial_kernel<bf16>, dim3(grid), dim3(256), 0, ST(stream), (const bf16*)x, P, C, partial);
     else hipLaunchKernelGGL(colsum_partial_kernel<float>, dim3(grid), dim3(256), 0, ST(stream), (const float*)x, P, C, partial);
     DH_CHECK_LAUNCH("colsum");
-    return dh_reduce_partials(partial, grid, C, 1.0f, out, accumulate, stream);
+    *rows_out = grid;
+    return 0;
+}
+extern "C" int dh_colsum_partial(int dtype, const void* x, long P, int C, float* partial, int* rows_out, void* stream) {
+    DH_REQUIRE(partial && rows_out, "colsum_partial: partial / rows_out missing");
+    return colsum_partial(dtype, x, P, C, partial, rows_out, stream);
+}
+extern "C" int dh_colsum(int dtype, const void* x, long P, int C, float* out, int accumulate, void* workspace, void* stream) {
+    int rows = 0;
+    float* partial = reinterpret_cast<float*>(workspace);
+    const int rc = colsum_partial(dtype, x, P, C, partial, &rows, stream);
+    return rc ? rc : dh_reduce_partials(partial, rows, C, 1.0f, out, accumulate, stream);
 }
 extern "C" int dh_cast_from_f32(int dtype, const float* src, void* dst, long n, void* stream) {
     if (dtype == DH_DTYPE_BF16) hipLaunchKernelGGL(cast_from_f32_kernel<bf16>, dim3(ew_grid(n, 256)), dim3(256), 0, ST(stream), src, (bf16*)dst, n);
diff --git a/dahitra_amd/engine.py b/dahitra_amd/engine.py
--- a/dahitra_amd/engine.py
+++ b/dahitra_amd/engine.py
@@ -281,7 +281,7 @@
             dy = ops.act_bwd(dout, out, RELU) if (act == RELU and not masked) else dout
             ops.conv2d_wgrad(x, dy, self.g[wkey], ks, 1, pad, accumulate=True, use_tr=self.use_tr)
             if bkey:
-                ops.colsum(dy.view(-1, cout), self.g[bkey], accumulate=True)
+                ops.colsum(dy.view(-1, cout), self.g[bkey], accumulate=True, defer=True)
             dx = self.conv_dgrad(dy, wkey, ks, 1, pad, x.shape, residual=dx_res) if need_dx else None
             return dx
         return out, bwd
@@ -295,7 +295,7 @@
 
         def bwd(dout):
             ops.conv_up2_wgrad(x, dout, self.g[wkey], accumulate=True, use_tr=self.use_tr)
-            ops.colsum(dout.view(-1, 32), self.g[bkey], accumulate=True)
+            ops.colsum(dout.view(-1, 32), self.g[bkey], accumulate=True, defer=True)
             return ops.conv_up2_dgrad(dout, wd, x.shape[-1])
         return out, bwd
 
@@ -909,7 +909,7 @@
         tok_cat, tsaved = ops.tokenizer_fwd(feat, wa, self.p["pos_embedding"], B, L)
         tok2d, b_enc = self.encoder(tok_cat.view(B * 2 * L, DIM), "transformer", cfg["enc_depth"], BIT_HEADS,
                                     BIT_DIM_HEAD, B, 2 * L)
-        dtok = torch.zeros_like(tok2d) if self.need_grad else None
+        dtok = ops.zeros_like(tok2d) if self.need_grad else None
         dec, b_dec = self.decoder(feat.view(S2 * hw, DIM), S2, tok2d, 2 * L * DIM, L * DIM, B, dtok,
                                   "transformer_decoder", cfg["dec_depth"], BIT_HEADS, cfg["dec_dim_head"], L)
         dec4 = dec.view(S2, fh, fw, DIM)
@@ -963,7 +963,7 @@
             out = zp[0][zp[1]:zp[1] + n].view(t.shape)
             zp[1] += (n + 63) // 64 * 64
             return out
-        return torch.zeros_like(t)
+        return ops.zeros_like(t)
 
     def _run_staged(self, gens, ew=False):
         vals = {}
@@ -1074,7 +1074,7 @@
             if pos is not None:
                 ops.add_pos_bwd(dxin, self.g["pos_embedding_decoder_3"], accumulate=True)
             dcat = b_cd(dxin)
-            dtok = torch.zeros_like(tok2d)
+            dtok = ops.zeros_like(tok2d)
             ops.absdiff_halves_bwd(tk3, ddtk, dtok)
             dtok_cat = b_enc(dtok)
             yield
@@ -1102,7 +1102,7 @@
         def bwd(dout, masked=False):
             dy = dout if masked else ops.act_bwd(dout, out, RELU)
             ops.conv_up2_wgrad(x, dy, self.g[wkey], accumulate=True, use_tr=self.use_tr)
-            ops.colsum(dy.view(-1, 32), self.g[bkey], accumulate=True)
+            ops.colsum(dy.view(-1, 32), self.g[bkey], accumulate=True, defer=True)
             return ops.conv_up2_dgrad(dy, wd, 32)
         return out, bwd
 
@@ -1117,7 +1117,7 @@
         s16, b_l3 = self.res_layer(p16, 3, 1, 2)
         level = self._xbd_level if self.cfg["kind"] == "xbd" else self._level
         if self.need_grad:
-            self._zpool = [torch.zeros(3 * 3 * B * self.cfg["token_len"] * DIM, dtype=torch.float32, device=s4.device), 0]
+            self._zpool = [ops.zeros((3 * 3 * B * self.cfg["token_len"] * DIM,), torch.float32, s4.device), 0]
         ew = self.cfg["kind"] != "xbd"
         (o5, b5), (t4, b4), (t3, b3) = self._run_staged([level(5, s16, B), level(4, s8, B), level(3, s4, B)], ew=ew)
         self._zpool = None
@@ -1142,7 +1142,7 @@
             do2 = b_out(dl, relu_out=o2)
             dy2 = bu2(do2, masked=True)
             ops.conv2d_wgrad(y, dy2, self.g["conv_layer2_0.3.weight"], 3, 1, 1, accumulate=True, use_tr=self.use_tr)
-            ops.colsum(dy2.view(-1, 32), self.g["conv_layer2_0.3.bias"], accumulate=True)
+            ops.colsum(dy2.view(-1, 32), self.g["conv_layer2_0.3.bias"], accumulate=True, defer=True)
             dy = self.conv_dgrad(dy2, "conv_layer2_0.3.weight", 3, 1, 1, y.shape, gate=b20.gate)
             dcat2, _ = b20(dy)
             if split2:
diff --git a/dahitra_amd/graph.py b/dahitra_amd/graph.py
--- a/dahitra_amd/graph.py
+++ b/dahitra_amd/graph.py
@@ -21,6 +21,7 @@
         self.persist_bn_launches = None
         self._set_inputs(a, b, lab)
         net._ensure_arena(a.device)
+        self._step_plan = ops.StepPlan(a.device) if ops.FOLD_SMALL else None
         flat0 = net._arena.flat.clone()
         bufs0 = [t.clone() for t in net.buffers()]
         conf0 = confusion.clone() if confusion is not None else None
@@ -46,6 +47,8 @@
             confusion.copy_(conf0)
         cs = self._capture_stream = torch.cuda.Stream()
         ops.rekey_workspace(a.device, s, cs)
+        if self._step_plan is not None and self._step_plan.frozen:
+            ops.rekey_bn_sync(a.device, s, cs)
         self.graph = torch.cuda.CUDAGraph()
         if split:
             self.graph2 = torch.cuda.CUDAGraph()
@@ -64,6 +67,9 @@
             with torch.cuda.graph(self.graph, stream=cs):
                 self.loss = self._body(include_opt=not self.exchange)
         self._pinned = ops.pin_captured_buffers(net)
+        if self._step_plan is not None:
+            self._pinned += self._step_plan.tensors()
+            ops._PINNED.extend(self._step_plan.tensors())
         self._generation = net._arena.generation
         self._calls = 0
         torch.cuda.synchronize()
@@ -92,18 +98,36 @@
         if type(self)._eager_body is not GraphedTrainStep._eager_body or os.environ.get("DAHITRA_GRAPH_AUTOGRAD") == "1":
             return self._eager_body(include_opt)
         net = self.net
-        logits = self._forward_split()
-        bwd = net._engine.take_backward()
-        self.logits = logits
-        loss, dl = self._loss_and_grad(logits)
-        self._count(logits)
-        net._arena.grad.zero_()
-        net._engine.backward(dl, bwd)
+        self._plan_begin()
+        try:
+            logits = self._forward_split()
+            bwd = net._engine.take_backward()
+            self.logits = logits
+            loss, dl = self._loss_and_grad(logits)
+            self._count(logits)
+            ops.zero_(net._arena.grad)
+            net._engine.backward(dl, bwd)
+        except BaseException:
+            self._plan_abort()
+            raise
+        self._plan_end()
         net._bind_grad_views()
         if include_opt:
             self.opt.step()
         return loss
 
+    def _plan_begin(self):
+        if self._step_plan is not None:
+            self._step_plan.begin()
+
+    def _plan_end(self):
+        if self._step_plan is not None:
+            self._step_plan.end()
+
+    def _plan_abort(self):
+        if self._step_plan is not None:
+            self._step_plan.abort()
+
     def _forward_split(self):
         return self.net._run_forward(self.a, self.b, need_grad=True)
 
@@ -122,22 +146,32 @@
 
     def _split_first(self):
         net = self.net
-        logits = self._forward_split()
-        bwd = net._engine.take_backward()
-        self.logits = logits
-        loss, dl = self._loss_and_grad(logits)
-        self._count(logits)
-        net._arena.grad.zero_()
-        net._engine.backward_first(dl, bwd)
+        self._plan_begin()
+        try:
+            logits = self._forward_split()
+            bwd = net._engine.take_backward()
+            self.logits = logits
+            loss, dl = self._loss_and_grad(logits)
+            self._count(logits)
+            ops.zero_(net._arena.grad)
+            net._engine.backward_first(dl, bwd)
+        except BaseException:
+            self._plan_abort()
+            raise
         net._bind_grad_views()
         return loss
 
     def _second(self):
-        if os.environ.get("DAHITRA_OVERLAP_PERSIST_BN") == "1":
-            self.net._engine.backward_second()
-            return
-        with ops.no_persist_bn():
-            self.net._engine.backward_second()
+        try:
+            if os.environ.get("DAHITRA_OVERLAP_PERSIST_BN") == "1":
+                self.net._engine.backward_second()
+            else:
+                with ops.no_persist_bn():
+                    self.net._engine.backward_second()
+        except BaseException:
+            self._plan_abort()
+            raise
+        self._plan_end()
 
     def _after_replay(self):
         parallel.allreduce_net_grads_(self.net)
diff --git a/dahitra_amd/ops.py b/dahitra_amd/ops.py
--- a/dahitra_amd/ops.py
+++ b/dahitra_amd/ops.py
@@ -135,7 +135,10 @@
     class _Job(ctypes.Structure):
         _fields_ = [("w", ctypes.c_void_p), ("fwd", ctypes.c_void_p), ("dgrad", ctypes.c_void_p), ("O", ctypes.c_int),
                     ("I", ctypes.c_int), ("KS", ctypes.c_int), ("OPad", ctypes.c_int), ("IPad", ctypes.c_int),
-                    ("OK", ctypes.c_int), ("dtype", ctypes.c_int), ("first_block", ctypes.c_int), ("nblocks", ctypes.c_int)]
+                    ("OK", ctypes.c_int), ("dtype", ctypes.c_int), ("first_block", ctypes.c_int), ("nblocks", ctypes.c_int),
+                    ("kind", ctypes.c_int), ("bias", ctypes.c_void_p), ("bias4", ctypes.c_void_p)]
+
+    KIND_WEIGHT, KIND_ZERO, KIND_PHASE, KIND_S2_DGRAD = 0, 1, 2, 3
 
     def __init__(self, device):
         self.device, self.jobs, self.blocks, self.table, self.keep = device, [], 0, None, []
@@ -163,12 +166,17 @@
             nb = min(256, (O // 32) * (I // 32))
         self.jobs.append(self._Job(w.data_ptr(), fwd.data_ptr() if fwd is not None else None,
                                    dg.data_ptr() if dg is not None else None, O, I, ks, OPad, IPad, OK,
-                                   _DT[dtype] | (0x200 if frag else 0), self.blocks, nb))
+                                   _DT[dtype] | (0x200 if frag else 0), self.blocks, nb, self.KIND_WEIGHT, None, None))
         self.blocks += nb
         self.keep += [w, fwd, dg]
         return fwd, dg
 
     def run(self):
+        sp = _step_plan()
+        if sp is not None and sp.arm():
+            table, njobs, blocks = sp.table_for(self)
+            _call("dh_pack_weights_multi", P(table), _ci(njobs), _ci(blocks), S())
+            return
         if not self.jobs:
             return
         if self.table is None:
@@ -178,12 +186,157 @@
         _call("dh_pack_weights_multi", P(self.table), _ci(len(self.jobs)), _ci(self.blocks), S())
 
 
+FOLD_SMALL = os.environ.get("DAHITRA_FOLD_SMALL", "1") != "0"
+_STEP_PLAN = None
+
+
+def _step_plan():
+    return _STEP_PLAN if PROFILE is None else None
+
+
+class StepPlan:
+
+    def __init__(self, device):
+        self.device = device
+        self.head, self.frozen, self.armed = [], False, False
+        self.bufs, self.cur, self.bcur, self._zeroed = [], 0, 0, set()
+        self._tables = {}
+
+    def begin(self):
+        global _STEP_PLAN
+        if _STEP_PLAN is not None:
+            raise RuntimeError("dahitra_amd: a StepPlan is already active")
+        _STEP_PLAN = self
+        self.cur, self.bcur, self.armed, self._zeroed = 0, 0, False, set()
+
+    def end(self):
+        global _STEP_PLAN
+        _STEP_PLAN = None
+        if not self.frozen:
+            self.frozen = True
+        elif self.cur != len(self.head):
+            raise RuntimeError("dahitra_amd: the recorded step made %d of the %d requests its first pass made" % (self.cur, len(self.head)))
+
+    def abort(self):
+        global _STEP_PLAN
+        _STEP_PLAN = None
+
+    def arm(self):
+        if not self.frozen or not self.head or self.cur != 0 or self.armed:
+            return False
+        self.armed = True
+        return True
+
+    def table_for(self, pack):
+        key = (id(pack), len(pack.jobs))
+        t = self._tables.get(key)
+        if t is None:
+            if torch.cuda.is_current_stream_capturing():
+                raise RuntimeError("dahitra_amd: the step plan's job table is missing during graph capture; run two eager "
+                                   "passes of the step first")
+            J = PackPlan._Job
+            assert ctypes.sizeof(J) == _lib.lib().dh_pack_job_size()
+            raw, blocks = [bytes(j) for j in pack.jobs], pack.blocks
+            for _, j in self.head:
+                j.first_block = blocks
+                blocks += j.nblocks
+                raw.append(bytes(j))
+            t = self._tables[key] = (torch.frombuffer(bytearray(b"".join(raw)), dtype=torch.uint8).to(self.device),
+                                     len(raw), blocks, pack)
+        return t[:3]
+
+    def tensors(self):
+        return list(self.bufs) + [t[0] for t in self._tables.values()]
+
+    def _request(self, sig, job):
+        i, self.cur = self.cur, self.cur + 1
+        if not self.frozen:
+            self.head.append((sig, job))
+            return False
+        if i >= len(self.head) or self.head[i][0] != sig:
+            raise RuntimeError("dahitra_amd: the recorded step's request %d (%s) differs from its first pass; build a new "
+                               "GraphedTrainStep" % (i, sig[0]))
+        return self.armed
+
+    def _buf(self, nbytes):
+        i, self.bcur = self.bcur, self.bcur + 1
+        if i == len(self.bufs):
+            if self.frozen:
+                raise RuntimeError("dahitra_amd: the recorded step asks for a buffer its first pass did not")
+            self.bufs.append(torch.empty(max(int(nbytes), 16), dtype=torch.uint8, device=self.device))
+        if self.bufs[i].numel() < nbytes:
+            raise RuntimeError("dahitra_amd: the recorded step's buffer %d grew; build a new GraphedTrainStep" % i)
+        return self.bufs[i]
+
+    def _typed(self, shape, dtype):
+        n = 1
+        for d in shape:
+            n *= int(d)
+        nbytes = n * torch.empty(0, dtype=dtype).element_size()
+        return self._buf(nbytes)[:nbytes].view(dtype).view(*shape), nbytes
+
+    @staticmethod
+    def _zero_job(ptr, nbytes):
+        nb = max(1, min(256, cdiv(nbytes, 16 * 256 * 4)))
+        return PackPlan._Job(None, ptr, None, nbytes & 0x7fffffff, nbytes >> 31, 0, 0, 0, 0, 0, 0, nb, PackPlan.KIND_ZERO, None, None)
+
+    def zeros(self, shape, dtype):
+        t, nbytes = self._typed(shape, dtype)
+        if not self._request(("zeros", t.data_ptr(), nbytes), self._zero_job(t.data_ptr(), nbytes)):
+            t.zero_()
+        return t
+
+    def zero_(self, t):
+        assert t.is_contiguous()
+        if t.data_ptr() in self._zeroed:
+            return t
+        self._zeroed.add(t.data_ptr())
+        nbytes = t.numel() * t.element_size()
+        if not self._request(("zero_", t.data_ptr(), nbytes), self._zero_job(t.data_ptr(), nbytes)):
+            t.zero_()
+        return t
+
+    def phase_weights(self, w, bias, dtype):
+        I = w.shape[1]
+        (fwd, _), (dg, _), (b4, _) = self._typed((4, 128, I), dtype), self._typed((4, I, 128), dtype), self._typed((128,), torch.float32)
+        job = PackPlan._Job(w.data_ptr(), fwd.data_ptr(), dg.data_ptr(), 32, I, 3, 0, 0, 0, _DT[dtype], 0, cdiv(32 * I, 256),
+                            PackPlan.KIND_PHASE, bias.data_ptr() if bias is not None else None, b4.data_ptr())
+        if not self._request(("phase", w.data_ptr(), bias.data_ptr() if bias is not None else 0, I, _DT[dtype], fwd.data_ptr()), job):
+            _call("dh_pack_phase_weights", _ci(_DT[dtype]), P(w), P(bias), _ci(I), P(fwd), P(dg), P(b4), S())
+        return fwd, dg, b4
+
+    def s2_dgrad_phase_weights(self, w, dtype):
+        Co, Ci = w.shape[0], w.shape[1]
+        out, _ = self._typed((4, 4 * Ci, Co), dtype)
+        job = PackPlan._Job(w.data_ptr(), out.data_ptr(), None, Co, Ci, 3, 0, 0, 0, _DT[dtype], 0, cdiv(Co * Ci, 256),
+                            PackPlan.KIND_S2_DGRAD, None, None)
+        if not self._request(("s2_dgrad", w.data_ptr(), Co, Ci, _DT[dtype], out.data_ptr()), job):
+            _call("dh_pack_s2_dgrad_phase_weights", _ci(_DT[dtype]), P(w), _ci(Co), _ci(Ci), P(out), S())
+        return out
+
+
+def zeros(shape, dtype, device):
+    sp = _step_plan()
+    return sp.zeros(tuple(shape), dtype) if sp is not None else torch.zeros(*shape, dtype=dtype, device=device)
+
+
+def zeros_like(t):
+    return zeros(t.shape, t.dtype, t.device)
+
+
+def zero_(t):
+    sp = _step_plan()
+    return sp.zero_(t) if sp is not None else t.zero_()
+
+
 class WgradPlan:
 
     class _Job(ctypes.Structure):
         _fields_ = [("part", ctypes.c_void_p), ("dw", ctypes.c_void_p), ("splitk", ctypes.c_int), ("taps", ctypes.c_int),
                     ("Oslab", ctypes.c_int), ("O", ctypes.c_int), ("I", ctypes.c_int), ("accumulate", ctypes.c_int),
-                    ("first_block", ctypes.c_int), ("nblocks", ctypes.c_int)]
+                    ("first_block", ctypes.c_int), ("nblocks", ctypes.c_int), ("kind", ctypes.c_int), ("scale", ctypes.c_float)]
+
+    KIND_SPLITK, KIND_PARTIALS, KIND_STEM = 0, 1, 2
 
     def __init__(self, device, batch=False):
         self.device, self.slots, self.cur, self.blocks = device, [], 0, 0
@@ -192,12 +345,14 @@
         self.post = []
         self.batch = batch and os.environ.get("DAHITRA_WGRAD_BATCH", "1") != "0"
         self.batching, self.keep = False, []
+        self._targets = set()
 
     def __enter__(self):
         global _WGRAD_PLAN
         self._prev, _WGRAD_PLAN = _WGRAD_PLAN, self
         self.cur = 0
         self.jobs = []
+        self._targets = set()
         self.post = []
         self.blocks = 0
         self.phase = 0
@@ -239,7 +394,26 @@
     def add(self, part, dw, splitk, taps, oslab, o, i, accumulate):
         nb = cdiv(o * i * taps, _lib.lib().dh_wgrad_reduce_outputs_per_block(i))
         self.jobs.append(self._Job(part.data_ptr(), dw.data_ptr(), splitk, taps, oslab, o, i, int(accumulate),
-                                   self.blocks, nb))
+                                   self.blocks, nb, self.KIND_SPLITK, 1.0))
+        self.blocks += nb
+
+    def folding(self):
+        return _step_plan() is not None
+
+    def add_partials(self, part, rows, n, out, accumulate, scale=1.0):
+        if out.data_ptr() in self._targets:
+            return False
+        self._targets.add(out.data_ptr())
+        nb = cdiv(n, 32)
+        self.jobs.append(self._Job(part.data_ptr(), out.data_ptr(), rows, 0, 0, n, 0, int(accumulate), self.blocks, nb,
+                                   self.KIND_PARTIALS, scale))
+        self.blocks += nb
+        return True
+
+    def add_stem(self, part, dw, splitk, accumulate):
+        nb = cdiv(64 * 16 * 16, _lib.lib().dh_wgrad_reduce_outputs_per_block(16))
+        self.jobs.append(self._Job(part.data_ptr(), dw.data_ptr(), splitk, 16, 64, 64, 16, int(accumulate), self.blocks, nb,
+                                   self.KIND_STEM, 1.0))
         self.blocks += nb
 
     def run(self):
@@ -250,7 +424,7 @@
             self._run_reduce()
         for fn in self.post:
             fn()
-        self.jobs, self.post, self.blocks = [], [], 0
+        self.jobs, self.post, self.blocks, self._targets = [], [], 0, set()
         self.phase += 1
 
     def _run_reduce(self):
@@ -607,6 +781,8 @@
 def pack_phase_weights(w, bias, dtype):
     O, I = w.shape[0], w.shape[1]
     assert O == 32 and tuple(w.shape[2:]) == (3, 3)
+    if _step_plan() is not None:
+        return _step_plan().phase_weights(w, bias, dtype)
     fwd = torch.empty(4, 128, I, dtype=dtype, device=w.device)
     dg = torch.empty(4, I, 128, dtype=dtype, device=w.device)
     b4 = torch.empty(128, dtype=torch.float32, device=w.device)
@@ -627,6 +803,8 @@
 
 def pack_s2_dgrad_phase_weights(w, dtype):
     Co, Ci = w.shape[0], w.shape[1]
+    if _step_plan() is not None:
+        return _step_plan().s2_dgrad_phase_weights(w, dtype)
     out = torch.empty(4, 4 * Ci, Co, dtype=dtype, device=w.device)
     _call("dh_pack_s2_dgrad_phase_weights", _ci(_DT[dtype]), P(w), _ci(Co), _ci(Ci), P(out), S())
     return out
@@ -764,6 +942,14 @@
         y, coef, groups = bn
         assert cp == 16 and O == 64 and y.shape == dy.shape
         L = _lib.lib()
+        plan = _WGRAD_PLAN
+        if plan is not None and plan.folding():
+            ws = plan.slab(L.dh_conv2d_wgrad_workspace_size(N, H2, W2, 16, O, 4, 1))
+            sk = ctypes.c_int(0)
+            _call("dh_stem_wgrad_bn_partial", P(x_s2d), P(dy), P(y), P(coef), _ci(groups), _ci(N), _ci(H2), _ci(W2),
+                  _ci(int(use_tr)), P(ws), ctypes.byref(sk), S())
+            plan.add_stem(ws, dw, sk.value, accumulate)
+            return
         ws = workspace(L.dh_conv2d_wgrad_workspace_size(N, H2, W2, 16, O, 4, 1), dy.device)
         with _Prof("conv_wgrad<bf16,ks4,s1>", 2.0 * N * H2 * W2 * O * 16 * 16, _nb(x_s2d, dy, y)):
             _call("dh_stem_wgrad_bn", P(x_s2d), P(dy), P(y), P(coef), _ci(groups), _ci(N), _ci(H2), _ci(W2), P(dw2),
@@ -837,7 +1023,19 @@
     t = _BN_SYNC.get(key)
     if t is None:
         t = _BN_SYNC[key] = torch.zeros(8192, dtype=torch.int32, device=device)
+    sp = _step_plan()
+    if sp is not None:
+        sp.zero_(t)
     return t
+
+
+def rekey_bn_sync(device, old_stream, new_stream):
+    t = _BN_SYNC.pop((str(device), old_stream.cuda_stream), None)
+    if t is not None:
+        prev = _BN_SYNC.get((str(device), new_stream.cuda_stream))
+        if prev is not None:
+            _BN_SYNC[(str(device), ("retired", prev.data_ptr()))] = prev
+        _BN_SYNC[(str(device), new_stream.cuda_stream)] = t
 
 
 def bn_persist_check(device=None):
@@ -1154,9 +1352,18 @@
     _call("dh_absdiff_bwd", _ci(dt(a)), P(a), P(b), P(dy), P(da), P(db), _cl(a.numel()), _ci(int(accumulate)), S())
 
 
-def colsum(x2d, out, accumulate=False):
+def colsum(x2d, out, accumulate=False, defer=False):
     C = x2d.shape[-1]
     Pn = x2d.numel() // C
+    plan = _WGRAD_PLAN if defer else None
+    if plan is not None and plan.folding():
+        part = plan.slab(1024 * C * 4 + 1024).view(torch.float32)
+        rows = ctypes.c_int(0)
+        _call("dh_colsum_partial", _ci(dt(x2d)), P(x2d), _cl(Pn), _ci(C), P(part), ctypes.byref(rows), S())
+        if not plan.add_partials(part, rows.value, C, out, accumulate):
+            plan.post.append(lambda n=rows.value: _call("dh_reduce_partials", P(part), _cl(n), _cl(C), _cf(1.0), P(out),
+                                                        _ci(int(accumulate)), S()))
+        return
     ws = workspace(1024 * C * 4 + 1024, x2d.device)
     _call("dh_colsum", _ci(dt(x2d)), P(x2d), _cl(Pn), _ci(C), P(out), _ci(int(accumulate)), P(ws), S())
 
diff --git a/include/dahitra_hip.h b/include/dahitra_hip.h
--- a/include/dahitra_hip.h
+++ b/include/dahitra_hip.h
@@ -91,6 +91,8 @@
                              float* dbeta, int accumulate, void* workspace, void* stream);
 int dh_stem_wgrad_bn(const void* xs16, const void* d, const void* y, const float* coef, int groups, int N, int OH, int OW,
                      float* dw2, int use_tr, void* workspace, void* stream);
+int dh_stem_wgrad_bn_partial(const void* xs16, const void* d, const void* y, const float* coef, int groups, int N, int OH,
+                             int OW, int use_tr, void* workspace, int* splitk_out, void* stream);
 
 int dh_bn_finalize(const float* partial, int ntiles, int CP, int C, int groups, double count, const float* gamma,
                    const float* beta, float* running_mean, float* running_var, float momentum, float eps,
@@ -176,6 +178,7 @@
 int dh_absdiff(int dtype, const void* a, const void* b, void* y, long n, void* stream);
 int dh_absdiff_bwd(int dtype, const void* a, const void* b, const void* dy, void* da, void* db, long n, int accumulate, void* stream);
 int dh_colsum(int dtype, const void* x, long P, int C, float* out, int accumulate, void* workspace, void* stream);
+int dh_colsum_partial(int dtype, const void* x, long P, int C, float* partial, int* rows_out, void* stream);
 int dh_cast_from_f32(int dtype, const float* src, void* dst, long n, void* stream);
 int dh_cast_to_f32(int dtype, const void* src, float* dst, long n, int accumulate, void* stream);
 
```
